# saiakarsh193/GenVox

Hardware: AMD Instinct MI355X
Metric: mel-frames/sec (teacher-forced batch) (higher is better)
Workload: dtype f32

## Files before the change

### genvox_amd/_lib.py

```python
from __future__ import annotations

import ctypes as C
import os

_HERE = os.path.dirname(os.path.abspath(__file__))
LIB_PATH = os.path.join(_HERE, os.environ.get("GVX_LIB", "libgenvox_amd.so"))


class GvxError(RuntimeError):
    pass


class gvx_dims(C.Structure):
    _fields_ = [(n, C.c_int32) for n in (
        "n_tokens", "embed_dim", "enc_kernel", "enc_n_conv", "prenet_dim", "att_rnn_dim", "dec_rnn_dim", "att_dim",
        "att_loc_filters", "att_loc_kernel", "postnet_dim", "postnet_kernel", "postnet_n_conv", "n_mels")]


class gvx_weight_desc(C.Structure):
    _fields_ = [("name", C.c_char_p), ("data", C.c_void_p), ("numel", C.c_int64)]


_vp, _i, _sz, _f, _l = C.c_void_p, C.c_int, C.c_size_t, C.c_float, C.c_long

# ... 192 lines not shown
    "gvx_mel_project": (_i, [_vp, _i, _i, _i, _vp, _i, _vp, _vp]),
    "gvx_dtw_workspace_bytes": (_sz, [_i, _i, _i, _i]),
    "gvx_dtw_uses_lds_tables": (_i, [_i, _i, _i]),
    "gvx_dtw_distance": (_i, [_vp, _vp, _vp, _vp, _i, _i, _i, _i, _vp, _vp, _vp, _sz, _vp]),
    "gvx_monotonic_align_workspace_bytes": (_sz, [_i, _i, _i]),
    "gvx_monotonic_align_uses_lds": (_i, [_i, _i]),
    "gvx_monotonic_align": (_i, [_vp, _vp, _vp, _i, _i, _i, _f, _vp, _vp, _vp, _vp, _vp, _vp, _vp, _sz, _vp]),
    "gvx_duration_scale": (_i, [_vp, _vp, _vp, _i, _i, _f, _vp, _vp, _vp, _vp, _vp]),
    "gvx_mel_time_warp": (_i, [_vp, _vp, _vp, _vp, _i, _i, _i, _i, _i, _vp, _vp, _vp, _vp, _vp]),
    "gvx_pitch_frames": (_i, [_l, _i]),
    "gvx_pitch_tile_frames": (_i, [C.POINTER(gvx_pitch_params)]),
    "gvx_pitch_yin": (_i, [_vp, _vp, _i, _l, C.POINTER(gvx_pitch_params), _vp, _vp, _vp, _vp, _vp]),
    "gvx_f0_compare": (_i, [_vp, _vp, _vp, _vp, _i, _i, _vp, _vp, _vp, _vp, _vp]),
    "gvx_psola_max_marks": (_l, [_l, _i]),
    "gvx_psola_max_grains": (_l, [_l, _i]),
    "gvx_psola_plan": (_i, [_vp, _vp, _vp, _vp, _i, _l, C.POINTER(gvx_psola_params), _vp, _vp, _vp, _vp, _vp, _vp, _vp]),
    "gvx_psola_synth": (_i, [_vp, _vp, _vp, _vp, _vp, _vp, _vp, _vp, _i, _l, C.POINTER(gvx_psola_params), _vp, _vp]),
    "gvx_melgan_blob_floats":(_sz, [C.POINTER(gvx_melgan_dims)]),
    "gvx_melgan_workspace_bytes": (_sz, [C.POINTER(gvx_melgan_dims), _i, _i]),
    "gvx_melgan_pack_weights_device": (_i, [C.POINTER(gvx_melgan_dims), C.POINTER(gvx_weight_desc), _i, _vp, _vp]),
    "gvx_melgan_create": (_i, [C.POINTER(gvx_melgan_dims), C.POINTER(_vp)]),
    "gvx_melgan_destroy": (None, [_vp]),
    "gvx_melgan_bind": (_i, [_vp, _vp]),
    "gvx_melgan_forward": (_i, [_vp, _vp, _vp, _i, _i, _vp, C.POINTER(_vp), _vp, _sz, _vp]),
    "gvx_melgan_timing_enable": (_i, [_vp, _i]),
    "gvx_melgan_stage_times_ms": (_i, [_vp, C.POINTER(_f), C.POINTER(_i)]),
    "gvx_melgan_tape_bytes": (_sz, [C.POINTER(gvx_melgan_dims), _i, _i]),
    "gvx_melgan_tape_layout": (_i, [C.POINTER(gvx_melgan_dims), _i, _i, C.POINTER(gvx_melgan_tape_entry), _i]),
    "gvx_melgan_backward_workspace_bytes": (_sz, [C.POINTER(gvx_melgan_dims), _i, _i]),
    "gvx_melgan_forward_train": (_i, [_vp, _vp, _vp, _i, _i, _vp, _vp, _sz, _vp, _sz, _vp]),
    "gvx_melgan_backward": (_i, [_vp, _vp, _vp, _i, _i, _vp, _sz, C.POINTER(gvx_weight_desc), _i, _vp, _vp, _sz, _vp]),
    "gvx_hifigan_blob_floats": (_sz, [C.POINTER(gvx_hifigan_dims)]),
    "gvx_hifigan_workspace_bytes": (_sz, [C.POINTER(gvx_hifigan_dims), _i, _i]),
    "gvx_hifigan_pack_weights_device": (_i, [C.POINTER(gvx_hifigan_dims), C.POINTER(gvx_weight_desc), _i, _vp, _vp]),
    "gvx_hifigan_create": (_i, [C.POINTER(gvx_hifigan_dims), C.POINTER(_vp)]),
    "gvx_hifigan_destroy": (None, [_vp]),
    "gvx_hifigan_bind": (_i, [_vp, _vp]),
    "gvx_hifigan_forward": (_i, [_vp, _vp, _vp, _i, _i, _vp, C.POINTER(_vp), _vp, _sz, _vp]),
    "gvx_hifigan_timing_enable": (_i, [_vp, _i]),
    "gvx_hifigan_stage_times_ms": (_i, [_vp, C.POINTER(_f), C.POINTER(_i)]),
    "gvx_hifigan_backward_stage_times_ms": (_i, [_vp, C.POINTER(_f), C.POINTER(_i)]),
    "gvx_hifigan_tape_bytes": (_sz, [C.POINTER(gvx_hifigan_dims), _i, _i]),
    "gvx_hifigan_tape_layout": (_i, [C.POINTER(gvx_hifigan_dims), _i, _i, C.POINTER(gvx_melgan_tape_entry), _i]),
    "gvx_hifigan_backward_workspace_bytes": (_sz, [C.POINTER(gvx_hifigan_dims), _i, _i]),
    "gvx_hifigan_forward_train": (_i, [_vp, _vp, _vp, _i, _i, _vp, _vp, _sz, _vp, _sz, _vp]),
    "gvx_hifigan_backward": (_i, [_vp, _vp, _vp, _i, _i, _vp, _sz, C.POINTER(gvx_weight_desc), _i, _vp, _vp, _sz, _vp]),
    "gvx_melgan_disc_blob_floats": (_sz, [C.POINTER(gvx_melgan_disc_dims)]),
    "gvx_melgan_disc_pack_weights_device": (_i, [C.POINTER(gvx_melgan_disc_dims), C.POINTER(gvx_weight_desc), _i, _vp, _vp]),
    "gvx_melgan_disc_create": (_i, [C.POINTER(gvx_melgan_disc_dims), C.POINTER(_vp)]),
    "gvx_melgan_disc_destroy": (None, [_vp]),
    "gvx_melgan_disc_bind": (_i, [_vp, _vp]),
    "gvx_melgan_disc_layout": (_i, [C.POINTER(gvx_melgan_disc_dims), _i, _i, C.POINTER(gvx_melgan_disc_entry), _i]),
    "gvx_melgan_disc_features_bytes": (_sz, [C.POINTER(gvx_melgan_disc_dims), _i, _i]),
    "gvx_melgan_disc_workspace_bytes": (_sz, [C.POINTER(gvx_melgan_disc_dims), _i, _i, _i]),
    "gvx_melgan_disc_forward": (_i, [_vp, _vp, _vp, _i, _i, _vp, _sz, _vp, _sz, _vp]),
    "gvx_melgan_disc_backward": (_i, [_vp, _vp, _vp, _i, _i, _vp, _vp, C.POINTER(gvx_weight_desc), _i, _vp, _vp, _sz, _vp]),
    "gvx_snake_antialiased": (_i, [_vp, _vp, _i, _i, _i, _vp, _vp, _vp, _vp, _vp]),
    "gvx_bigvgan_blob_floats": (_sz, [C.POINTER(gvx_bigvgan_dims)]),
    "gvx_bigvgan_workspace_bytes": (_sz, [C.POINTER(gvx_bigvgan_dims), _i, _i]),
    "gvx_bigvgan_pack_weights_device": (_i, [C.POINTER(gvx_bigvgan_dims), C.POINTER(gvx_weight_desc), _i, _vp, _vp]),
    "gvx_bigvgan_create": (_i, [C.POINTER(gvx_bigvgan_dims), C.POINTER(_vp)]),
    "gvx_bigvgan_destroy": (None, [_vp]),
    "gvx_bigvgan_bind": (_i, [_vp, _vp]),
    "gvx_bigvgan_forward": (_i, [_vp, _vp, _vp, _i, _i, _vp, C.POINTER(_vp), _vp, _sz, _vp]),
    "gvx_bigvgan_timing_enable": (_i, [_vp, _i]),
    "gvx_bigvgan_stage_times_ms": (_i, [_vp, C.POINTER(_f), C.POINTER(_i)]),
    "gvx_dwconv_layernorm": (_i, [_vp, _vp, _i, _i, _i, _i, _vp, _vp, _vp, _vp, _f, _vp, _vp]),
    "gvx_istft_head_workspace_bytes": (_sz, [_i, _i, _i]),
    "gvx_istft_head": (_i, [_vp, _vp, _i, _i, _i, _i, _i, _vp, _vp, _vp, _vp]),
    "gvx_vocos_blob_floats": (_sz, [C.POINTER(gvx_vocos_dims)]),
    "gvx_vocos_workspace_bytes": (_sz, [C.POINTER(gvx_vocos_dims), _i, _i]),
    "gvx_vocos_pack_weights_device": (_i, [C.POINTER(gvx_vocos_dims), C.POINTER(gvx_weight_desc), _i, _vp, _vp]),
    "gvx_vocos_create": (_i, [C.POINTER(gvx_vocos_dims), C.POINTER(_vp)]),
    "gvx_vocos_destroy": (None, [_vp]),
    "gvx_vocos_bind": (_i, [_vp, _vp]),
    "gvx_vocos_forward": (_i, [_vp, _vp, _vp, _i, _i, _vp, C.POINTER(_vp), _vp, _sz, _vp]),
    "gvx_vocos_timing_enable": (_i, [_vp, _i]),
    "gvx_vocos_stage_times_ms": (_i, [_vp, C.POINTER(_f), C.POINTER(_i)]),
    "gvx_self_attention": (_i, [_vp, _vp, _i, _i, _i, _i, _vp, _vp]),
    "gvx_add_layer_norm": (_i, [_vp, _vp, _vp, _i, _i, _i, _vp, _vp, _vp, _vp, _vp]),
    "gvx_fastpitch_blob_floats": (_sz, [C.POINTER(gvx_fastpitch_dims)]),
    "gvx_fastpitch_workspace_bytes": (_sz, [C.POINTER(gvx_fastpitch_dims), _i, _i]),
    "gvx_fastpitch_pack_weights_device": (_i, [C.POINTER(gvx_fastpitch_dims), C.POINTER(gvx_weight_desc), _i, _vp, _vp]),
    "gvx_fastpitch_create": (_i, [C.POINTER(gvx_fastpitch_dims), C.POINTER(_vp)]),
    "gvx_fastpitch_destroy": (None, [_vp]),
    "gvx_fastpitch_bind": (_i, [_vp, _vp]),
    "gvx_fastpitch_encode": (_i, [_vp, _vp, _vp, _i, _i, _f, _vp, _vp, _vp, _vp, _vp, _vp, _vp, _vp, _vp, C.POINTER(_vp), _vp, _sz, _vp]),
    "gvx_fastpitch_decode": (_i, [_vp, _vp, _vp, _vp, _vp, _vp, _i, _i, _i, _vp, _vp, _vp, C.POINTER(_vp), _vp, _sz, _vp]),
    "gvx_fastpitch_timing_enable": (_i, [_vp, _i]),
    "gvx_fastpitch_stage_times_ms": (_i, [_vp, C.POINTER(_f), C.POINTER(_i)]),
    "gvx_lvc_gated": (_i, [_vp, _vp, _i, _i, _vp, _vp, _i, _vp, _i, _i, _i, _i, _f, _vp, _vp, _vp]),
    "gvx_univnet_blob_floats": (_sz, [C.POINTER(gvx_univnet_dims)]),
    "gvx_univnet_workspace_bytes": (_sz, [C.POINTER(gvx_univnet_dims), _i, _i]),
    "gvx_univnet_pack_weights_device": (_i, [C.POINTER(gvx_univnet_dims), C.POINTER(gvx_weight_desc), _i, _vp, _vp]),
    "gvx_univnet_create": (_i, [C.POINTER(gvx_univnet_dims), C.POINTER(_vp)]),
    "gvx_univnet_destroy": (None, [_vp]),
    "gvx_univnet_bind": (_i, [_vp, _vp]),
    "gvx_univnet_forward": (_i, [_vp, _vp, _vp, _vp, _i, _i, _vp, C.POINTER(_vp), _vp, _sz, _vp]),
    "gvx_univnet_timing_enable": (_i, [_vp, _i]),
    "gvx_univnet_stage_times_ms": (_i, [_vp, C.POINTER(_f), C.POINTER(_i)]),
    "gvx_hifigan_mpd_blob_floats": (_sz, [C.POINTER(gvx_hifigan_mpd_dims)]),
    "gvx_hifigan_mpd_pack_weights_device": (_i, [C.POINTER(gvx_hifigan_mpd_dims), C.POINTER(gvx_weight_desc), _i, _vp, _vp]),
    "gvx_hifigan_mpd_create": (_i, [C.POINTER(gvx_hifigan_mpd_dims), C.POINTER(_vp)]),
    "gvx_hifigan_mpd_destroy": (None, [_vp]),
    "gvx_hifigan_mpd_bind": (_i, [_vp, _vp]),
    "gvx_hifigan_mpd_layout": (_i, [C.POINTER(gvx_hifigan_mpd_dims), _i, _i, C.POINTER(gvx_hifigan_mpd_entry), _i]),
    "gvx_hifigan_mpd_features_bytes": (_sz, [C.POINTER(gvx_hifigan_mpd_dims), _i, _i]),
    "gvx_hifigan_mpd_workspace_bytes": (_sz, [C.POINTER(gvx_hifigan_mpd_dims), _i, _i, _i]),
    "gvx_hifigan_mpd_forward": (_i, [_vp, _vp, _vp, _i, _i, _vp, _sz, _vp, _sz, _vp]),
    "gvx_hifigan_mpd_backward": (_i, [_vp, _vp, _vp, _i, _i, _vp, _vp, C.POINTER(gvx_weight_desc), _i, _vp, _vp, _sz, _vp]),
    "gvx_hifigan_mpd_timing_enable": (_i, [_vp, _i]),
    "gvx_hifigan_mpd_layer_times_ms": (_i, [_vp, C.POINTER(_f), C.POINTER(_f), C.POINTER(_i)]),
    "gvx_mrd_blob_floats": (_sz, [C.POINTER(gvx_mrd_dims)]),
    "gvx_mrd_pack_weights_device": (_i, [C.POINTER(gvx_mrd_dims), C.POINTER(gvx_weight_desc), _i, _vp, _vp]),
    "gvx_mrd_create": (_i, [C.POINTER(gvx_mrd_dims), C.POINTER(_vp)]),
    "gvx_mrd_destroy": (None, [_vp]),
    "gvx_mrd_bind": (_i, [_vp, _vp]),
    "gvx_mrd_layout": (_i, [C.POINTER(gvx_mrd_dims), _i, _i, C.POINTER(gvx_mrd_entry), _i]),
    "gvx_mrd_features_bytes": (_sz, [C.POINTER(gvx_mrd_dims), _i, _i]),
    "gvx_mrd_workspace_bytes": (_sz, [C.POINTER(gvx_mrd_dims), _i, _i, _i]),
    "gvx_mrd_forward": (_i, [_vp, _vp, _vp, _i, _i, _vp, _sz, _vp, _sz, _vp]),
    "gvx_mrd_backward": (_i, [_vp, _vp, _vp, _i, _i, _vp, _vp, C.POINTER(gvx_weight_desc), _i, _vp, _vp, _sz, _vp]),
    "gvx_mrd_timing_enable": (_i, [_vp, _i]),
    "gvx_mrd_layer_times_ms": (_i, [_vp, C.POINTER(_f), C.POINTER(_f), C.POINTER(_i)]),
    "gvx_hifigan_msd_blob_floats": (_sz, [C.POINTER(gvx_hifigan_msd_dims)]),
    "gvx_hifigan_msd_pack_weights_device": (_i, [C.POINTER(gvx_hifigan_msd_dims), C.POINTER(gvx_weight_desc), _i, _vp, _vp]),
    "gvx_hifigan_msd_create": (_i, [C.POINTER(gvx_hifigan_msd_dims), C.POINTER(_vp)]),
    "gvx_hifigan_msd_destroy": (None, [_vp]),
    "gvx_hifigan_msd_bind": (_i, [_vp, _vp]),
    "gvx_hifigan_msd_layout": (_i, [C.POINTER(gvx_hifigan_msd_dims), _i, _i, C.POINTER(gvx_hifigan_msd_entry), _i]),
    "gvx_hifigan_msd_features_bytes": (_sz, [C.POINTER(gvx_hifigan_msd_dims), _i, _i]),
    "gvx_hifigan_msd_workspace_bytes": (_sz, [C.POINTER(gvx_hifigan_msd_dims), _i, _i, _i]),
    "gvx_hifigan_msd_forward": (_i, [_vp, _vp, _vp, _i, _i, _vp, _sz, _vp, _sz, _vp]),
    "gvx_hifigan_msd_backward": (_i, [_vp, _vp, _vp, _i, _i, _vp, _vp, C.POINTER(gvx_weight_desc), _i, _vp, _vp, _sz, _vp]),
    "gvx_hifigan_msd_timing_enable": (_i, [_vp, _i]),
    "gvx_hifigan_msd_layer_times_ms": (_i, [_vp, C.POINTER(_f), C.POINTER(_f), C.POINTER(_i)]),
    "gvx_stft_loss_create": (_i, [C.POINTER(gvx_stft_resolution), _i, _f, _f, _f, C.POINTER(_vp)]),
    "gvx_stft_loss_destroy": (None, [_vp]),
    "gvx_stft_loss_workspace_bytes": (_sz, [_vp, _i, _l]),
    "gvx_stft_loss": (_i, [_vp, _vp, _vp, _vp, _i, _l, _vp, _vp, _vp, C.POINTER(gvx_stft_loss_debug), _vp, _sz, _vp]),
    "gvx_mel_loss_create": (_i, [_i, _i, _i, _i, _vp, _f, _f, C.POINTER(_vp)]),
    "gvx_mel_loss_destroy": (None, [_vp]),
    "gvx_mel_loss_bands": (_i, [_vp, _i, _i, _vp, _vp, _vp, _vp]),
    "gvx_mel_loss_workspace_bytes": (_sz, [_vp, _i, _l]),
    "gvx_mel_loss": (_i, [_vp, _vp, _vp, _vp, _i, _l, _vp, _vp, _vp, C.POINTER(gvx_mel_loss_debug), _vp, _sz, _vp]),
    "gvx_denoise_create": (_i, [_i, _i, C.POINTER(_vp)]),
    "gvx_denoise_destroy": (None, [_vp]),
    "gvx_denoise_workspace_bytes": (_sz, [_vp, _i, _l]),
    "gvx_denoise": (_i, [_vp, _vp, _vp, _i, _l, _vp, _f, _vp, _vp, _vp, _sz, _vp]),
    "gvx_kernel_timing_enable": (_i, [_vp, _i]),
    "gvx_model_set_persistent_attention": (_i, [_vp, _i]),
    "gvx_model_set_resident_kernels": (_i, [_vp, _i]),
    "gvx_model_set_winograd": (_i, [_vp, _i]),
    "gvx_debug_conv_plan": (_i, [_vp, _i, _i, _i]),
    "gvx_teacher_forced_rows_per_call": (_i, [_vp, _i]),
    "gvx_teacher_forced_resident": (_i, [_vp, _i, _i]),
    "gvx_teacher_forced_loop_kind": (_i, [_vp, _i, _i]),
    "gvx_autoregressive_loop_kind": (_i, [_vp, _i, _i]),
    "gvx_autoregressive_windowed_loop_kind": (_i, [_vp, _i, _i]),
    "gvx_kernel_times_ms": (_i, [_vp, C.POINTER(_f), C.POINTER(_f), C.POINTER(_i)]),
}

_lib = None


def load() -> C.CDLL:
    global _lib
    if _lib is not None:
        return _lib
    if not os.path.exists(LIB_PATH):
        raise ImportError(
            f"{LIB_PATH} not found: build the gfx950 library first (python -m genvox_amd.build, or "
            f"__graft_entry__.build()). genvox_amd has no CPU or eager fallback.")
    import torch

    lib = C.CDLL(LIB_PATH)
    for name, (res, args) in SIGNATURES.items():
        fn = getattr(lib, name)
        fn.restype = res
        fn.argtypes = args
    _lib = lib
    return lib


def check(rc: int) -> None:
    if rc != 0:
        msg = load().gvx_last_error()
        raise GvxError(f"genvox_amd error {rc}: {msg.decode() if msg else '?'}")
```

### genvox_amd/build.py

```python
from __future__ import annotations

import glob
import os
import subprocess
import sys
from concurrent.futures import ThreadPoolExecutor

HERE = os.path.dirname(os.path.abspath(__file__))
CSRC = os.path.join(HERE, "csrc")
LIB = os.path.join(HERE, "libgenvox_amd.so")
SOURCES = ["gemm_f32.hip", "winograd_conv.hip", "skinny.hip", "dec_resident.hip", "attention.hip", "attn_persist.hip", "misc.hip", "griffinlim.hip", "wav_finalize.hip", "wav_to_mel.hip", "resample.hip", "eval_metrics.hip", "mas.hip", "time_warp.hip", "melgan.hip", "melgan_train.hip", "melgan_disc.hip", "hifigan.hip", "hifigan_train.hip", "hifigan_disc.hip", "hifigan_msd.hip", "mrd.hip", "bigvgan.hip", "vocos.hip", "univnet.hip", "fastpitch.hip", "pitch.hip", "psola.hip", "stft_loss.hip", "mel_loss.hip", "denoise.hip",
           "train_conv.hip", "train_ops.hip", "train_bptt_decoder.hip", "train_bptt_encoder.hip", "train_guided.hip", "gvx_pack.hip", "gvx_decoder.hip", "gvx_api.hip"]
ARCH = "gfx950"
HIPCC = os.environ.get("HIPCC", "/opt/rocm/bin/hipcc")
CXXFLAGS = ["-O3", "-std=c++17", "-fPIC", f"--offload-arch={ARCH}", "-Wall", "-Wno-unused-function",
            "-ffp-contract=off"]


def _newer(a: str, b: str) -> bool:
    return not os.path.exists(b) or os.path.getmtime(a) > os.path.getmtime(b)


def build(force: bool = False, verbose: bool = True, stamps: bool = False) -> str:
    objs, jobs = [], []
    flags = CXXFLAGS + (["-DGVX_STAMPS"] if stamps else []) + os.environ.get("GVX_EXTRA_FLAGS", "").split()
    lib = LIB.replace(".so", "_stamps.so") if stamps else LIB
    if os.environ.get("GVX_LIB_NAME"):
        lib = os.path.join(HERE, os.environ["GVX_LIB_NAME"])
    sfx = ".stamps.o" if stamps else ".o"
    if os.environ.get("GVX_LIB_NAME"):
        sfx = "." + os.environ["GVX_LIB_NAME"] + ".o"
    headers = sorted(glob.glob(os.path.join(CSRC, "*.h"))) + [os.path.join(os.path.dirname(HERE), "include", "genvox_amd.h")]
    for src in SOURCES:
        s = os.path.join(CSRC, src)
        o = os.path.join(CSRC, src.replace(".hip", sfx))
        objs.append(o)
        if force or _newer(s, o) or any(_newer(h, o) for h in headers):
            jobs.append([HIPCC, *flags, "-c", s, "-o", o])

    def run(cmd):
        if verbose:
            print(" ".join(cmd), flush=True)
        subprocess.run(cmd, check=True)

    if jobs:
        with ThreadPoolExecutor(max_workers=min(4, len(jobs))) as ex:
            list(ex.map(run, jobs))
    if jobs or not os.path.exists(lib):
        run([HIPCC, "-shared", "-fPIC", f"--offload-arch={ARCH}", *objs, "-L/opt/rocm/lib", "-lrocfft", "-Wl,-rpath,/opt/rocm/lib", "-o", lib])
    if not stamps and not os.environ.get("GVX_LIB_NAME"):
        variant = LIB.replace(".so", "_stamps.so")
        if os.path.exists(variant) and os.path.getmtime(variant) < os.path.getmtime(headers[-1]):
            os.remove(variant)
    return lib


if __name__ == "__main__":
    print(build(force="--force" in sys.argv, stamps="--stamps" in sys.argv))
```

### genvox_amd/csrc/gvx_api.hip

```cpp
#include "gvx_internal.h"

namespace gvx {
#ifdef GVX_STAMPS
hipError_t read_stamps_skinny(unsigned long long* host96);
hipError_t read_stamps_attention(unsigned long long* host96);
hipError_t read_stamps_persist(unsigned long long* host96);
hipError_t read_wg_spans(unsigned long long* host1024);
hipError_t read_stamps_resident(unsigned long long* host480);
hipError_t read_wg_stamps_resident(unsigned long long* host896);
hipError_t read_wg_stamps_resident_ar(unsigned long long* host896);
hipError_t read_row_stamps_persist_ar(unsigned long long* host256);
hipError_t read_loc_stamps_persist(unsigned long long* host32);
hipError_t read_row_stamps_persist(unsigned long long* host512);
#endif
hipError_t skinny_init();
hipError_t gemm_init();
int gemm_set_parent_epilogue(int on);
int gemm_epilogue_of(int tile, const GemmParams& p);
hipError_t attention_init();
hipError_t attention_persistent_init();
}

using namespace gvx;

// ... 9 lines not shown
    va_list ap;
    va_start(ap, fmt);
    vsnprintf(buf, sizeof buf, fmt, ap);
    va_end(ap);
    g_err = buf;
    return code;
}

std::mutex& capture_mutex() { return g_capture_mutex; }

bool conv_uses_winograd(const gvx_model* m, int cin, int cout, int k) {
    if (m->winograd <= 0 || !winograd_shape_ok(cin, cout, k)) return false;
    return m->winograd >= 2 || cin >= WINOGRAD_MIN_CHANNELS;
}

size_t winograd_scratch_floats(const gvx_model* m, int B, int T) {
    bool any = false;
    for (int i = 0; i < m->d.postnet_n_conv; ++i) any = any || postnet_layer_winograd_shape(m->d, i);
    if (!any) return 0;
    const size_t tile = (size_t)2 * WINO_PTS * m->d.postnet_dim, all = (size_t)B * ((T + WINO_OUT - 1) / WINO_OUT) * tile;
    const size_t budget = WINOGRAD_GROUP_BYTES / sizeof(float) / tile * tile;
    return all <= budget ? all : budget > tile ? budget : tile;
}

long winograd_group_tiles(long total, long fit, int C) {
    if (fit >= total) return total;
    const long groups = (total + fit - 1) / fit, per = (total + groups - 1) / groups;
    GemmParams g{};
    g.M = (int)per; g.N = C; g.K = C; g.slices = WINO_PTS;
    const long unit = gemm_round_rows(g);
    if (unit <= 0) return per;
    auto whole = [&](long rows) { g.M = (int)rows; return rows > 0 && rows <= fit && rows % unit == 0 && gemm_round_rows(g) == unit; };
    const long down = per / unit * unit, up = (per + unit - 1) / unit * unit, most = fit / unit * unit;
    if (whole(down) && total - (groups - 1) * down <= fit) return down;
    if (whole(up)) return up;
    return whole(most) ? most : per;
}

WsPlan make_ws_plan(const gvx_model* m, int B, int L, int T, int mode) {
    const gvx_dims& d = m->d;
    const int E = d.embed_dim, H = E / 2, M = d.n_mels, P = d.prenet_dim, A = d.att_rnn_dim, D = d.dec_rnn_dim;
    const int pe = (d.enc_kernel - 1) / 2, pp = (d.postnet_kernel - 1) / 2;
    WsPlan w{};
    size_t off = 0;
    auto take = [&](size_t floats) { size_t o = off; off = align_up(off + floats * sizeof(float), 256); return o; };
    w.flags = take(128);
    w.sync = take(HANDOFF_WORDS);
    w.xa = take((size_t)B * (L + 2 * pe) * E);
    w.xb = take((size_t)B * (L + 2 * pe) * E);
    w.xg = take((size_t)B * L * 8 * H);
    w.enc_h = take((size_t)2 * 2 * B * H);
    w.enc_c = take((size_t)2 * B * H);
    w.memory = take((size_t)B * L * E);
    w.len_copy = take((size_t)B);
    w.pm = take((size_t)B * L * d.att_dim);
    w.frames = take((size_t)(T + 1) * B * M);
    w.pre1 = take((size_t)(T + 1) * B * P);
    w.prenet = take((size_t)(T + 1) * B * P);
    w.h_a = take((size_t)RS_HA_SLOTS * B * A);
    w.c_a = take((size_t)B * A);
    w.c_d = take((size_t)B * D);
    w.hc = take((size_t)(T + 1) * B * (D + E));
    w.w_cum = take((size_t)B * L);
    w.q_slab = take((size_t)(A / 8) * B * d.att_dim);
    w.proj = take((size_t)B * T * m->PSB());
    w.energies = take((size_t)B * L);
    w.align_tm = take((size_t)T * B * L);
    w.loc = take((size_t)B * L * d.att_dim);
    w.p_slab = take((size_t)(D / 8) * B * m->PSB());
    w.p_ctx = take((size_t)B * m->PSB());
    w.att_part = take((size_t)2 * B * 4 * A);
    w.dec_part = take((size_t)2 * B * 4 * D);
    w.pre_gate = take(mode == WS_TEACHER_FORCED && plan_teacher_forced(m, B, L, TF_INFERENCE).pre_gate ? (size_t)T * B * 4 * A : 0);
    w.xchg = take(attention_persistent_xchg_floats(B));
    w.ar_masks = take(((size_t)2 * T * B * P + 3) / 4);
    const int cmax = d.postnet_dim > M ? d.postnet_dim : M;
    w.ya = take((size_t)B * (T + 2 * pp) * cmax);
    w.yb = take((size_t)B * (T + 2 * pp) * cmax);
    w.total = off;
    return w;
}

gvx_model::GraphSet* touch_graph_set(gvx_model* m, std::vector<gvx_model::GraphSet>& cache, const gvx_model::LoopKey& key) {
    gvx_model::GraphSet* hit = nullptr;
    for (auto& gs : cache)
        if (gs.key == key) hit = &gs;
    if (!hit) {
        if (cache.size() >= gvx_model::GRAPH_SETS) {
            size_t lru = 0;
            for (size_t i = 1; i < cache.size(); ++i)
                if (cache[i].last_use < cache[lru].last_use) lru = i;
            for (auto e : cache[lru].execs)
                if (e) (void)hipGraphExecDestroy(e);
            cache.erase(cache.begin() + lru);
        }
        cache.emplace_back();
        hit = &cache.back();
        hit->key = key;
    }
    ++hit->sightings;
    hit->last_use = ++m->use_clock;
    return hit;
}

int check_common(const gvx_model* m, int B, int L, int T, void* ws, size_t ws_bytes, int mode) {
    if (!m) return fail(GVX_ERR_INVALID_ARG, "null model");
    if (!m->dev_blob) return fail(GVX_ERR_STATE, "weights not bound (call gvx_model_bind_blob)");
    if (B < 1 || B > 64) return fail(GVX_ERR_UNSUPPORTED, "batch %d not in [1, 64] (shard larger batches across calls / GPUs)", B);
    if (L < 1 || T < 1) return fail(GVX_ERR_INVALID_ARG, "L and T must be >= 1");
    if (!ws) return fail(GVX_ERR_WORKSPACE, "null workspace");
    if (reinterpret_cast<uintptr_t>(ws) & 255) return fail(GVX_ERR_WORKSPACE, "workspace must be 256-byte aligned");
    const size_t need = make_ws_plan(m, B, L, T, mode).total;
    if (ws_bytes < need) return fail(GVX_ERR_WORKSPACE, "workspace too small: %zu < %zu bytes", ws_bytes, need);
    if (!attention_supported(L, m->d.att_dim, m->d.att_loc_filters, m->d.att_loc_kernel, m->d.embed_dim))
        return fail(GVX_ERR_UNSUPPORTED, "L = %d is too long for the attention kernels' LDS budget", L);
    return GVX_OK;
}

}

namespace {

int check_dims(const gvx_dims& d) {
    if (d.n_tokens < 1) return fail(GVX_ERR_INVALID_ARG, "n_tokens must be >= 1");
    const int dims8[] = {d.embed_dim, d.prenet_dim, d.att_rnn_dim, d.dec_rnn_dim, d.att_dim, d.postnet_dim, d.n_mels};
    const char* names[] = {"embed_dim", "prenet_dim", "att_rnn_dim", "dec_rnn_dim", "att_dim", "postnet_dim", "n_mels"};
    for (int i = 0; i < 7; ++i)
        if (dims8[i] < 8 || dims8[i] % 8) return fail(GVX_ERR_UNSUPPORTED, "%s = %d must be a positive multiple of 8", names[i], dims8[i]);
    if (d.embed_dim % 16) return fail(GVX_ERR_UNSUPPORTED, "embed_dim = %d must be a multiple of 16 (BiLSTM halves are multiples of 8)", d.embed_dim);
    if (d.att_dim > 256) return fail(GVX_ERR_UNSUPPORTED, "att_dim = %d > 256 is not supported", d.att_dim);
    if (d.att_loc_filters < 1 || d.att_loc_filters > 32) return fail(GVX_ERR_UNSUPPORTED, "att_loc_filters = %d must be in [1, 32]", d.att_loc_filters);
    const int ks[] = {d.enc_kernel, d.att_loc_kernel, d.postnet_kernel};
    for (int k : ks)
        if (k < 1 || k % 2 == 0) return fail(GVX_ERR_UNSUPPORTED, "kernel size %d must be odd (the reference pads (k-1)/2 on both sides)", k);
    if (d.enc_n_conv < 1 || d.enc_n_conv > MAX_CONV || d.postnet_n_conv < 1 || d.postnet_n_conv > MAX_CONV)
        return fail(GVX_ERR_UNSUPPORTED, "number of convolutions must be in [1, %d]", MAX_CONV);
    return GVX_OK;
}

void read_knobs(gvx_model* m) {
    auto env = [](const char* name) { const char* e = std::getenv(name); return e ? e : ""; };
    auto flag = [&](const char* name, bool dflt) { const char c = env(name)[0]; return c == '\0' ? dflt : dflt ? c != '0' : c == '1'; };
    auto number = [&](const char* name, int dflt) { const char* e = env(name); return e[0] ? std::atoi(e) : dflt; };
    m->use_graph = !flag("GVX_NO_GRAPH", false);
    m->capture_first = flag("GVX_GRAPH_FIRST", false);
    m->attn_one_launch = !flag("GVX_ATTN_SPLIT", false);
    m->attn_persistent = flag("GVX_ATTN_PERSISTENT", true);
    for (const char* name : {"AMD_SERIALIZE_KERNEL", "HIP_LAUNCH_BLOCKING"})
        if (env(name)[0] != '\0' && env(name)[0] != '0') m->attn_persistent = false;
    m->ar_resident = flag("GVX_AR_RESIDENT", false);
    m->ar_split_h = flag("GVX_AR_SPLIT_H", true);
    m->enc_persistent = flag("GVX_ENC_PERSISTENT", true);
    m->enc_fork_after = number("GVX_ENC_FORK_AFTER", 2);
    m->train_resident = flag("GVX_TRAIN_RESIDENT", true);
    m->train_resident_loop = flag("GVX_TRAIN_RESIDENT_LOOP", true);
    m->tf_rows64 = flag("GVX_TF_ROWS64", false);
    m->tf_resident = flag("GVX_TF_RESIDENT", true);
    m->ar_resident_loop = flag("GVX_AR_RESIDENT_LOOP", true);
    m->tf_long_rows_224 = flag("GVX_TF_LONG_224", true);
    m->attn_prefetch = flag("GVX_ATTN_PREFETCH", true);
    m->pa_depth = number("GVX_PA_DEPTH", 4) == 6 ? 6 : 4;
    m->side_pool = env("GVX_SIDE_POOL")[0] == '2' ? 2u : 1u;
    m->spin_limit = (unsigned)std::strtoul(env("GVX_HANDOFF_SPIN_LIMIT"), nullptr, 10);
    m->rs_debug = number("GVX_RS_DEBUG", 0);
    m->debug_skip_resident = flag("GVX_DEBUG_SKIP_RESIDENT", false);
    m->debug_enc_skip_block = number("GVX_DEBUG_ENC_SKIP_BLOCK", -1);
    m->debug_plan = std::getenv("GVX_DEBUG_PLAN") != nullptr;
    m->winograd = number("GVX_CONV_WINOGRAD", 1);
    if (m->winograd < 0 || m->winograd > 2) m->winograd = 1;
}

}

extern "C" {

const char* gvx_last_error(void) { return g_err.c_str(); }
int gvx_version(void) { return 1; }

int gvx_model_create(const gvx_dims* dims, gvx_model** out) {
    if (!dims || !out) return fail(GVX_ERR_INVALID_ARG, "null argument");
    int rc = check_dims(*dims);
    if (rc != GVX_OK) return rc;
    gvx_model* m = new gvx_model();
    m->d = *dims;
    m->blob = make_blob_layout(*dims);
    read_knobs(m);
    *out = m;
    return GVX_OK;
}

void gvx_model_destroy(gvx_model* m) {
    if (m) {
        if (m->gather_off) (void)hipFree(m->gather_off);
        if (m->gather_tid) (void)hipFree(m->gather_tid);
    }
    if (!m) return;
    if (m->ev_valid)
        for (auto& e : m->ev) (void)hipEventDestroy(e);
    for (auto& e : m->kev) (void)hipEventDestroy(e);
    m->drop_graphs();
    if (m->cap_stream) (void)hipStreamDestroy(m->cap_stream);
    if (m->pa_fork) (void)hipEventDestroy(m->pa_fork);
    if (m->pa_join) (void)hipEventDestroy(m->pa_join);
    if (m->enc_mid) (void)hipEventDestroy(m->enc_mid);
    if (m->ar_done_host) (void)hipHostFree(m->ar_done_host);
    for (hipEvent_t e : m->ar_ev)
        if (e) (void)hipEventDestroy(e);
    delete m;
}

size_t gvx_model_blob_bytes(const gvx_model* m) { return m ? m->blob.total * sizeof(float) : 0; }

int gvx_model_bind_blob(gvx_model* m, const void* device_blob) {
    if (!m || !device_blob) return fail(GVX_ERR_INVALID_ARG, "null argument");
    if (reinterpret_cast<uintptr_t>(device_blob) & 255) return fail(GVX_ERR_INVALID_ARG, "blob must be 256-byte aligned");
    if (m->dev_blob != device_blob) m->drop_graphs();
    m->dev_blob = reinterpret_cast<const float*>(device_blob);
    HIP_TRY(gemm_init());
    HIP_TRY(skinny_init());
    HIP_TRY(attention_init());
    HIP_TRY(attention_persistent_init());
    HIP_TRY(decoder_resident_init());
    return GVX_OK;
}

size_t gvx_workspace_bytes(const gvx_model* m, int B, int L, int T) {
    if (!m || B < 1 || L < 1 || T < 1) return 0;
    return make_ws_plan(m, B, L, T).total;
}

size_t gvx_workspace_bytes_autoregressive(const gvx_model* m, int B, int L, int max_steps) {
    if (!m || B < 1 || L < 1 || max_steps < 1) return 0;
    return make_ws_plan(m, B, L, max_steps, WS_AUTOREGRESSIVE).total;
}

}

namespace {

int conv_layer(const gvx_model* m, const float* in, float* out, int B, int T, int cin, int cout, int k, size_t w_off, size_t b_off,
               int act, int out_halo, hipStream_t s) {
    const int p = (k - 1) / 2;
    GemmParams g{};
    g.A = in; g.amap = RowMap{T, (long)(T + 2 * p) * cin, (long)cin};
    g.W = m->dev_blob + w_off; g.ldw = (long)k * cin;
    g.C = out + (long)out_halo * cout; g.cmap = RowMap{T, (long)(T + 2 * out_halo) * cout, (long)cout};
    g.bias = m->dev_blob + b_off;
    g.M = B * T; g.N = cout; g.K = k * cin; g.act = act;
    HIP_TRY(launch_gemm(g, s));
    return GVX_OK;
}

int winograd_layer(const gvx_model* m, const char* who, const float* cur, float* nxt, int B, int T, int C, size_t u_off, size_t b_off,
                   const int32_t* row_len, int act, float* wino, size_t wino_floats, hipStream_t s) {
    const long total = (long)B * ((T + WINO_OUT - 1) / WINO_OUT);
    const size_t tile = (size_t)2 * WINO_PTS * C, budget = WINOGRAD_GROUP_BYTES / sizeof(float);
    long fit = (long)((wino_floats < budget ? wino_floats : budget) / tile);
    if (fit < 1) return fail(GVX_ERR_WORKSPACE, "%s: %zu floats of scratch do not hold one Winograd tile (%zu)", who, wino_floats, tile);
    if (m->wino_group > 0 && m->wino_group < fit) fit = m->wino_group;
    const long per_group = winograd_group_tiles(total, fit, C);
    for (long mt0 = 0, Mt; mt0 < total; mt0 += Mt) {
        Mt = total - mt0 <= fit ? total - mt0 : per_group;
        float* V = wino;
        float* Mm = wino + (size_t)WINO_PTS * Mt * C;
        HIP_TRY(launch_winograd_input(cur, V, B, mt0, Mt, T, C, s));
        GemmParams g{};
        g.A = V; g.amap = RowMap{(int)Mt, 0, (long)C};
        g.W = m->dev_blob + u_off; g.ldw = C;
        g.C = Mm; g.cmap = RowMap{(int)Mt, 0, (long)C};
        g.bias = nullptr; g.M = (int)Mt; g.N = C; g.K = C; g.act = ACT_NONE;
        g.slices = WINO_PTS; g.a_slice = Mt * C; g.w_slice = (long)C * C; g.c_slice = Mt * C;
        HIP_TRY(launch_gemm(g, s));
        HIP_TRY(launch_winograd_output(Mm, m->dev_blob + b_off, row_len, nxt, B, mt0, Mt, T, C, act, s));
    }
    return GVX_OK;
}

struct WinoScratch { size_t off, floats; };
WinoScratch encoder_wino_scratch(const WsPlan& wp, bool alone) {
    if (alone) return {wp.xg, (wp.total - wp.xg) / sizeof(float)};
    const size_t front = wp.frames - wp.xg, back = wp.pre_gate - wp.h_a;
    return front >= back ? WinoScratch{wp.xg, front / sizeof(float)} : WinoScratch{wp.h_a, back / sizeof(float)};
}

int encoder_impl(gvx_model* m, const int64_t* tokens, const int32_t* lengths, int B, int L, float* memory_out, void* ws,
                 const WsPlan& wp, const WinoScratch& wsc, hipStream_t s, const float* conv_out = nullptr, float* c_seq_out = nullptr,
                 float* xg_out = nullptr, hipEvent_t dense_done = nullptr) {
    const gvx_dims& d = m->d;
    const int E = d.embed_dim, H = E / 2, pe = (d.enc_kernel - 1) / 2;
    float* xa = ws_ptr<float>(ws, wp.xa);
    float* xb = ws_ptr<float>(ws, wp.xb);
    float* xg = ws_ptr<float>(ws, wp.xg);
    float* enc_h = ws_ptr<float>(ws, wp.enc_h);
    float* enc_c = ws_ptr<float>(ws, wp.enc_c);
    int* flags = ws_ptr<int>(ws, wp.flags);
    float* cur = xa;
    float* nxt = xb;
    if (conv_out) {
        HIP_TRY(launch_to_channels_last(conv_out, xa, B, E, L, pe, nullptr, s));
    } else {
        HIP_TRY(launch_embed(tokens, m->dev_blob + m->blob.emb, d.n_tokens, xa, xb, B, L, E, pe, flags + FLAG_TOKEN, s));
        for (int i = 0; i < d.enc_n_conv; ++i) {
            if (dense_done && i == m->enc_fork_after) { HIP_TRY(hipEventRecord(dense_done, s)); dense_done = nullptr; }
            const bool wino = encoder_layer_winograd_shape(d, i) && conv_uses_winograd(m, E, E, d.enc_kernel);
            int rc = wino ? winograd_layer(m, "encoder", cur, nxt, B, L, E, m->blob.enc_u[i], m->blob.enc_b[i], nullptr, ACT_RELU,
                                           ws_ptr<float>(ws, wsc.off), wsc.floats, s)
                          : conv_layer(m, cur, nxt, B, L, E, E, d.enc_kernel, m->blob.enc_w[i], m->blob.enc_b[i], ACT_RELU, pe, s);
            if (rc != GVX_OK) return rc;
            float* t = cur; cur = nxt; nxt = t;
        }
    }
    if (dense_done) HIP_TRY(hipEventRecord(dense_done, s));
    {
        GemmParams g{};
        g.A = cur + (long)pe * E; g.amap = RowMap{L, (long)(L + 2 * pe) * E, (long)E};
        g.W = m->dev_blob + m->blob.enc_wih; g.ldw = E;
        g.C = xg; g.cmap = RowMap{B * L, 0, (long)8 * H};
        g.bias = m->dev_blob + m->blob.enc_bih;
        g.M = B * L; g.N = 8 * H; g.K = E; g.act = ACT_NONE;
        HIP_TRY(launch_gemm(g, s));
    }
    const bool resident = m->enc_persistent && encoder_persistent_supported(B, H);
    if (!resident) HIP_TRY(zero_async(enc_h, (size_t)4 * B * H * sizeof(float), s));
    if (!resident) HIP_TRY(zero_async(enc_c, (size_t)2 * B * H * sizeof(float), s));
    float* mem_ws = ws_ptr<float>(ws, wp.memory);
    if (!resident) HIP_TRY(zero_async(mem_ws, (size_t)B * L * E * sizeof(float), s));
    const int32_t* len_ws = nullptr;
    if (lengths) {
        int32_t* lc = ws_ptr<int32_t>(ws, wp.len_copy);
        HIP_TRY(hipMemcpyAsync(lc, lengths, (size_t)B * sizeof(int32_t), hipMemcpyDeviceToDevice, s));
        len_ws = lc;
    }
    auto enqueue = [&](hipStream_t st) -> int {
        for (int step = 0; step < L; ++step) {
            SkinnyJob jobs[2];
            for (int dir = 0; dir < 2; ++dir) {
                SkinnyJob& J = jobs[dir];
                std::memset(&J, 0, sizeof J);
                float* h_cur = enc_h + ((size_t)dir * 2 + (step & 1)) * B * H;
                float* h_nxt = enc_h + ((size_t)dir * 2 + ((step + 1) & 1)) * B * H;
                J.Wp = m->dev_blob + m->blob.enc_whh_frag[dir];
                J.x[0] = XSeg{h_cur, H};
                J.N = 4 * H; J.nkg = H / 8; J.mode = 0; J.B = B;
                J.c = enc_c + (size_t)dir * B * H;
                J.h_out = h_nxt;
                J.addend = xg + (size_t)dir * 4 * H; J.add_bs = (long)L * 8 * H; J.add_ts = 8 * H;
                J.lengths = len_ws; J.step = step; J.reverse = dir; J.seq_len = L;
                J.seq_out = mem_ws + (size_t)dir * H; J.seq_bs = (long)L * E; J.seq_ts = E;
                if (c_seq_out) J.c_seq_out = c_seq_out + (size_t)dir * H;
                J.h_prev = h_cur;
            }
            HIP_TRY(launch_skinny(jobs, 2, SK_ENCODER, st));
        }
        return GVX_OK;
    };
    if (resident) {
        unsigned* sync = ws_ptr<unsigned>(ws, wp.sync);
        void* const zp[2] = {enc_h, sync + HANDOFF_TIMEOUT};
        const size_t zb[2] = {(size_t)4 * B * H * sizeof(float), sizeof(unsigned)};
        HIP_TRY(launch_zero_many(zp, zb, 2, s));
        EncPersistParams ep{};
        ep.Wp[0] = m->dev_blob + m->blob.enc_whh_frag[0]; ep.Wp[1] = m->dev_blob + m->blob.enc_whh_frag[1];
        ep.xg = xg; ep.lengths = len_ws; ep.hx = enc_h; ep.seq_out = mem_ws; ep.c_seq_out = c_seq_out;
        ep.sync = sync; ep.spin_limit = m->spin_limit; ep.B = B; ep.L = L; ep.H = H;
        ep.debug_skip_block = m->debug_enc_skip_block;
        HIP_TRY(launch_encoder_persistent(ep, s));
        float* outs[2] = {mem_ws, c_seq_out};
        const size_t counts[2] = {(size_t)B * L * E, (size_t)B * L * E};
        HIP_TRY(launch_poison_on_timeout(sync + HANDOFF_TIMEOUT, flags + FLAG_TIMEOUT, outs, counts, c_seq_out ? 2 : 1, s));
    } else {
        const gvx_model::LoopKey key{ws, mem_ws, m->dev_blob, B, L, 0, lengths != nullptr};
        const int rc = run_chunk(m, m->use_graph && !c_seq_out ? touch_graph_set(m, m->enc_graphs, key) : nullptr, 0, s, enqueue);
        if (rc != GVX_OK) return rc;
    }
    if (xg_out) HIP_TRY(hipMemcpyAsync(xg_out, xg, (size_t)B * L * 8 * H * sizeof(float), hipMemcpyDeviceToDevice, s));
    if (memory_out != mem_ws)
        HIP_TRY(hipMemcpyAsync(memory_out, mem_ws, (size_t)B * L * E * sizeof(float), hipMemcpyDeviceToDevice, s));
    return GVX_OK;
}

int postnet_impl(gvx_model* m, const float* mel_in, const int32_t* mel_lengths, int B, int T, float* mel_post_out, float* ya,
                 float* yb, float* wino, size_t wino_floats, hipStream_t s) {
    const gvx_dims& d = m->d;
    const int M = d.n_mels, pp = (d.postnet_kernel - 1) / 2, n = d.postnet_n_conv;
    HIP_TRY(launch_to_channels_last(mel_in, ya, B, M, T, pp, mel_lengths, s));
    float* cur = ya;
    float* nxt = yb;
    for (int i = 0; i < n; ++i) {
        const int cin = i == 0 ? M : d.postnet_dim, cout = i == n - 1 ? M : d.postnet_dim;
        const bool last = i == n - 1;
        if (postnet_layer_winograd_shape(d, i) && conv_uses_winograd(m, cin, cout, d.postnet_kernel)) {
            const int rc = winograd_layer(m, "Postnet", cur, nxt, B, T, cin, m->blob.post_u[i], m->blob.post_b[i], mel_lengths, ACT_TANH, wino, wino_floats, s);
            if (rc != GVX_OK) return rc;
            float* t = cur; cur = nxt; nxt = t;
            continue;
        }
        const int out_halo = last ? 0 : pp;
        const bool fused_halo = out_halo > 0 && T >= out_halo;
        if (out_halo > 0 && !fused_halo) HIP_TRY(launch_zero_halo(nxt, B, T, pp, cout, s));
        GemmParams g{};
        g.A = cur; g.amap = RowMap{T, (long)(T + 2 * pp) * cin, (long)cin};
        g.W = m->dev_blob + m->blob.post_w[i]; g.ldw = (long)d.postnet_kernel * cin;
        g.C = nxt + (long)out_halo * cout; g.cmap = RowMap{T, (long)(T + 2 * out_halo) * cout, (long)cout};
        g.bias = m->dev_blob + m->blob.post_b[i];
        g.M = B * T; g.N = cout; g.K = d.postnet_kernel * cin; g.act = last ? ACT_NONE : ACT_TANH;
        g.row_len = last ? nullptr : mel_lengths;
        g.c_halo = fused_halo ? out_halo : 0;
        HIP_TRY(launch_gemm(g, s));
        float* t = cur; cur = nxt; nxt = t;
    }
    HIP_TRY(launch_residual_to_channels_first(mel_in, cur, mel_post_out, B, M, T, mel_lengths, s));
    return GVX_OK;
}

struct PostnetPlan { size_t ya, yb, wino, wino_floats, total; };
PostnetPlan make_postnet_plan(const gvx_model* m, int B, int T) {
    const gvx_dims& d = m->d;
    const int pp = (d.postnet_kernel - 1) / 2, cmax = d.postnet_dim > d.n_mels ? d.postnet_dim : d.n_mels;
    const size_t buf = align_up((size_t)B * (T + 2 * pp) * cmax * sizeof(float), 256);
    PostnetPlan p;
    p.ya = align_up((128 + HANDOFF_WORDS) * sizeof(float), 256);
    p.yb = p.ya + buf;
    p.wino = p.yb + buf;
    const WsPlan w = make_ws_plan(m, B, 1, T, WS_AUTOREGRESSIVE);
    const size_t tile = (size_t)2 * WINO_PTS * d.postnet_dim, room = (w.ya - w.xa) / sizeof(float) / tile * tile;
    p.wino_floats = winograd_scratch_floats(m, B, T);
    if (p.wino_floats > room) p.wino_floats = room > tile ? room : tile;
    p.total = p.wino + align_up(p.wino_floats * sizeof(float), 256);
    return p;
}

}

extern "C" {

int gvx_teacher_forced_rows_per_call(const gvx_model* m, int L) {
    if (!m) return 0;
    return plan_teacher_forced(m, 64, L, TF_INFERENCE).kind != 0 ? 64 : 32;
}

int gvx_teacher_forced_resident(const gvx_model* m, int B, int L) {
    if (!m || B < 1 || L < 1) return 0;
    return plan_teacher_forced(m, B, L, TF_INFERENCE).kind != 0 ? 1 : 0;
}

int gvx_teacher_forced_loop_kind(const gvx_model* m, int B, int L) {
    if (!m || B < 1 || L < 1) return 0;
    return plan_teacher_forced(m, B, L, TF_INFERENCE).kind;
}

int gvx_autoregressive_loop_kind(const gvx_model* m, int B, int L) {
    if (!m || B < 1 || L < 1) return 0;
    return plan_autoregressive(m, B, L).kind;
}

int gvx_autoregressive_windowed_loop_kind(const gvx_model* m, int B, int L) {
    if (!m || B < 1 || L < 1) return 0;
    return plan_autoregressive(m, B, L, true).kind;
}

int gvx_debug_decoder_plan_windowed(const gvx_model* m, int B, int L, int* out) {
    if (!m || !out) return fail(GVX_ERR_INVALID_ARG, "null argument");
    if (B < 1 || L < 1) return fail(GVX_ERR_INVALID_ARG, "B, L >= 1 (got %d, %d)", B, L);
    const ArLoopPlan a = plan_autoregressive(m, B, L, true);
    out[0] = a.kind; out[1] = a.split_h; out[2] = a.fold; out[3] = a.graph;
    return GVX_OK;
}

int gvx_debug_decoder_plan(const gvx_model* m, int mode, int B, int L, int* out) {
    if (!m || !out) return fail(GVX_ERR_INVALID_ARG, "null argument");
    if (mode < 0 || mode > 2 || B < 1 || L < 1) return fail(GVX_ERR_INVALID_ARG, "mode must be 0, 1 or 2 and B, L >= 1 (got %d, %d, %d)", mode, B, L);
    const TfLoopPlan t = plan_teacher_forced(m, B, L, (TfMode)mode);
    const ArLoopPlan a = plan_autoregressive(m, B, L);
    const int v[12] = {t.kind, t.pa_layout, t.tile_layout, t.rows64, t.pre_gate, t.timeout_check, t.side_stream, t.graph,
                       a.kind, a.split_h, a.fold, a.graph};
    for (int i = 0; i < 12; ++i) out[i] = v[i];
    return GVX_OK;
}

long long gvx_debug_graph_replays(const gvx_model* m) { return m ? (long long)m->graph_replays : -1; }

int gvx_debug_encoder_resident(const gvx_model* m, int B) {
    if (!m || B < 1) return 0;
    return m->enc_persistent && encoder_persistent_supported(B, m->H()) ? 1 : 0;
}

int gvx_model_set_persistent_attention(gvx_model* m, int enable) {
    if (!m) return fail(GVX_ERR_INVALID_ARG, "null argument");
    m->attn_persistent = enable != 0;
    return GVX_OK;
}

int gvx_model_set_winograd(gvx_model* m, int mode) {
    if (!m) return fail(GVX_ERR_INVALID_ARG, "null argument");
    if (mode < 0 || mode > 2) return fail(GVX_ERR_INVALID_ARG, "winograd mode must be 0, 1 or 2 (got %d)", mode);
    m->winograd = mode;
    return GVX_OK;
}

int gvx_debug_conv_plan(const gvx_model* m, int cin, int cout, int k) {
    if (!m || cin < 1 || cout < 1 || k < 1) return -1;
    return conv_uses_winograd(m, cin, cout, k) ? 1 : 0;
}

int gvx_debug_set_winograd_group(gvx_model* m, int tiles) {
    if (!m || tiles < 0) return fail(GVX_ERR_INVALID_ARG, "bad argument");
    m->wino_group = tiles;
    return GVX_OK;
}

long gvx_debug_winograd_group_tiles(long total, long fit, int channels) {
    if (total < 1 || fit < 1 || channels < 4 || total > INT_MAX) return -1;
    return winograd_group_tiles(total, fit, channels);
}

int gvx_debug_gemm_parent_epilogue(int on) { return gemm_set_parent_epilogue(on); }

int gvx_debug_gemm_epilogue(int tile, int kmajor, int has_bias, int act, int has_keep, int has_row_len, int c_halo) {
    if (tile < 1111 || tile > 9999 || c_halo < 0) return -1;
    static const float some_bias = 0.f; static const uint8_t some_keep = 0; static const int32_t some_len = 0;
    GemmParams g{};
    g.kmajor = kmajor != 0;
    g.bias = has_bias ? &some_bias : nullptr; g.act = act;
    g.keep = has_keep ? &some_keep : nullptr; g.row_len = has_row_len ? &some_len : nullptr; g.c_halo = c_halo;
    return gemm_epilogue_of(tile, g);
}

int gvx_debug_gemm_row_walk(int R, long s1, long s0, int first_row, long* off, int* grp, int* idx) {
    if (R < 1 || first_row < 0 || !off || !grp || !idx) return GVX_ERR_INVALID_ARG;
    const RowMap map{R, s1, s0};
    RowWalk w = row_walk_begin(map, first_row);
    for (int q = 0; q < 16; ++q) {
        if (q > 0) row_walk_advance(w, map, mfma32_row_step(q));
        off[q] = w.off; grp[q] = w.grp; idx[q] = w.idx;
    }
    return GVX_OK;
}

int gvx_debug_winograd_constants(double* at, double* g, double* bt) {
    if (!at || !g || !bt) return fail(GVX_ERR_INVALID_ARG, "null argument");
    for (int i = 0; i < WINO_OUT; ++i)
        for (int s = 0; s < WINO_PTS; ++s) at[i * WINO_PTS + s] = wino_AT(i, s);
    for (int s = 0; s < WINO_PTS; ++s) {
        for (int k = 0; k < WINO_TAPS; ++k) g[s * WINO_TAPS + k] = wino_G(s, k);
        for (int i = 0; i < WINO_PTS; ++i) bt[s * WINO_PTS + i] = wino_BT(s, i);
    }
    return GVX_OK;
}

int gvx_model_set_resident_kernels(gvx_model* m, int enable) {
    if (!m) return fail(GVX_ERR_INVALID_ARG, "null argument");
    m->attn_persistent = m->enc_persistent = m->tf_resident = enable != 0;
    if (!enable) m->ar_resident = false;
    return GVX_OK;
}

int gvx_workspace_status(const gvx_model* m, void* ws, size_t ws_bytes, void* stream, int32_t* host_out) {
    if (!m || !ws || !host_out) return fail(GVX_ERR_INVALID_ARG, "null argument");
    const WsPlan wp = make_ws_plan(m, 1, 1, 1, WS_AUTOREGRESSIVE);
    if (ws_bytes < wp.flags + 4 * sizeof(int32_t)) return fail(GVX_ERR_WORKSPACE, "workspace too small");
    hipStream_t s = (hipStream_t)stream;
    int32_t h[4] = {0, 0, 0, 0}, tmo = 0;
    int32_t* flags = ws_ptr<int32_t>(ws, wp.flags);
    HIP_TRY(hipMemcpyAsync(h, flags, sizeof h, hipMemcpyDeviceToHost, s));
    if (ws_bytes >= wp.sync + HANDOFF_WORDS * sizeof(unsigned))
        HIP_TRY(hipMemcpyAsync(&tmo, reinterpret_cast<const char*>(ws) + wp.sync + HANDOFF_TIMEOUT * sizeof(unsigned), sizeof tmo,
                               hipMemcpyDeviceToHost, s));
    HIP_TRY(zero_async(flags + FLAG_TOKEN, sizeof(int32_t), s));
    HIP_TRY(zero_async(flags + FLAG_TIMEOUT, sizeof(int32_t), s));
    if (ws_bytes >= wp.sync + HANDOFF_WORDS * sizeof(unsigned))
        HIP_TRY(zero_async(ws_ptr<unsigned>(ws, wp.sync) + HANDOFF_TIMEOUT, sizeof(unsigned), s));
    HIP_TRY(hipStreamSynchronize(s));
    host_out[0] = h[FLAG_TOKEN];
    host_out[1] = h[FLAG_TIMEOUT] ? h[FLAG_TIMEOUT] : tmo;
    return GVX_OK;
}

int gvx_encoder_forward(gvx_model* m, const int64_t* tokens, const int32_t* lengths, int B, int L, float* memory_out,
                        void* ws, size_t ws_bytes, void* stream) {
    int rc = check_common(m, B, L, 1, ws, ws_bytes, WS_AUTOREGRESSIVE);
    if (rc != GVX_OK) return rc;
    if (!tokens || !memory_out) return fail(GVX_ERR_INVALID_ARG, "null argument");
    const WsPlan wp = make_ws_plan(m, B, L, 1, WS_AUTOREGRESSIVE);
    return encoder_impl(m, tokens, lengths, B, L, memory_out, ws, wp, encoder_wino_scratch(wp, true), (hipStream_t)stream);
}

int gvx_decoder_teacher_forced(gvx_model* m, const float* memory, const int32_t* lengths, int B, int L, const float* mel_in, int T,
                               const uint8_t* keep_masks, float* mel_out, float* gate_out, float* align_out, void* ws,
                               size_t ws_bytes, void* stream) {
    int rc = check_common(m, B, L, T, ws, ws_bytes);
    if (rc != GVX_OK) return rc;
    if (!memory || !mel_in || !keep_masks || !mel_out || !gate_out || !align_out) return fail(GVX_ERR_INVALID_ARG, "null argument");
    const WsPlan wp = make_ws_plan(m, B, L, T);
    rc = decoder_tf_impl(m, memory, lengths, B, L, mel_in, T, keep_masks, mel_out, gate_out, align_out, ws, wp, (hipStream_t)stream);
    if (rc != GVX_OK) return rc;
    float* outs[3] = {mel_out, gate_out, align_out};
    const size_t counts[3] = {(size_t)B * m->d.n_mels * T, (size_t)B * T, (size_t)B * T * L};
    return poison_if_timed_out(m, B, L, ws, wp, outs, counts, 3, (hipStream_t)stream);
}

int gvx_encoder_lstm_forward(gvx_model* m, const float* conv_out, const int32_t* lengths, int B, int L, float* memory_out,
                             float* cell_states_out, float* input_preact_out, void* ws, size_t ws_bytes, void* stream) {
    int rc = check_common(m, B, L, 1, ws, ws_bytes, WS_AUTOREGRESSIVE);
    if (rc != GVX_OK) return rc;
    if (!conv_out || !memory_out) return fail(GVX_ERR_INVALID_ARG, "null argument");
    if (cell_states_out) HIP_TRY(zero_async(cell_states_out, (size_t)B * L * m->d.embed_dim * sizeof(float), (hipStream_t)stream));
    const WsPlan wp = make_ws_plan(m, B, L, 1, WS_AUTOREGRESSIVE);
    return encoder_impl(m, nullptr, lengths, B, L, memory_out, ws, wp, encoder_wino_scratch(wp, true), (hipStream_t)stream, conv_out, cell_states_out,
                        input_preact_out);
}

int gvx_decoder_teacher_forced_train(gvx_model* m, const float* memory, const int32_t* lengths, int B, int L, const float* mel_in, int T,
                                     const uint8_t* keep_masks, const uint8_t* att_keep, const uint8_t* dec_keep, float p_att, float p_dec,
                                     float* mel_out, float* gate_out, float* align_out, float* att_hidden_all, float* att_cell_all,
                                     float* dec_cell_all, float* dec_hidden_context_all, float* att_preact_all, float* dec_preact_all,
                                     void* ws, size_t ws_bytes, void* stream) {
    int rc = check_common(m, B, L, T, ws, ws_bytes);
    if (rc != GVX_OK) return rc;
    if (!memory || !mel_in || !keep_masks || !att_keep || !dec_keep || !mel_out || !gate_out || !align_out) return fail(GVX_ERR_INVALID_ARG, "null argument");
    if (!(p_att >= 0.f && p_att < 1.f && p_dec >= 0.f && p_dec < 1.f)) return fail(GVX_ERR_INVALID_ARG, "dropout probabilities must be in [0, 1)");
    if (plan_teacher_forced(m, B, L, TF_TRAIN_PARTIAL_TAPE).rows64)
        return fail(GVX_ERR_UNSUPPORTED, "training mode with %d rows on a GVX_TF_ROWS64 handle: the 64-row loop has no dropout and no tape (at most 32 rows per call)", B);
    hipStream_t s = (hipStream_t)stream;
    const int A = m->d.att_rnn_dim, D = m->d.dec_rnn_dim, E = m->d.embed_dim;
    const LstmDropout tr{att_keep, dec_keep, 1.f / (1.f - p_att), 1.f / (1.f - p_dec), att_hidden_all, att_cell_all, dec_cell_all, att_preact_all, dec_preact_all};
    if (att_hidden_all) HIP_TRY(zero_async(att_hidden_all, (size_t)B * A * sizeof(float), s));
    if (att_cell_all) HIP_TRY(zero_async(att_cell_all, (size_t)B * A * sizeof(float), s));
    if (dec_cell_all) HIP_TRY(zero_async(dec_cell_all, (size_t)B * D * sizeof(float), s));
    const WsPlan wp = make_ws_plan(m, B, L, T);
    rc = decoder_tf_impl(m, memory, lengths, B, L, mel_in, T, keep_masks, mel_out, gate_out, align_out, ws, wp, s, false, &tr);
    if (rc != GVX_OK) return rc;
    {
        float* outs[3] = {mel_out, gate_out, align_out};
        const size_t counts[3] = {(size_t)B * m->d.n_mels * T, (size_t)B * T, (size_t)B * T * L};
        rc = poison_if_timed_out(m, B, L, ws, wp, outs, counts, 3, s);
        if (rc != GVX_OK) return rc;
    }
    if (dec_hidden_context_all)
        HIP_TRY(hipMemcpyAsync(dec_hidden_context_all, ws_ptr<float>(ws, wp.hc), (size_t)(T + 1) * B * (D + E) * sizeof(float),
                               hipMemcpyDeviceToDevice, s));
    return GVX_OK;
}

int gvx_train_export(const gvx_model* m, const void* ws_c, size_t ws_bytes, int B, int L, int T, int what, float* dst, void* stream) {
    void* ws = const_cast<void*>(ws_c);
    if (!m || !ws || !dst) return fail(GVX_ERR_INVALID_ARG, "null argument");
    const WsPlan wp = make_ws_plan(m, B, L, T);
    if (ws_bytes < wp.total) return fail(GVX_ERR_WORKSPACE, "workspace too small");
    const gvx_dims& d = m->d;
    hipStream_t s = (hipStream_t)stream;
    const size_t rows = (size_t)(T + 1) * B;
    switch (what) {
        case 0: HIP_TRY(hipMemcpyAsync(dst, ws_ptr<float>(ws, wp.frames), rows * d.n_mels * sizeof(float), hipMemcpyDeviceToDevice, s)); break;
        case 1: HIP_TRY(hipMemcpyAsync(dst, ws_ptr<float>(ws, wp.pre1), rows * d.prenet_dim * sizeof(float), hipMemcpyDeviceToDevice, s)); break;
        case 2: return gvx_train_unblock(ws_ptr<float>(ws, wp.prenet), dst, T + 1, B, d.prenet_dim, stream);
        case 3: HIP_TRY(hipMemcpyAsync(dst, ws_ptr<float>(ws, wp.pm), (size_t)B * L * d.att_dim * sizeof(float), hipMemcpyDeviceToDevice, s)); break;
        case 4: HIP_TRY(hipMemcpyAsync(dst, ws_ptr<float>(ws, wp.memory), (size_t)B * L * d.embed_dim * sizeof(float), hipMemcpyDeviceToDevice, s)); break;
        default: return fail(GVX_ERR_INVALID_ARG, "gvx_train_export: unknown buffer %d", what);
    }
    return GVX_OK;
}

size_t gvx_postnet_workspace_bytes(const gvx_model* m, int B, int T) {
    if (!m || B < 1 || T < 1) return 0;
    return make_postnet_plan(m, B, T).total;
}

int gvx_postnet_forward(gvx_model* m, const float* mel_in, const int32_t* mel_lengths, int B, int T, float* mel_post_out, void* ws,
                        size_t ws_bytes, void* stream) {
    if (!m) return fail(GVX_ERR_INVALID_ARG, "null model");
    if (!m->dev_blob) return fail(GVX_ERR_STATE, "weights not bound (call gvx_model_bind_blob)");
    if (B < 1 || T < 1) return fail(GVX_ERR_INVALID_ARG, "B and T must be >= 1");
    if ((long)B * T > (1L << 30)) return fail(GVX_ERR_UNSUPPORTED, "B * T = %ld frames exceed the GEMM row index range", (long)B * T);
    if (!ws) return fail(GVX_ERR_WORKSPACE, "null workspace");
    if (reinterpret_cast<uintptr_t>(ws) & 255) return fail(GVX_ERR_WORKSPACE, "workspace must be 256-byte aligned");
    const PostnetPlan pp = make_postnet_plan(m, B, T);
    if (ws_bytes < pp.total) return fail(GVX_ERR_WORKSPACE, "workspace too small: %zu < %zu bytes", ws_bytes, pp.total);
    if (!mel_in || !mel_post_out) return fail(GVX_ERR_INVALID_ARG, "null argument");
    return postnet_impl(m, mel_in, mel_lengths, B, T, mel_post_out, ws_ptr<float>(ws, pp.ya), ws_ptr<float>(ws, pp.yb), ws_ptr<float>(ws, pp.wino), pp.wino_floats,
                        (hipStream_t)stream);
}

int gvx_mask_padding(float* mel, float* mel_post, float* gate, const int32_t* mel_lengths, int B, int n_mels, int T, void* stream) {
    if (!mel_lengths || B < 1 || T < 1 || n_mels < 1) return fail(GVX_ERR_INVALID_ARG, "bad argument");
    HIP_TRY(launch_mask_padding(mel, mel_post, gate, mel_lengths, B, n_mels, T, (hipStream_t)stream));
    return GVX_OK;
}

int gvx_tacotron2_forward(gvx_model* m, const int64_t* tokens, const int32_t* token_lengths, int B, int L, const float* mel_in,
                          const int32_t* mel_lengths, int T, const uint8_t* keep_masks, float* mel_out, float* mel_post_out,
                          float* gate_out, float* align_out, void* ws, size_t ws_bytes, void* stream) {
    int rc = check_common(m, B, L, T, ws, ws_bytes);
    if (rc != GVX_OK) return rc;
    if (!tokens || !mel_in || !keep_masks || !mel_out || !gate_out || !align_out)
        return fail(GVX_ERR_INVALID_ARG, "null argument");
    hipStream_t s = (hipStream_t)stream;
    const WsPlan wp = make_ws_plan(m, B, L, T);
    const bool timed = m->timing && m->ev_valid;
    float* memory = ws_ptr<float>(ws, wp.memory);
    if (timed) HIP_TRY(hipEventRecord(m->ev[0], s));
    const bool overlap = plan_teacher_forced(m, B, L, TF_INFERENCE).side_stream;
    if (overlap) {
        rc = ensure_side_stream(m);
        if (rc != GVX_OK) return rc;
        HIP_TRY(hipEventRecord(m->pa_fork, s));
        HIP_TRY(hipStreamWaitEvent(m->pa_stream, m->pa_fork, 0));
        rc = encoder_impl(m, tokens, token_lengths, B, L, memory, ws, wp, encoder_wino_scratch(wp, false), m->pa_stream, nullptr, nullptr, nullptr, m->enc_mid);
        if (rc != GVX_OK) return rc;
        rc = decoder_init_states(m, memory, B, L, decoder_buffers(ws, wp), m->pa_stream);
        if (rc != GVX_OK) return rc;
        HIP_TRY(hipEventRecord(m->pa_join, m->pa_stream));
        HIP_TRY(hipStreamWaitEvent(s, m->enc_mid, 0));
        rc = decoder_prenet_part(m, B, L, mel_in, T, keep_masks, ws, wp, s);
        if (rc != GVX_OK) return rc;
        HIP_TRY(hipStreamWaitEvent(s, m->pa_join, 0));
    } else {
        rc = encoder_impl(m, tokens, token_lengths, B, L, memory, ws, wp, encoder_wino_scratch(wp, false), s);
        if (rc != GVX_OK) return rc;
    }
    if (timed) HIP_TRY(hipEventRecord(m->ev[1], s));
    rc = decoder_tf_impl(m, memory, token_lengths, B, L, mel_in, T, keep_masks, mel_out, gate_out, align_out, ws, wp, s, overlap);
    if (rc != GVX_OK) return rc;
    if (timed) HIP_TRY(hipEventRecord(m->ev[4], s));
    if (mel_post_out) {
        rc = postnet_impl(m, mel_out, nullptr, B, T, mel_post_out, ws_ptr<float>(ws, wp.ya), ws_ptr<float>(ws, wp.yb), ws_ptr<float>(ws, wp.xa),
                          (wp.ya - wp.xa) / sizeof(float), s);
        if (rc != GVX_OK) return rc;
        if (mel_lengths) HIP_TRY(launch_mask_padding(mel_out, mel_post_out, gate_out, mel_lengths, B, m->d.n_mels, T, s));
    }
    float* outs[4] = {mel_out, gate_out, align_out, mel_post_out};
    const size_t nm = (size_t)B * m->d.n_mels * T;
    const size_t counts[4] = {nm, (size_t)B * T, (size_t)B * T * L, nm};
    rc = poison_if_timed_out(m, B, L, ws, wp, outs, counts, mel_post_out ? 4 : 3, s);
    if (rc != GVX_OK) return rc;
    if (timed) HIP_TRY(hipEventRecord(m->ev[5], s));
    return GVX_OK;
}

int gvx_tacotron2_loss(const float* mel_out, const float* mel_post_out, const float* gate_out, const float* mel_target,
                       const float* gate_target, int B, int n_mels, int T, float* loss_out, void* scratch, size_t scratch_bytes,
                       void* stream) {
    if (!mel_out || !mel_post_out || !gate_out || !mel_target || !gate_target || !loss_out || !scratch)
        return fail(GVX_ERR_INVALID_ARG, "null argument");
    if (B < 1 || n_mels < 1 || T < 1) return fail(GVX_ERR_INVALID_ARG, "B, n_mels and T must be >= 1");
    if (scratch_bytes < loss_scratch_bytes() || (reinterpret_cast<uintptr_t>(scratch) & 7))
        return fail(GVX_ERR_WORKSPACE, "scratch too small (%zu bytes needed) or not 8-byte aligned", loss_scratch_bytes());
    HIP_TRY(launch_tacotron2_loss(mel_out, mel_post_out, gate_out, mel_target, gate_target, (long)B * n_mels * T, (long)B * T,
                                  reinterpret_cast<double*>(scratch), loss_out, (hipStream_t)stream));
    return GVX_OK;
}

int gvx_prenet_masks_generate(uint8_t* masks_out, size_t n, uint64_t seed, void* stream) {
    if (!masks_out) return fail(GVX_ERR_INVALID_ARG, "null argument");
    HIP_TRY(launch_mask_gen(masks_out, n, seed, (hipStream_t)stream));
    return GVX_OK;
}

int gvx_stage_timing_enable(gvx_model* m, int enable) {
    if (!m) return fail(GVX_ERR_INVALID_ARG, "null model");
    if (enable && !m->ev_valid) {
        for (auto& e : m->ev) HIP_TRY(hipEventCreate(&e));
        m->ev_valid = true;
    }
    m->timing = enable != 0;
    return GVX_OK;
}

int gvx_kernel_timing_enable(gvx_model* m, int enable) {
    if (!m) return fail(GVX_ERR_INVALID_ARG, "null model");
    m->ktiming = enable != 0;
    return GVX_OK;
}

int gvx_kernel_times_ms(gvx_model* m, float* lstm_avg_ms, float* attn_avg_ms, int* n_steps) {
    if (!m || !lstm_avg_ms || !attn_avg_ms) return fail(GVX_ERR_INVALID_ARG, "null argument");
    if (m->n_lstm_ev < 1) return fail(GVX_ERR_STATE, "no timed decoder loop has run");
    HIP_TRY(hipEventSynchronize(m->kev[2]));
    float a = 0, b = 0;
    HIP_TRY(hipEventElapsedTime(&a, m->kev[0], m->kev[1]));
    HIP_TRY(hipEventElapsedTime(&b, m->kev[1], m->kev[2]));
    *lstm_avg_ms = a / m->n_lstm_ev;
    *attn_avg_ms = m->n_attn_ev > 0 ? b / m->n_attn_ev : 0.f;
    if (n_steps) *n_steps = m->n_lstm_ev;
    return GVX_OK;
}

int gvx_stage_times_ms(gvx_model* m, float* t5, int* launches) {
    if (!m || !t5) return fail(GVX_ERR_INVALID_ARG, "null argument");
    if (!m->ev_valid) return fail(GVX_ERR_STATE, "stage timing was not enabled");
    HIP_TRY(hipEventSynchronize(m->ev[5]));
    for (int i = 0; i < 5; ++i) HIP_TRY(hipEventElapsedTime(&t5[i], m->ev[i], m->ev[i + 1]));
    if (launches) *launches = m->last_decoder_launches;
    return GVX_OK;
}
#ifdef GVX_STAMPS
int gvx_debug_read_stamps_skinny(unsigned long long* host96) {
    HIP_TRY(hipDeviceSynchronize());
    HIP_TRY(gvx::read_stamps_skinny(host96));
    return GVX_OK;
}
int gvx_debug_read_stamps_persist(unsigned long long* host96) {
    HIP_TRY(hipDeviceSynchronize());
    HIP_TRY(gvx::read_stamps_persist(host96));
    return GVX_OK;
}
int gvx_debug_read_wg_spans(unsigned long long* host1024) {
    HIP_TRY(hipDeviceSynchronize());
    HIP_TRY(gvx::read_wg_spans(host1024));
    return GVX_OK;
}
int gvx_debug_read_stamps_resident(unsigned long long* host480) {
    HIP_TRY(hipDeviceSynchronize());
    HIP_TRY(gvx::read_stamps_resident(host480));
    return GVX_OK;
}
int gvx_debug_read_wg_stamps_resident(unsigned long long* host896, unsigned long long* rows512) {
    HIP_TRY(hipDeviceSynchronize());
    HIP_TRY(gvx::read_wg_stamps_resident(host896));
    HIP_TRY(gvx::read_row_stamps_persist(rows512));
    return GVX_OK;
}
int gvx_debug_read_loc_stamps(unsigned long long* host32) {
    HIP_TRY(hipDeviceSynchronize());
    HIP_TRY(gvx::read_loc_stamps_persist(host32));
    return GVX_OK;
}
int gvx_debug_read_stamps_ar(unsigned long long* host896, unsigned long long* rows256) {
    HIP_TRY(hipDeviceSynchronize());
    HIP_TRY(gvx::read_wg_stamps_resident_ar(host896));
    HIP_TRY(gvx::read_row_stamps_persist_ar(rows256));
    return GVX_OK;
}
int gvx_debug_read_stamps(unsigned long long* host96) {
    HIP_TRY(hipDeviceSynchronize());
    unsigned long long tmp[96];
    HIP_TRY(gvx::read_stamps_skinny(host96));
    HIP_TRY(gvx::read_stamps_attention(tmp));
    for (int i = 32; i < 96; ++i) host96[i] = tmp[i];
    return GVX_OK;
}
#endif

}
```

### genvox_amd/csrc/gvx_decoder.hip

```cpp
#include "gvx_internal.h"

using namespace gvx;

namespace gvx {

namespace {
bool resident_attention_serves(const gvx_model* m, int B, int L) {
    const gvx_dims& d = m->d;
    return attention_persistent_supported(B, L, d.att_dim, d.att_loc_filters, d.att_loc_kernel, d.embed_dim, d.att_rnn_dim, d.dec_rnn_dim);
}
}

TfLoopPlan plan_teacher_forced(const gvx_model* m, int B, int L, TfMode mode) {
    TfLoopPlan p{};
    const bool train = mode != TF_INFERENCE;
    const bool pa_shape = (B <= 32 || m->tf_rows64) && m->attn_persistent && m->attn_one_launch && resident_attention_serves(m, B, L);
    const bool pa = pa_shape && (!train || m->train_resident);
    p.pa_layout = attention_persistent_layout(B, L);
    const bool resident = pa && (p.pa_layout == 1 || p.pa_layout == 2) && m->tf_resident &&
                          (!train || (m->train_resident_loop && mode == TF_TRAIN_WHOLE_TAPE)) && decoder_resident_supported(B, L);
    p.kind = resident ? 2 : (pa ? 1 : 0);
    p.tile_layout = resident && p.pa_layout == 2 && B > 2 && B <= 16 && m->tf_long_rows_224 ? 1 : p.pa_layout;
    p.rows64 = p.kind == 1 && p.pa_layout == 3;
    p.pre_gate = p.timeout_check = pa_shape;
    p.side_stream = p.kind != 0;
    p.graph = m->use_graph && !m->ktiming && p.kind != 2 && (p.rows64 || !train);
    return p;
}

ArLoopPlan plan_autoregressive(const gvx_model* m, int B, int L, bool windowed) {
    ArLoopPlan p{};
    const gvx_dims& d = m->d;
    const int E = d.embed_dim, D = d.dec_rnn_dim, lay = attention_persistent_layout(B, L);
    const bool pa_any = m->attn_one_launch && resident_attention_serves(m, B, L);
    const bool pair = pa_any && B <= 32 && E / 4 == D / 8 && m->attn_persistent && m->tf_resident && m->ar_resident_loop &&
                      decoder_resident_supported(B, L) && (lay == 1 || (lay == 2 && B <= 16)) && d.prenet_dim == 256 && d.n_mels <= 80 &&
                      m->PSB() <= 96 && d.att_dim == 128;
    p.kind = pair ? 2 : (pa_any && lay == 1 && m->ar_resident ? 1 : 0);
    if (windowed && !(p.kind == 2 && lay == 1)) p.kind = 0;
    p.fold = B <= 32 && E / 4 == D / 8;
    p.split_h = p.kind == 0 && m->ar_split_h && m->attn_persistent && m->attn_one_launch && B <= 32 && d.att_dim > 32 && d.att_dim <= 128;
    p.graph = m->use_graph && p.kind != 2;
    return p;
}

DecoderBuffers decoder_buffers(void* ws, const WsPlan& wp) {
    DecoderBuffers b;
    b.pm = ws_ptr<float>(ws, wp.pm); b.frames = ws_ptr<float>(ws, wp.frames); b.pre1 = ws_ptr<float>(ws, wp.pre1);
    b.prenet = ws_ptr<float>(ws, wp.prenet); b.h_a = ws_ptr<float>(ws, wp.h_a); b.c_a = ws_ptr<float>(ws, wp.c_a);
    b.c_d = ws_ptr<float>(ws, wp.c_d); b.hc = ws_ptr<float>(ws, wp.hc); b.w_cum = ws_ptr<float>(ws, wp.w_cum);
    b.q_slab = ws_ptr<float>(ws, wp.q_slab); b.proj = ws_ptr<float>(ws, wp.proj); b.energies = ws_ptr<float>(ws, wp.energies);
    b.align_tm = ws_ptr<float>(ws, wp.align_tm); b.len_copy = ws_ptr<int32_t>(ws, wp.len_copy);
    b.loc = ws_ptr<float>(ws, wp.loc);
    b.p_slab = ws_ptr<float>(ws, wp.p_slab); b.p_ctx = ws_ptr<float>(ws, wp.p_ctx);
    b.att_part = ws_ptr<float>(ws, wp.att_part); b.dec_part = ws_ptr<float>(ws, wp.dec_part);
    b.pre_gate = ws_ptr<float>(ws, wp.pre_gate);
    return b;
}

int decoder_init_states(gvx_model* m, const float* memory, int B, int L, const DecoderBuffers& db, hipStream_t s) {
    const gvx_dims& d = m->d;
    const int E = d.embed_dim, A = d.att_rnn_dim, D = d.dec_rnn_dim;
    void* const zp[5] = {db.h_a, db.c_a, db.c_d, db.hc , db.w_cum};
    const size_t zb[5] = {(size_t)RS_HA_SLOTS * B * A * sizeof(float), (size_t)B * A * sizeof(float), (size_t)B * D * sizeof(float),
                          (size_t)B * (D + E) * sizeof(float), (size_t)B * L * sizeof(float)};
    HIP_TRY(launch_zero_many(zp, zb, 5, s));
    GemmParams g{};
    g.A = memory; g.amap = RowMap{B * L, 0, (long)E};
    g.W = m->dev_blob + m->blob.wmem; g.ldw = E;
    g.C = db.pm; g.cmap = RowMap{B * L, 0, (long)d.att_dim};
    g.M = B * L; g.N = d.att_dim; g.K = E; g.act = ACT_NONE;
    HIP_TRY(launch_gemm(g, s));
    return GVX_OK;
}

namespace {

void fill_att_job(const gvx_model* m, SkinnyJob& J, const float* prenet_t, int t, int B, const DecoderBuffers& db) {
    const gvx_dims& d = m->d;
    const int E = d.embed_dim, P = d.prenet_dim, A = d.att_rnn_dim, D = d.dec_rnn_dim;
    std::memset(&J, 0, sizeof J);
    const float* hc_t = db.hc + (size_t)t * B * (D + E);
    J.Wp = m->dev_blob + m->blob.att_frag; J.bias = m->dev_blob + m->blob.att_bias;
    J.x[0] = XSeg{prenet_t, P};
    J.x[1] = XSeg{hc_t + (size_t)D * B, E};
    J.x[2] = XSeg{db.h_a + (size_t)(t & 1) * B * A, A};
    J.N = 4 * A; J.nkg = (P + E + A) / 8; J.mode = 0; J.B = B;
    J.c = db.c_a;
    J.h_out = db.h_a + (size_t)((t + 1) & 1) * B * A;
    J.Wq_t = m->dev_blob + m->blob.wq_t; J.q_slab = db.q_slab; J.att_dim = d.att_dim;
}

void fill_dec_job(const gvx_model* m, SkinnyJob& J, int t, int B, const DecoderBuffers& db) {
    const gvx_dims& d = m->d;
    const int E = d.embed_dim, A = d.att_rnn_dim, D = d.dec_rnn_dim;
    std::memset(&J, 0, sizeof J);
    const float* hc_t = db.hc + (size_t)t * B * (D + E);
    float* hc_n = db.hc + (size_t)(t + 1) * B * (D + E);
    J.Wp = m->dev_blob + m->blob.dec_frag; J.bias = m->dev_blob + m->blob.dec_bias;
    J.x[0] = XSeg{db.h_a + (size_t)((t + 1) & 1) * B * A, A};
    J.x[1] = XSeg{hc_n + (size_t)D * B, E};
    J.x[2] = XSeg{hc_t, D};
    J.N = 4 * D; J.nkg = (A + E + D) / 8; J.mode = 0; J.B = B;
    J.c = db.c_d;
    J.h_out = hc_n;
}

void fill_loc(const gvx_model* m, LocJob& q, int t, int B, int L, const float* align_base, long align_bs, long align_ts,
              const DecoderBuffers& db) {
    const gvx_dims& d = m->d;
    q.w_prev = t > 0 ? align_base + (size_t)(t - 1) * align_ts : nullptr; q.w_prev_bs = align_bs;
    q.w_cum = db.w_cum;
    q.loc_conv_t = m->dev_blob + m->blob.loc_conv; q.loc_dense_t = m->dev_blob + m->blob.loc_dense;
    q.loc_out = db.loc;
    q.pm = m->attn_one_launch ? db.pm : nullptr;
    q.B = B; q.L = L; q.a = d.att_dim; q.kl = d.att_loc_kernel; q.G = attention_groups(B, L);
}

void fill_attn(const gvx_model* m, AttnParams& p, const float* memory, const int32_t* lengths, int t, int B, int L,
               float* align_out, long align_bs, long align_ts, const DecoderBuffers& db) {
    const gvx_dims& d = m->d;
    const int E = d.embed_dim, D = d.dec_rnn_dim;
    std::memset(&p, 0, sizeof p);
    p.q_slab = db.q_slab; p.n_slabs = d.att_rnn_dim / 8;
    p.w_cum = db.w_cum;
    p.loc = db.loc; p.v = m->dev_blob + m->blob.v;
    p.pm = db.pm; p.memory = memory; p.lengths = lengths;
    p.w_out = align_out + (size_t)t * align_ts; p.w_out_bs = align_bs;
    p.ctx_out = db.hc + (size_t)(t + 1) * B * (D + E) + (size_t)D * B;
    p.energies = db.energies;
    p.B = B; p.L = L; p.a = d.att_dim; p.F = d.att_loc_filters; p.kl = d.att_loc_kernel; p.E = E;
    p.G = m->attn_one_launch ? attention_slices(B, E) : attention_groups(B, L);
}

hipError_t launch_attn(const gvx_model* m, const AttnParams& p, hipStream_t s) {
    return m->attn_one_launch ? launch_attention_step(p, s) : launch_attention(p, s);
}

struct SidePool { hipStream_t s[2] = {nullptr, nullptr}; unsigned next = 0; };
std::mutex g_pool_mutex;
std::unordered_map<int, SidePool> g_side_pools;

struct ResidentTurn { hipEvent_t ev[4] = {nullptr, nullptr, nullptr, nullptr}; unsigned n = 0; };
std::mutex g_turn_mutex;
std::unordered_map<int, ResidentTurn> g_turns;

int turn_begin(hipStream_t s) {
    int dev = 0;
    HIP_TRY(hipGetDevice(&dev));
    ResidentTurn& t = g_turns[dev];
    if (!t.ev[0])
        for (auto& e : t.ev) HIP_TRY(hipEventCreateWithFlags(&e, hipEventDisableTiming));
    if (t.n > 0) HIP_TRY(hipStreamWaitEvent(s, t.ev[(t.n - 1) & 3], 0));
    return GVX_OK;
}
int turn_end(hipStream_t s) {
    int dev = 0;
    HIP_TRY(hipGetDevice(&dev));
    ResidentTurn& t = g_turns[dev];
    HIP_TRY(hipEventRecord(t.ev[t.n & 3], s));
    ++t.n;
    return GVX_OK;
}

}

int ensure_side_stream(gvx_model* m) {
    if (!m->pa_fork) {
        HIP_TRY(hipEventCreateWithFlags(&m->pa_fork, hipEventDisableTiming));
        HIP_TRY(hipEventCreateWithFlags(&m->pa_join, hipEventDisableTiming));
        HIP_TRY(hipEventCreateWithFlags(&m->enc_mid, hipEventDisableTiming));
    }
    int dev = 0;
    HIP_TRY(hipGetDevice(&dev));
    std::lock_guard<std::mutex> lock(g_pool_mutex);
    SidePool& pool = g_side_pools[dev];
    if (!pool.s[0]) {
        int least = 0, greatest = 0;
        HIP_TRY(hipDeviceGetStreamPriorityRange(&least, &greatest));
        for (auto& st : pool.s) HIP_TRY(hipStreamCreateWithPriority(&st, hipStreamNonBlocking, greatest));
    }
    m->pa_stream = pool.s[pool.next++ % m->side_pool];
    return GVX_OK;
}

namespace {

AttnPersistParams fill_attn_persist(const gvx_model* m, const DecoderBuffers& db, const float* memory, const int32_t* len_ws,
                                    unsigned* sync, int B, int L, int T) {
    const gvx_dims& d = m->d;
    const int E = d.embed_dim, D = d.dec_rnn_dim;
    AttnPersistParams pp{};
    pp.q_slab = db.q_slab;
    pp.v = m->dev_blob + m->blob.v; pp.pm = db.pm; pp.memory = memory; pp.lengths = len_ws;
    pp.loc_conv_t = m->dev_blob + m->blob.loc_conv; pp.loc_dense_t = m->dev_blob + m->blob.loc_dense;
    pp.w_out = db.align_tm; pp.w_out_bs = (long)L; pp.w_out_ts = (long)B * L;
    pp.ctx_base = db.hc + (size_t)B * (D + E) + (size_t)D * B; pp.ctx_ts = (long)B * (D + E);
    pp.sync = sync; pp.B = B; pp.L = L; pp.T = T; pp.kl = d.att_loc_kernel;
    pp.spin_limit = m->spin_limit;
    return pp;
}
void use_resident_flags(const gvx_model* m, AttnPersistParams& pp) {
    pp.q_flags = pp.sync + RS_FLAG_Q; pp.n_q_flags = pp.n_slabs;
    pp.ctx_flags = pp.sync + RS_FLAG_CTX;
    pp.debug = m->rs_debug;
}

int launch_resident_attention(gvx_model* m, const AttnPersistParams& pp, hipStream_t s) {
    HIP_TRY(hipEventRecord(m->pa_fork, s));
    HIP_TRY(hipStreamWaitEvent(m->pa_stream, m->pa_fork, 0));
    if (!m->debug_skip_resident) HIP_TRY(launch_attention_persistent(pp, m->pa_stream));
    HIP_TRY(hipEventRecord(m->pa_join, m->pa_stream));
    return GVX_OK;
}

template <class P>
void fill_resident_common(const gvx_model* m, const DecoderBuffers& db, unsigned* sync, int B, int T, P& rp) {
    const gvx_dims& d = m->d;
    rp.att_frag = m->dev_blob + m->blob.att_frag; rp.att_bias = m->dev_blob + m->blob.att_bias; rp.wq_t = m->dev_blob + m->blob.wq_t;
    rp.dec_frag = m->dev_blob + m->blob.dec_frag; rp.dec_bias = m->dev_blob + m->blob.dec_bias;
    rp.h_a = db.h_a; rp.hc = db.hc; rp.q_slab = db.q_slab; rp.c_a = db.c_a; rp.c_d = db.c_d;
    rp.sync = sync;
    rp.att_frag_bytes = (unsigned)(frag_floats(4 * d.att_rnn_dim, d.prenet_dim + d.embed_dim + d.att_rnn_dim) * sizeof(float));
    rp.B = B; rp.T = T; rp.spin_limit = m->spin_limit; rp.debug = m->rs_debug;
}

int ensure_ar_host_slots(gvx_model* m) {
    if (m->ar_done_host) return GVX_OK;
    HIP_TRY(hipHostMalloc(reinterpret_cast<void**>(&m->ar_done_host), 2 * sizeof(int32_t), hipHostMallocDefault));
    for (auto& e : m->ar_ev) HIP_TRY(hipEventCreateWithFlags(&e, hipEventDisableTiming));
    return GVX_OK;
}

}

int decoder_prenet_part(gvx_model* m, int B, int L, const float* mel_in, int T, const uint8_t* keep_masks, void* ws, const WsPlan& wp,
                        hipStream_t s) {
    const gvx_dims& d = m->d;
    const int M = d.n_mels, P = d.prenet_dim;
    const DecoderBuffers db = decoder_buffers(ws, wp);
    HIP_TRY(zero_async(db.frames, (size_t)B * M * sizeof(float), s));
    HIP_TRY(launch_frames_from_mel(mel_in, db.frames, B, M, T, s));
    const int rows = (T + 1) * B;
    GemmParams g{};
    g.A = db.frames; g.amap = RowMap{rows, 0, (long)M};
    g.W = m->dev_blob + m->blob.pre_w0; g.ldw = M;
    g.C = db.pre1; g.cmap = RowMap{rows, 0, (long)P};
    g.keep = keep_masks; g.keep_ld = P;
    g.M = rows; g.N = P; g.K = M; g.act = ACT_RELU;
    HIP_TRY(launch_gemm(g, s));
    g.A = db.pre1; g.amap = RowMap{rows, 0, (long)P};
    g.W = m->dev_blob + m->blob.pre_w1; g.ldw = P;
    g.C = db.prenet; g.cmap = RowMap{B, (long)B * P, 8}; g.c_nblk = (long)B * 8;
    g.keep = keep_masks + (size_t)rows * P;
    g.K = P;
    HIP_TRY(launch_gemm(g, s));
    if (plan_teacher_forced(m, B, L, TF_INFERENCE).pre_gate) {
        GemmParams h{};
        h.A = db.prenet; h.amap = RowMap{B, (long)B * P, 8}; h.a_kblk = (long)B * 8;
        h.W = m->dev_blob + m->blob.att_wpre; h.ldw = P;
        h.C = db.pre_gate; h.cmap = RowMap{T * B, 0, (long)4 * d.att_rnn_dim};
        h.M = T * B; h.N = 4 * d.att_rnn_dim; h.K = P; h.act = ACT_NONE;
        HIP_TRY(launch_gemm(h, s));
    }
    return GVX_OK;
}

int poison_if_timed_out(const gvx_model* m, int B, int L, void* ws, const WsPlan& wp, float* const* outs, const size_t* counts, int n,
                        hipStream_t s) {
    if (!plan_teacher_forced(m, B, L, TF_INFERENCE).timeout_check) return GVX_OK;
    HIP_TRY(launch_poison_on_timeout(ws_ptr<unsigned>(ws, wp.sync) + HANDOFF_TIMEOUT, ws_ptr<int>(ws, wp.flags) + FLAG_TIMEOUT, outs, counts, n, s));
    return GVX_OK;
}

namespace {

struct TfLoop {
    gvx_model* m; TfLoopPlan plan; DecoderBuffers db;
    const float* memory; const int32_t* len_ws; void* ws; unsigned* sync; float* xchg;
    int B, L, T;
    const LstmDropout* train;
};

void defer_context(const TfLoop& c, SkinnyJob& J, int t_ctx, bool first) {
    if (c.plan.kind == 0) return;
    const gvx_dims& d = c.m->d;
    J.defer_seg = 1;
    if (J.q_slab) {
        const int P = d.prenet_dim, E = d.embed_dim, A = d.att_rnn_dim;
        J.x[0] = XSeg{J.x[1].p, 0};
        J.kg0 = P / 8; J.nkg_w = (P + E + A) / 8; J.nkg = (E + A) / 8;
        J.addend = c.db.pre_gate + (size_t)(t_ctx + 1) * c.B * 4 * A; J.add_bs = 4 * A;
    }
    J.tmo = c.sync + HANDOFF_TIMEOUT;
    J.spin_limit = c.m->spin_limit;
    if (t_ctx >= 0) { J.ctx_cnt = c.sync + HANDOFF_CNT_CTX; J.ctx_target = (unsigned)c.B * (unsigned)(t_ctx + 1); }
    J.start_cnt = c.sync + HANDOFF_CNT_Q;
    if (first) { J.ready_cnt = c.sync + HANDOFF_READY; J.ready_target = (unsigned)attention_persistent_workgroups(c.B, c.L); }
}

void wire_tape(const LstmDropout& tr, SkinnyJob* att, SkinnyJob* dec, int t, size_t BA, size_t BD) {
    if (att) {
        att->h_keep = tr.att_keep + (size_t)t * BA; att->h_scale = tr.att_scale;
        if (tr.h_a_all) { att->x[2].p = tr.h_a_all + (size_t)t * BA; att->h_out = tr.h_a_all + (size_t)(t + 1) * BA; }
        if (tr.c_a_all) { att->c = tr.c_a_all + (size_t)t * BA; att->c_out = tr.c_a_all + (size_t)(t + 1) * BA; }
        if (tr.pre_a_all) att->pre_out = tr.pre_a_all + (size_t)t * 4 * BA;
    }
    if (dec) {
        if (tr.pre_d_all) dec->pre_out = tr.pre_d_all + (size_t)(t - 1) * 4 * BD;
        dec->h_keep = tr.dec_keep + (size_t)(t - 1) * BD; dec->h_scale = tr.dec_scale;
        if (tr.h_a_all) dec->x[0].p = tr.h_a_all + (size_t)t * BA;
        if (tr.c_d_all) { dec->c = tr.c_d_all + (size_t)(t - 1) * BD; dec->c_out = tr.c_d_all + (size_t)t * BD; }
    }
}

int tf_step_jobs(const TfLoop& c, int t, SkinnyJob* jobs) {
    const gvx_dims& d = c.m->d;
    SkinnyJob* att = t < c.T ? &jobs[0] : nullptr;
    SkinnyJob* dec = t > 0 ? &jobs[att ? 1 : 0] : nullptr;
    if (att) {
        fill_att_job(c.m, *att, c.db.prenet + (size_t)t * c.B * d.prenet_dim, t, c.B, c.db);
        defer_context(c, *att, t - 1, t == 0);
    }
    if (dec) {
        fill_dec_job(c.m, *dec, t - 1, c.B, c.db);
        defer_context(c, *dec, t - 1, false);
    }
    if (c.train) wire_tape(*c.train, att, dec, t, (size_t)c.B * d.att_rnn_dim, (size_t)c.B * d.dec_rnn_dim);
    return (att ? 1 : 0) + (dec ? 1 : 0);
}

int tf_step_jobs64(const TfLoop& c, int t, SkinnyJob* jobs) {
    const gvx_model* m = c.m;
    const gvx_dims& d = m->d;
    const int E = d.embed_dim, P = d.prenet_dim, A = d.att_rnn_dim, D = d.dec_rnn_dim, B = c.B, T = c.T;
    const DecoderBuffers& db = c.db;
    float* dec_part2[2] = {db.dec_part, db.dec_part + (size_t)B * 4 * D};
    int n = 0;
    if (t < T) {
        fill_att_job(m, jobs[n], db.prenet + (size_t)t * B * P, t, B, db);
        defer_context(c, jobs[n], t - 1, t == 0);
        ++n;
    }
    if (t >= 1 && t - 1 < T) {
        SkinnyJob& J = jobs[n];
        fill_dec_job(m, J, t - 1, B, db);
        J.x[2] = XSeg{nullptr, 0};
        J.nkg = (A + E) / 8; J.kg0 = 0; J.nkg_w = (A + E + D) / 8;
        J.mode = 2; J.bias = nullptr; J.c = nullptr; J.h_out = nullptr;
        J.y = dec_part2[t & 1];
        defer_context(c, J, t - 1, false);
        ++n;
    }
    if (t >= 2 && t - 2 < T) {
        SkinnyJob& J = jobs[n];
        std::memset(&J, 0, sizeof J);
        const float* hc_t = db.hc + (size_t)(t - 2) * B * (D + E);
        float* hc_n = db.hc + (size_t)(t - 1) * B * (D + E);
        J.Wp = m->dev_blob + m->blob.dec_frag; J.bias = m->dev_blob + m->blob.dec_bias;
        J.x[0] = XSeg{hc_t, D};
        J.N = 4 * D; J.nkg = D / 8; J.kg0 = (A + E) / 8; J.nkg_w = (A + E + D) / 8; J.mode = 0; J.B = B;
        J.c = db.c_d; J.h_out = hc_n;
        J.addend = dec_part2[(t - 1) & 1]; J.add_bs = 4 * D;
        J.start_cnt = c.sync + HANDOFF_CNT_Q;
        ++n;
    }
    return n;
}

template <class F>
int enqueue_or_replay(const TfLoop& c, int variant, hipStream_t s, F&& enqueue) {
    if (!c.plan.graph) return enqueue(s);
    const gvx_model::LoopKey key{c.ws, c.memory, c.m->dev_blob, c.B, c.L, c.T, c.len_ws != nullptr, 0.f, variant};
    return run_chunk(c.m, touch_graph_set(c.m, c.m->loop_graphs, key), 0, s, enqueue);
}

int tf_loop_resident(const TfLoop& c, hipStream_t s, int* launches) {
    gvx_model* m = c.m;
    const gvx_dims& d = m->d;
    DecResidentParams rp{};
    fill_resident_common(m, c.db, c.sync, c.B, c.T, rp);
    rp.pre_gate = c.db.pre_gate;
    rp.kg_pre = d.prenet_dim / 8;
    if (const LstmDropout* train = c.train) {
        rp.h_a = train->h_a_all;
        rp.tr_keep_a = train->att_keep; rp.tr_keep_d = train->dec_keep; rp.tr_scale_a = train->att_scale; rp.tr_scale_d = train->dec_scale;
        rp.tr_c_a = train->c_a_all; rp.tr_c_d = train->c_d_all; rp.tr_pre_a = train->pre_a_all; rp.tr_pre_d = train->pre_d_all;
    }
    rp.dec_frag_bytes = (unsigned)(frag_floats(4 * d.dec_rnn_dim, d.att_rnn_dim + d.embed_dim + d.dec_rnn_dim) * sizeof(float));
    rp.layout = c.plan.tile_layout;
    if (m->ktiming) HIP_TRY(hipEventRecord(m->kev[0], s));
    HIP_TRY(launch_decoder_resident(rp, s));
    if (m->ktiming) {
        HIP_TRY(hipEventRecord(m->kev[1], s));
        HIP_TRY(hipEventRecord(m->kev[2], s));
        m->n_lstm_ev = c.T; m->n_attn_ev = 0;
    }
    *launches = 1;
    return GVX_OK;
}

int tf_loop_beside_attention(const TfLoop& c, hipStream_t s, int* launches) {
    *launches = c.plan.rows64 ? c.T + 2 : c.T + 1;
    if (c.plan.rows64)
        return enqueue_or_replay(c, 48, s, [&](hipStream_t st) -> int {
            SkinnyJob jobs[3];
            for (int t = 0; t < c.T + 2; ++t) HIP_TRY(launch_skinny_pa64(jobs, tf_step_jobs64(c, t, jobs), st));
            return GVX_OK;
        });
    return enqueue_or_replay(c, c.m->pa_depth + 16 * c.plan.pa_layout, s, [&](hipStream_t st) -> int {
        SkinnyJob jobs[2];
        for (int t = 0; t < c.T; ++t) {
            tf_step_jobs(c, t, jobs);
            HIP_TRY(launch_skinny_pa(jobs[0], t > 0 ? &jobs[1] : nullptr, st, c.m->pa_depth, c.plan.pa_layout));
        }
        tf_step_jobs(c, c.T, jobs);
        HIP_TRY(launch_skinny(jobs, 1, SK_DECODER, st));
        return GVX_OK;
    });
}

int tf_loop_per_step(const TfLoop& c, hipStream_t s, int* launches) {
    const gvx_model* m = c.m;
    const gvx_dims& d = m->d;
    const int B = c.B, L = c.L, T = c.T;
    *launches = (m->attn_one_launch ? 2 : 3) * T + 1;
    return enqueue_or_replay(c, 0, s, [&](hipStream_t st) -> int {
        SkinnyJob jobs[2];
        for (int t = 0; t < T; ++t) {
            const int n = tf_step_jobs(c, t, jobs);
            LocJob lq;
            fill_loc(m, lq, t, B, L, c.db.align_tm, (long)L, (long)B * L, c.db);
            HIP_TRY(launch_skinny(jobs, n, SK_DECODER, st, &lq));
            AttnParams ap;
            fill_attn(m, ap, c.memory, c.len_ws, t, B, L, c.db.align_tm, (long)L, (long)B * L, c.db);
            if (m->attn_prefetch && m->attn_one_launch && B <= 32) {
                ap.pf_w[0] = m->dev_blob + m->blob.att_frag; ap.pf_w[1] = m->dev_blob + m->blob.dec_frag;
                ap.pf_nkg[0] = (d.prenet_dim + d.embed_dim + d.att_rnn_dim) / 8; ap.pf_nkg[1] = (d.att_rnn_dim + d.embed_dim + d.dec_rnn_dim) / 8;
                ap.pf_tiles0 = 4 * d.att_rnn_dim / 32; ap.pf_tiles = ap.pf_tiles0 + 4 * d.dec_rnn_dim / 32;
            }
            HIP_TRY(launch_attn(m, ap, st));
        }
        tf_step_jobs(c, T, jobs);
        HIP_TRY(launch_skinny(jobs, 1, SK_DECODER, st));
        return GVX_OK;
    });
}

int tf_time_step_launches(const TfLoop& c, hipStream_t s) {
    gvx_model* m = c.m;
    const int B = c.B, L = c.L, REPS = 64, tm = c.T > 1 ? c.T / 2 : 0;
    SkinnyJob jobs[3];
    fill_att_job(m, jobs[0], c.db.prenet + (size_t)tm * B * m->d.prenet_dim, tm, B, c.db);
    if (tm > 0) fill_dec_job(m, jobs[1], tm - 1, B, c.db);
    m->n_lstm_ev = REPS;
    m->n_attn_ev = 0;
    if (c.plan.kind == 0) {
        LocJob lq;
        fill_loc(m, lq, tm, B, L, c.db.align_tm, (long)L, (long)B * L, c.db);
        AttnParams ap;
        fill_attn(m, ap, c.memory, c.len_ws, tm, B, L, c.db.align_tm, (long)L, (long)B * L, c.db);
        ap.w_out = c.db.energies;
        ap.w_cum = c.db.energies;
        HIP_TRY(hipEventRecord(m->kev[0], s));
        for (int i = 0; i < REPS; ++i) HIP_TRY(launch_skinny(jobs, tm > 0 ? 2 : 1, SK_DECODER, s, &lq));
        HIP_TRY(hipEventRecord(m->kev[1], s));
        for (int i = 0; i < REPS; ++i) HIP_TRY(launch_attn(m, ap, s));
        HIP_TRY(hipEventRecord(m->kev[2], s));
        m->n_attn_ev = REPS;
        return GVX_OK;
    }
    HIP_TRY(hipStreamWaitEvent(s, m->pa_join, 0));
    int n = 0;
    if (c.plan.rows64) {
        n = tf_step_jobs64(c, tm > 2 ? tm : 2, jobs);
    } else {
        defer_context(c, jobs[0], tm - 1, false);
        if (tm > 0) defer_context(c, jobs[1], tm - 1, false);
        n = tm > 0 ? 2 : 1;
    }
    for (int i = 0; i < n; ++i) jobs[i].start_cnt = nullptr;
    HIP_TRY(hipEventRecord(m->kev[0], s));
    for (int i = 0; i < REPS; ++i)
        HIP_TRY(c.plan.rows64 ? launch_skinny_pa64(jobs, n, s) : launch_skinny_pa(jobs[0], tm > 0 ? &jobs[1] : nullptr, s, m->pa_depth, c.plan.pa_layout));
    HIP_TRY(hipEventRecord(m->kev[1], s));
    HIP_TRY(hipEventRecord(m->kev[2], s));
    return GVX_OK;
}

}

int decoder_tf_impl(gvx_model* m, const float* memory, const int32_t* lengths, int B, int L, const float* mel_in, int T,
                    const uint8_t* keep_masks, float* mel_out, float* gate_out, float* align_out, void* ws, const WsPlan& wp,
                    hipStream_t s, bool prenet_done, const LstmDropout* train) {
    const gvx_dims& d = m->d;
    const int E = d.embed_dim, M = d.n_mels, D = d.dec_rnn_dim;
    const DecoderBuffers db = decoder_buffers(ws, wp);
    unsigned* sync = ws_ptr<unsigned>(ws, wp.sync);
    HIP_TRY(zero_async(sync, HANDOFF_WORDS * sizeof(unsigned), s));
    const bool timed = m->timing && m->ev_valid;
    int rc = GVX_OK;
    if (!prenet_done) {
        rc = decoder_prenet_part(m, B, L, mel_in, T, keep_masks, ws, wp, s);
        if (rc != GVX_OK) return rc;
        rc = decoder_init_states(m, memory, B, L, db, s);
        if (rc != GVX_OK) return rc;
    }
    if (timed) HIP_TRY(hipEventRecord(m->ev[2], s));
    const int32_t* len_ws = nullptr;
    if (lengths) {
        HIP_TRY(hipMemcpyAsync(db.len_copy, lengths, (size_t)B * sizeof(int32_t), hipMemcpyDeviceToDevice, s));
        len_ws = db.len_copy;
    }
    if (m->ktiming) {
        rc = m->reserve_events(4);
        if (rc != GVX_OK) return rc;
        m->n_lstm_ev = m->n_attn_ev = 0;
    }
    const bool tape_whole = train && train->h_a_all && train->c_a_all && train->c_d_all && train->pre_a_all && train->pre_d_all;
    const TfLoopPlan plan = plan_teacher_forced(m, B, L, !train ? TF_INFERENCE : (tape_whole ? TF_TRAIN_WHOLE_TAPE : TF_TRAIN_PARTIAL_TAPE));
    const TfLoop c{m, plan, db, memory, len_ws, ws, sync, ws_ptr<float>(ws, wp.xchg), B, L, T, train};
    std::unique_lock<std::mutex> turn;
    if (plan.side_stream) {
        if (!prenet_done) {
            rc = ensure_side_stream(m);
            if (rc != GVX_OK) return rc;
        }
        turn = std::unique_lock<std::mutex>(g_turn_mutex);
        rc = turn_begin(s);
        if (rc != GVX_OK) return rc;
        AttnPersistParams pp = fill_attn_persist(m, db, memory, len_ws, sync, B, L, T);
        pp.n_slabs = attention_persistent_slabs(plan.tile_layout);
        pp.xchg = c.xchg;
        pp.q_first = 2;
        if (plan.kind == 2) use_resident_flags(m, pp);
        rc = launch_resident_attention(m, pp, s);
        if (rc != GVX_OK) return rc;
    }
    int launches = 0;
    switch (plan.kind) {
        case 2: rc = tf_loop_resident(c, s, &launches); break;
        case 1: rc = tf_loop_beside_attention(c, s, &launches); break;
        default: rc = tf_loop_per_step(c, s, &launches); break;
    }
    if (rc != GVX_OK) return rc;
    if (plan.side_stream) {
        HIP_TRY(hipStreamWaitEvent(s, m->pa_join, 0));
        ++launches;
        rc = turn_end(s);
        if (rc != GVX_OK) return rc;
        turn.unlock();
    }
    if (m->ktiming && plan.kind != 2) {
        rc = tf_time_step_launches(c, s);
        if (rc != GVX_OK) return rc;
    }
    HIP_TRY(launch_permute01(db.align_tm, align_out, T, B, L, s));
    m->last_decoder_launches = launches;
    if (timed) HIP_TRY(hipEventRecord(m->ev[3], s));
    {
        const int PS = m->PS();
        GemmParams g{};
        g.A = db.hc + (size_t)B * (D + E); g.amap = RowMap{B, (long)B * (D + E), 8}; g.a_kblk = (long)B * 8;
        g.W = m->dev_blob + m->blob.proj_w; g.ldw = D + E;
        g.C = db.proj; g.cmap = RowMap{B, (long)PS, (long)T * PS};
        g.bias = m->dev_blob + m->blob.proj_b;
        g.M = T * B; g.N = M + 1; g.K = D + E; g.act = ACT_NONE;
        HIP_TRY(launch_gemm(g, s));
        HIP_TRY(launch_split_projection(db.proj, mel_out, gate_out, B, M, T, s));
    }
    return GVX_OK;
}

namespace {

struct ArLoop {
    gvx_model* m; ArLoopPlan plan; DecoderBuffers db;
    const float* memory_ws; const int32_t* len_ws; const uint8_t* masks_ws; void* ws; unsigned* sync; float* xchg;
    int32_t* n_done; int32_t* n_frames_ws;
    int B, L, T;
    float gate_threshold;
    int32_t* centres; int win_back, win_ahead;
};

void print_ws_plan_once(const WsPlan& wp) {
    static bool printed = false;
    if (printed) return;
    printed = true;
#define GVX_PL(f) std::fprintf(stderr, "wsplan %s %zu\n", #f, wp.f);
    GVX_PL(xa) GVX_PL(xb) GVX_PL(xg) GVX_PL(enc_h) GVX_PL(enc_c) GVX_PL(flags) GVX_PL(sync) GVX_PL(memory) GVX_PL(pm) GVX_PL(frames) GVX_PL(pre1) GVX_PL(prenet) GVX_PL(h_a) GVX_PL(c_a) GVX_PL(c_d)
    GVX_PL(hc) GVX_PL(w_cum) GVX_PL(q_slab) GVX_PL(proj) GVX_PL(energies) GVX_PL(align_tm) GVX_PL(len_copy) GVX_PL(loc) GVX_PL(ar_masks)
    GVX_PL(p_slab) GVX_PL(p_ctx) GVX_PL(att_part) GVX_PL(dec_part) GVX_PL(pre_gate) GVX_PL(xchg) GVX_PL(ya) GVX_PL(yb) GVX_PL(total)
#undef GVX_PL
}

struct ArStep {
    const float* hc_t; float* hc_n; float* ctx_n; float* ha_new; float* att_part2; float* dec_part2;
    int kgP, kgE, kgA, kgD;
};
ArStep ar_step(const ArLoop& c, int t) {
    const gvx_dims& d = c.m->d;
    const int E = d.embed_dim, A = d.att_rnn_dim, D = d.dec_rnn_dim, B = c.B;
    ArStep q;
    q.hc_t = c.db.hc + (size_t)t * B * (D + E);
    q.hc_n = c.db.hc + (size_t)(t + 1) * B * (D + E);
    q.ctx_n = q.hc_n + (size_t)D * B;
    q.ha_new = c.db.h_a + (size_t)((t + 1) & 1) * B * A;
    q.att_part2 = c.db.att_part + (size_t)B * 4 * A;
    q.dec_part2 = c.db.dec_part + (size_t)B * 4 * D;
    q.kgP = d.prenet_dim / 8; q.kgE = E / 8; q.kgA = A / 8; q.kgD = D / 8;
    return q;
}

int ar_launch_a(const ArLoop& c, const ArStep& q, int t, hipStream_t st) {
    const gvx_model* m = c.m;
    const gvx_dims& d = m->d;
    const DecoderBuffers& db = c.db;
    const int P = d.prenet_dim, A = d.att_rnn_dim, D = d.dec_rnn_dim, B = c.B, L = c.L;
    const int kgP = q.kgP, kgE = q.kgE, kgA = q.kgA, kgD = q.kgD;
    SkinnyJob ja[2];
    std::memset(ja, 0, sizeof ja);
    {
        SkinnyJob& J = ja[0];
        J.Wp = m->dev_blob + m->blob.att_frag; J.bias = m->dev_blob + m->blob.att_bias;
        J.x[0] = XSeg{db.prenet, P};
        J.N = 4 * A; J.nkg = kgP; J.kg0 = 0; J.nkg_w = kgP + kgE + kgA; J.mode = 0; J.B = B;
        J.addend = db.att_part; J.add_bs = 4 * A; J.add_ts = 0;
        J.c = db.c_a; J.h_out = q.ha_new;
        J.Wq_t = m->dev_blob + m->blob.wq_t; J.q_slab = db.q_slab; J.att_dim = d.att_dim;
    }
    {
        SkinnyJob& J = ja[1];
        J.Wp = m->dev_blob + m->blob.dec_frag;
        J.x[0] = XSeg{q.hc_t, D};
        J.N = 4 * D; J.nkg = kgD; J.kg0 = kgA + kgE; J.nkg_w = kgA + kgE + kgD; J.mode = 2; J.B = B;
        J.y = db.dec_part;
    }
    if (c.plan.kind != 0) {
        if (t == 0) {
            ja[0].ready_cnt = c.sync + HANDOFF_READY; ja[0].ready_target = (unsigned)B;
            ja[0].tmo = c.sync + HANDOFF_TIMEOUT; ja[0].spin_limit = m->spin_limit;
        }
        HIP_TRY(launch_skinny(ja, 2, SK_AR, st));
        return GVX_OK;
    }
    LocJob lq;
    fill_loc(m, lq, t, B, L, db.align_tm, (long)L, (long)B * L, db);
    HIP_TRY(launch_skinny(ja, 2, SK_AR, st, &lq));
    AttnParams ap;
    fill_attn(m, ap, c.memory_ws, c.len_ws, t, B, L, db.align_tm, (long)L, (long)B * L, db);
    if (c.centres) {
        ap.c_prev = t > 0 ? c.centres + (t - 1) : nullptr; ap.c_out = c.centres + t; ap.c_bs = (long)c.T;
        ap.win_back = c.win_back; ap.win_ahead = c.win_ahead;
    }
    if (!c.plan.split_h) {
        HIP_TRY(launch_attn(m, ap, st));
        return GVX_OK;
    }
    SkinnyJob jb[2];
    std::memset(jb, 0, sizeof jb);
    {
        SkinnyJob& J = jb[0];
        J.Wp = m->dev_blob + m->blob.dec_frag;
        J.x[0] = XSeg{q.ha_new, A};
        J.N = 4 * D; J.nkg = kgA; J.kg0 = 0; J.nkg_w = kgA + kgE + kgD; J.mode = 2; J.B = B;
        J.y = q.dec_part2;
    }
    {
        SkinnyJob& J = jb[1];
        J.Wp = m->dev_blob + m->blob.att_frag;
        J.x[0] = XSeg{q.ha_new, A};
        J.N = 4 * A; J.nkg = kgA; J.kg0 = kgP + kgE; J.nkg_w = kgP + kgE + kgA; J.mode = 2; J.B = B;
        J.y = q.att_part2;
    }
    HIP_TRY(launch_skinny_attn(jb, 2, ap, st));
    return GVX_OK;
}

int ar_launch_cd(const ArLoop& c, const ArStep& q, int t, hipStream_t st) {
    const gvx_model* m = c.m;
    const gvx_dims& d = m->d;
    const DecoderBuffers& db = c.db;
    const int E = d.embed_dim, M = d.n_mels, P = d.prenet_dim, A = d.att_rnn_dim, D = d.dec_rnn_dim, B = c.B, T = c.T, PSB = m->PSB();
    const int kgP = q.kgP, kgE = q.kgE, kgA = q.kgA, kgD = q.kgD;
    const bool fold = c.plan.fold;
    SkinnyJob jc[3];
    std::memset(jc, 0, sizeof jc);
    {
        SkinnyJob& J = jc[0];
        J.Wp = m->dev_blob + m->blob.dec_frag; J.bias = m->dev_blob + m->blob.dec_bias;
        J.x[0] = XSeg{q.ha_new, A};
        J.x[1] = XSeg{q.ctx_n, E};
        J.N = 4 * D; J.nkg = kgA + kgE; J.kg0 = 0; J.nkg_w = kgA + kgE + kgD; J.mode = 0; J.B = B;
        J.addend = db.dec_part; J.add_bs = 4 * D; J.add_ts = 0;
        J.c = db.c_d; J.h_out = q.hc_n;
        J.Wq_t = m->dev_blob + m->blob.proj_hd_t; J.q_slab = db.p_slab; J.att_dim = PSB;
        if (fold) { J.xw = m->dev_blob + m->blob.proj_ctx_t; J.xsrc = q.ctx_n; }
    }
    {
        SkinnyJob& J = jc[1];
        J.Wp = m->dev_blob + m->blob.att_frag;
        J.x[0] = XSeg{q.ctx_n, 0};
        J.x[1] = XSeg{q.ctx_n, E};
        J.x[2] = XSeg{q.ha_new, A};
        J.N = 4 * A; J.nkg = kgE + kgA; J.kg0 = kgP; J.nkg_w = kgP + kgE + kgA; J.mode = 2; J.B = B;
        J.y = db.att_part;
    }
    if (c.plan.split_h) {
        SkinnyJob& Jd = jc[0];
        Jd.x[0] = XSeg{q.ctx_n, E}; Jd.x[1] = XSeg{nullptr, 0};
// ... 226 lines not shown
```

### genvox_amd/csrc/gvx_internal.h

```cpp
#pragma once
#include "../../include/genvox_amd.h"
#include "gvx_kernels.h"
#include "winograd_f45.h"

#include <cmath>
#include <cstdarg>
#include <cstdio>
#include <cstdlib>
#include <cstring>
#include <mutex>
#include <string>
#include <unordered_map>
#include <vector>

namespace gvx {

int fail(int code, const char* fmt, ...);

#define HIP_TRY(expr)                                                                          \
    do {                                                                                       \
        hipError_t _e = (expr);                                                                \
        if (_e != hipSuccess) return fail(GVX_ERR_HIP, "%s failed: %s", #expr, hipGetErrorString(_e)); \
    } while (0)

constexpr int MAX_CONV = 8;
constexpr double BN_EPS = 1e-5;

struct Blob {
    size_t emb;
    size_t enc_w[MAX_CONV], enc_b[MAX_CONV];
    size_t enc_wih, enc_bih, enc_whh_frag[2];
    size_t pre_w0, pre_w1, pre_w0_t, pre_w1_t;
    size_t att_frag, att_bias, att_wpre, wq_t, wmem, v, loc_conv, loc_dense;
    size_t dec_frag, dec_bias;
    size_t proj_w, proj_b, proj_frag, proj_hd_t, proj_ctx_frag, proj_ctx_t;
    size_t post_w[MAX_CONV], post_b[MAX_CONV];
    size_t post_u[MAX_CONV];
    size_t enc_u[MAX_CONV];
    size_t total;
};
inline bool winograd_shape_ok(int cin, int cout, int k) { return k == WINO_TAPS && cin == cout && cin % 32 == 0; }
inline bool postnet_layer_winograd_shape(const gvx_dims& d, int i) {
    return i > 0 && i < d.postnet_n_conv - 1 && winograd_shape_ok(d.postnet_dim, d.postnet_dim, d.postnet_kernel);
}
inline bool encoder_layer_winograd_shape(const gvx_dims& d, int i) {
    return i >= 0 && i < d.enc_n_conv && winograd_shape_ok(d.embed_dim, d.embed_dim, d.enc_kernel);
}
Blob make_blob_layout(const gvx_dims& d);

inline size_t frag_floats(int N, int K) { return (size_t)((N + 31) / 32) * (K / 8) * 64 * 4; }

struct WsPlan {
    size_t xa, xb, xg, enc_h, enc_c, flags, sync, memory;
    size_t pm, frames, pre1, prenet, h_a, c_a, c_d, hc, w_cum, q_slab, proj, energies, align_tm, len_copy, loc, ar_masks, p_slab, p_ctx;
    size_t att_part, dec_part, pre_gate, xchg;
    size_t ya, yb;
    size_t total;
};

}

struct gvx_model {
    gvx_dims d;
    gvx::Blob blob;
    const float* dev_blob = nullptr;
    bool use_graph = true;
    bool capture_first = false;
    bool attn_one_launch = true;
    bool attn_persistent = true;
    bool ar_resident = false;
    bool enc_persistent = true;
    bool ar_split_h = true;
    bool tf_rows64 = false;
    bool tf_resident = true;
    bool ar_resident_loop = true;
    bool tf_long_rows_224 = true;
    bool train_resident = true;
    bool train_resident_loop = true;
    bool attn_prefetch = true;
    int winograd = 1;
    int wino_group = 0;
    int enc_fork_after = 2;
    int pa_depth = 4;
    unsigned side_pool = 1;
    unsigned spin_limit = 0;
    int rs_debug = 0;
    bool debug_skip_resident = false;
    int debug_enc_skip_block = -1;
    bool debug_plan = false;
    bool timing = false;
    hipEvent_t ev[6] = {nullptr, nullptr, nullptr, nullptr, nullptr, nullptr};
    bool ev_valid = false;
    int last_decoder_launches = 0;
    struct LoopKey {
        const void* ws; const void* memory; const void* blob; int B, L, T; bool has_len;
        float threshold = 0.f;
        int variant = 0;
        const void* centres = nullptr; int win_back = 0, win_ahead = 0;
        bool operator==(const LoopKey& o) const {
            return ws == o.ws && memory == o.memory && blob == o.blob && B == o.B && L == o.L && T == o.T &&
                   has_len == o.has_len && threshold == o.threshold && variant == o.variant && centres == o.centres &&
                   win_back == o.win_back && win_ahead == o.win_ahead;
        }
    };
    struct GraphSet {
        LoopKey key;
        int sightings = 0;
        uint64_t last_use = 0;
        std::vector<hipGraphExec_t> execs;
    };
    static constexpr size_t GRAPH_SETS = 4;
    std::vector<GraphSet> ar_graphs, loop_graphs, enc_graphs;
    uint64_t use_clock = 0;
    uint64_t graph_replays = 0;
    hipStream_t pa_stream = nullptr;
    hipEvent_t pa_fork = nullptr, pa_join = nullptr, enc_mid = nullptr;
    int32_t* ar_done_host = nullptr;
    hipEvent_t ar_ev[2] = {nullptr, nullptr};
    std::vector<std::string> gather_names;
    std::vector<int64_t> gather_numel;
    int32_t* gather_off = nullptr;
    uint8_t* gather_tid = nullptr;
    void drop_graphs() {
        for (auto* c : {&ar_graphs, &loop_graphs, &enc_graphs}) {
            for (auto& gs : *c)
                for (auto e : gs.execs)
                    if (e) (void)hipGraphExecDestroy(e);
            c->clear();
        }
    }
    hipStream_t cap_stream = nullptr;
    bool ktiming = false;
    std::vector<hipEvent_t> kev;
    int n_lstm_ev = 0, n_attn_ev = 0;
    int reserve_events(size_t n) {
        while (kev.size() < n) {
            hipEvent_t e;
            if (hipEventCreate(&e) != hipSuccess) return GVX_ERR_HIP;
            kev.push_back(e);
        }
        return GVX_OK;
    }
    int H() const { return d.embed_dim / 2; }
    int PS() const { return (d.n_mels + 1 + 3) & ~3; }
    int PSB() const { return (d.n_mels + 1 + 7) & ~7; }
};

namespace gvx {

enum TfMode : int { TF_INFERENCE = 0, TF_TRAIN_WHOLE_TAPE = 1, TF_TRAIN_PARTIAL_TAPE = 2 };
struct TfLoopPlan {
    int kind;
    int pa_layout;
    int tile_layout;
    bool rows64;
    bool pre_gate;
    bool timeout_check;
    bool side_stream;
    bool graph;
};
struct ArLoopPlan {
    int kind;
    bool split_h;
    bool fold;
    bool graph;
};
TfLoopPlan plan_teacher_forced(const gvx_model* m, int B, int L, TfMode mode);
ArLoopPlan plan_autoregressive(const gvx_model* m, int B, int L, bool windowed = false);

enum WsMode : int { WS_TEACHER_FORCED = 0, WS_AUTOREGRESSIVE = 1 };

constexpr int WINOGRAD_MIN_CHANNELS = 256;
constexpr size_t WINOGRAD_GROUP_BYTES = (size_t)128 << 20;
bool conv_uses_winograd(const gvx_model* m, int cin, int cout, int k);
long winograd_group_tiles(long total, long fit, int C);
size_t winograd_scratch_floats(const gvx_model* m, int B, int T);

constexpr int FLAG_TOKEN = 0;
constexpr int FLAG_AR_DONE = 1;
constexpr int FLAG_TIMEOUT = 2;
constexpr int FLAG_AR_FRAMES = 64;

WsPlan make_ws_plan(const gvx_model* m, int B, int L, int T, int mode = WS_TEACHER_FORCED);
int check_common(const gvx_model* m, int B, int L, int T, void* ws, size_t ws_bytes, int mode = WS_TEACHER_FORCED);

template <typename T>
T* ws_ptr(void* ws, size_t off) { return reinterpret_cast<T*>(reinterpret_cast<char*>(ws) + off); }

inline hipError_t zero_async(void* p, size_t bytes, hipStream_t s) { return hipMemsetAsync(p, 0, bytes, s); }

gvx_model::GraphSet* touch_graph_set(gvx_model* m, std::vector<gvx_model::GraphSet>& cache, const gvx_model::LoopKey& key);
std::mutex& capture_mutex();

template <class F>
int run_chunk(gvx_model* m, gvx_model::GraphSet* gs, size_t chunk, hipStream_t s, F&& enqueue) {
    if (!m->use_graph || !gs || (gs->sightings < 2 && !m->capture_first)) return enqueue(s);
    if (gs->execs.size() <= chunk) gs->execs.resize(chunk + 1, nullptr);
    hipGraphExec_t exec = gs->execs[chunk];
    if (!exec) {
        std::lock_guard<std::mutex> lock(capture_mutex());
        hipGraph_t graph = nullptr;
        if (!m->cap_stream) HIP_TRY(hipStreamCreateWithFlags(&m->cap_stream, hipStreamNonBlocking));
        HIP_TRY(hipStreamBeginCapture(m->cap_stream, hipStreamCaptureModeThreadLocal));
        const int rc = enqueue(m->cap_stream);
        const hipError_t ce = hipStreamEndCapture(m->cap_stream, &graph);
        if (rc != GVX_OK) { if (graph) (void)hipGraphDestroy(graph); return rc; }
        HIP_TRY(ce);
        HIP_TRY(hipGraphInstantiate(&exec, graph, nullptr, nullptr, 0));
        HIP_TRY(hipGraphDestroy(graph));
        gs->execs[chunk] = exec;
    }
    HIP_TRY(hipGraphLaunch(exec, s));
    ++m->graph_replays;
    return GVX_OK;
}

struct DecoderBuffers {
    float *pm, *frames, *pre1, *prenet, *h_a, *c_a, *c_d, *hc, *w_cum, *q_slab, *proj, *energies, *align_tm, *loc, *p_slab, *p_ctx;
    float *att_part, *dec_part, *pre_gate;
    int32_t* len_copy;
};
DecoderBuffers decoder_buffers(void* ws, const WsPlan& wp);

struct LstmDropout {
    const uint8_t* att_keep; const uint8_t* dec_keep; float att_scale, dec_scale;
    float* h_a_all; float* c_a_all; float* c_d_all;
    float* pre_a_all; float* pre_d_all;
};

int ensure_side_stream(gvx_model* m);
int decoder_init_states(gvx_model* m, const float* memory, int B, int L, const DecoderBuffers& db, hipStream_t s);
int decoder_prenet_part(gvx_model* m, int B, int L, const float* mel_in, int T, const uint8_t* keep_masks, void* ws, const WsPlan& wp,
                        hipStream_t s);
int decoder_tf_impl(gvx_model* m, const float* memory, const int32_t* lengths, int B, int L, const float* mel_in, int T,
                    const uint8_t* keep_masks, float* mel_out, float* gate_out, float* align_out, void* ws, const WsPlan& wp,
                    hipStream_t s, bool prenet_done = false, const LstmDropout* train = nullptr);
int poison_if_timed_out(const gvx_model* m, int B, int L, void* ws, const WsPlan& wp, float* const* outs, const size_t* counts, int n,
                        hipStream_t s);

}
```

### genvox_amd/csrc/gvx_kernels.h

```cpp
#pragma once
#include <hip/hip_runtime.h>
#include <stddef.h>
#include <stdint.h>

#ifdef GVX_STAMPS
namespace gvx { namespace { __device__ unsigned long long gvx_stamps[3][32]; } }
#define GVX_STAMP(k, i)                                                                         \
    do {                                                                                        \
        if (blockIdx.x == 0 && blockIdx.y == 0 && threadIdx.x == 0) gvx::gvx_stamps[k][i] = wall_clock64(); \
    } while (0)
#else
#define GVX_STAMP(k, i) do { } while (0)
#endif

namespace gvx {

int set_error(int code, const char* msg);

inline size_t align_up(size_t x, size_t a) { return (x + a - 1) / a * a; }

enum Act : int { ACT_NONE = 0, ACT_RELU = 1, ACT_TANH = 2, ACT_GELU = 3 };

struct RowMap {
    int R;
    long s1, s0;
};

struct RowWalk { int grp, idx; long off; };
__host__ __device__ inline RowWalk row_walk_begin(const RowMap& m, int row) {
    RowWalk w;
    w.grp = row / m.R; w.idx = row - w.grp * m.R;
    w.off = (long)w.grp * m.s1 + (long)w.idx * m.s0;
    return w;
}
__host__ __device__ inline void row_walk_advance(RowWalk& w, const RowMap& m, int step) {
    w.idx += step; w.off += (long)step * m.s0;
    while (w.idx >= m.R) { w.idx -= m.R; ++w.grp; w.off += m.s1 - (long)m.R * m.s0; }
}
__host__ __device__ inline int mfma32_row_step(int q) { return (q & 3) ? 1 : 5; }

struct GemmParams {
    const float* A; RowMap amap; long a_kblk = 8;
    const float* W; long ldw;
    float* C; RowMap cmap; long c_nblk = 8;
    const float* bias;
    const uint8_t* keep; long keep_ld;
    int M, N, K;
    int act;
    int splitk = 1; int kchunk = 0; long c_split = 0;
    bool kmajor = false; RowMap wmap{1, 0, 0};
    int m_begin = 0;
    const int32_t* row_len = nullptr;
    int c_halo = 0;
    int slices = 1; long a_slice = 0, w_slice = 0, c_slice = 0;
    const float* res = nullptr;
};
hipError_t launch_gemm(const GemmParams& p, hipStream_t s);
struct GemmPlan { hipError_t err; int tile; int rows_big; };
GemmPlan plan_gemm(const GemmParams& p);
long gemm_round_rows(const GemmParams& p);
void set_splitk(GemmParams& p, int splitk);
hipError_t launch_gemm_splitk(const GemmParams& p, int splitk, float* scratch, hipStream_t s);

struct XSeg { const float* p; int len; };

struct SkinnyJob {
    const float* Wp;
    const float* bias;
    XSeg x[3];
    int N;
    int nkg;
    int kg0, nkg_w;
    int mode;
    float* c;
    float* h_out;
    const float* addend; long add_bs, add_ts;
    const float* addend2;
    const int32_t* lengths; int step; int reverse; int seq_len;
    float* seq_out; long seq_bs, seq_ts;
    const float* h_prev;
    const uint8_t* h_keep; float h_scale;
    float* c_out; float* c_seq_out;
    float* pre_out;
    const float* Wq_t;
    float* q_slab; int att_dim;
    const float* xw; const float* xsrc;
    int defer_seg;
    const unsigned* ctx_cnt; unsigned ctx_target;
    unsigned* start_cnt;
    const unsigned* ready_cnt; unsigned ready_target;
    unsigned* tmo;
    unsigned spin_limit;
    float* y;
    const uint8_t* keep; long keep_stride;
    int act;
    int B;
};
struct LocJob {
    const float* w_prev; long w_prev_bs;
    const float* w_cum;
    const float* loc_conv_t;
    const float* loc_dense_t;
    const float* pm;
    float* loc_out;
    int B, L, a, kl, G;
};
enum SkinnyKind : int { SK_DECODER = 0, SK_ENCODER = 1, SK_AR = 2, SK_TRAIN = 3 };
hipError_t launch_skinny(const SkinnyJob* jobs, int njobs, int kind, hipStream_t s, const LocJob* loc = nullptr);
struct AttnParams;
hipError_t launch_skinny_attn(const SkinnyJob* jobs, int njobs, const AttnParams& ap, hipStream_t s);
struct EncPersistParams {
    const float* Wp[2];
    const float* xg;
    const int32_t* lengths;
    float* hx;
    float* seq_out;
    float* c_seq_out;
    unsigned* sync;
    unsigned spin_limit;
    int B, L, H;
    int debug_skip_block;
};
bool encoder_persistent_supported(int B, int H);
hipError_t launch_encoder_persistent(const EncPersistParams& p, hipStream_t s);
hipError_t launch_skinny_pa(const SkinnyJob& att, const SkinnyJob* dec, hipStream_t s, int depth = 4, int layout = 1);
hipError_t launch_skinny_pa64(const SkinnyJob* jobs, int njobs, hipStream_t s);

struct AttnParams {
    const float* q_slab; int n_slabs;
    float* w_cum;
    const float* loc;
    const float* v;
    const float* pm;
    const float* memory;
    const int32_t* lengths;
    float* energies;
    float* w_out; long w_out_bs;
    float* ctx_out;
    int B, L, a, F, kl, E, G;
    const float* pf_w[2]; int pf_nkg[2]; int pf_tiles0, pf_tiles;
    const int32_t* c_prev; int32_t* c_out; long c_bs; int win_back, win_ahead;
};
hipError_t launch_attention(const AttnParams& p, hipStream_t s);
hipError_t launch_attention_step(const AttnParams& p, hipStream_t s);
int attention_slices(int B, int E);
int attention_groups(int B, int L);
bool attention_supported(int L, int a, int F, int kl, int E);

constexpr int HANDOFF_CNT_Q = 0, HANDOFF_CNT_CTX = 1024, HANDOFF_READY = 2048, HANDOFF_TIMEOUT = 3072;
constexpr int HANDOFF_STOP = 3072 + 512;
constexpr int HANDOFF_PAIR = 4096;
constexpr int HANDOFF_WORDS = 69632;
constexpr unsigned HANDOFF_SPIN_LIMIT = 200000u;
struct AttnPersistParams {
    const float* q_slab; int n_slabs;
    const float* v; const float* pm; const float* memory; const int32_t* lengths;
    const float* loc_conv_t; const float* loc_dense_t;
    float* w_out; long w_out_bs, w_out_ts;
    float* ctx_base; long ctx_ts;
    unsigned* sync;
    int B, L, T, kl;
    unsigned spin_limit;
    float* xchg;
    unsigned q_first;
    const unsigned* q_flags; int n_q_flags;
    unsigned* ctx_flags;
    int debug;
    const float* p_slab; int PSB, n_mels;
    const float* proj_b;
    float* proj_out;
    const float* pre_w0_t;
    const uint8_t* keep0;
    float* y1;
    int32_t* n_frames; int32_t* n_done; float gate_threshold;
    const unsigned* p_flags;
    unsigned* y1_flags;
    int32_t* centres; int win_back, win_ahead;
};
constexpr int RS_REP = 32;
constexpr int RS_FLAG_ATT = 8192;
constexpr int RS_FLAG_DEC = RS_FLAG_ATT + RS_REP * 128;
constexpr int RS_REP1 = 8;
constexpr int RS_FLAG_CTX = RS_FLAG_DEC + RS_REP * 128;
constexpr int RS_FLAG_Q = RS_FLAG_CTX + RS_REP1 * 32 * 32;
constexpr int RS_FLAG_Y1 = RS_FLAG_Q + RS_REP1 * 96 * 32;
constexpr int RS_REP_PRE = 8;
constexpr int RS_FLAG_PRE = RS_FLAG_Y1 + 32 * 32;
constexpr int RS_REP_P = 4;
constexpr int RS_FLAG_P = RS_FLAG_PRE + RS_REP_PRE * 8 * 32;
static_assert(RS_FLAG_P + RS_REP_P * 128 * 32 <= HANDOFF_WORDS, "flag replicas inside the hand-off block");
constexpr int RS_HA_SLOTS = 8;
struct DecResidentParams {
    const float* att_frag; const float* att_bias; const float* wq_t;
    const float* dec_frag; const float* dec_bias;
    const float* pre_gate;
    float* h_a;
    float* hc;
    float* q_slab;
    float* c_a; float* c_d;
    unsigned* sync;
    unsigned att_frag_bytes, dec_frag_bytes;
    int B, T;
    unsigned spin_limit;
    int debug;
    int kg_pre;
    int layout;
    const uint8_t* tr_keep_a; const uint8_t* tr_keep_d; float tr_scale_a, tr_scale_d;
    float* tr_c_a; float* tr_c_d; float* tr_pre_a; float* tr_pre_d;
};
struct ArResidentParams {
    const float* att_frag; const float* att_bias; const float* wq_t;
    const float* dec_frag; const float* dec_bias;
    const float* proj_hd_t;
    const float* proj_ctx_t;
    const float* pre_w1;
    const uint8_t* keep1;
    float* prenet;
    const float* y1;
    float* h_a; float* hc; float* q_slab;
    float* p_slab;
    float* c_a; float* c_d;
    const int32_t* n_done;
    unsigned* sync;
    unsigned att_frag_bytes;
    int B, T, PSB;
    unsigned spin_limit;
    int debug;
};
bool decoder_resident_supported(int B, int L);
hipError_t launch_decoder_ar_resident(const ArResidentParams& p, hipStream_t s);
hipError_t decoder_resident_init();
hipError_t launch_decoder_resident(const DecResidentParams& p, hipStream_t s);

bool attention_persistent_supported(int B, int L, int a, int F, int kl, int E, int att_rnn_dim, int dec_rnn_dim);
int attention_persistent_layout(int B, int L);
int attention_persistent_slabs(int layout);
int attention_persistent_workgroups(int B, int L);
size_t attention_persistent_xchg_floats(int B);
hipError_t attention_persistent_init();
hipError_t launch_attention_persistent(const AttnPersistParams& p, hipStream_t s);
hipError_t launch_handoff_set(unsigned* word, hipStream_t s);

#if defined(__HIPCC__)
typedef __attribute__((ext_vector_type(4))) unsigned gvx_u32x4;
__device__ __forceinline__ __amdgpu_buffer_rsrc_t make_rsrc(const void* p) {
    return __builtin_amdgcn_make_buffer_rsrc(const_cast<void*>(p), 0, 0x7fffffff, 0x00020000);
}
__device__ __forceinline__ float4 load_sc1(__amdgpu_buffer_rsrc_t r, unsigned byte_off) {
    const gvx_u32x4 v = __builtin_amdgcn_raw_buffer_load_b128(r, (int)byte_off, 0, 16);
    return make_float4(__uint_as_float(v.x), __uint_as_float(v.y), __uint_as_float(v.z), __uint_as_float(v.w));
}
__device__ __forceinline__ float load_sc1_f32(__amdgpu_buffer_rsrc_t r, unsigned byte_off) {
    return __uint_as_float(__builtin_amdgcn_raw_buffer_load_b32(r, (int)byte_off, 0, 16));
}
__device__ __forceinline__ void store_sc1(__amdgpu_buffer_rsrc_t r, unsigned byte_off, float4 v) {
    gvx_u32x4 u;
    u.x = __float_as_uint(v.x); u.y = __float_as_uint(v.y); u.z = __float_as_uint(v.z); u.w = __float_as_uint(v.w);
    __builtin_amdgcn_raw_buffer_store_b128(u, r, (int)byte_off, 0, 16);
}
template <bool FEW_WAITERS = false>
__device__ __forceinline__ bool handoff_wait(const unsigned* cnt, unsigned target, unsigned* tmo, unsigned code, unsigned limit = 0u,
                                             const unsigned* stop = nullptr) {
    if (limit == 0u) limit = HANDOFF_SPIN_LIMIT;
    unsigned spins = 0;
    while (__hip_atomic_load(cnt, __ATOMIC_RELAXED, __HIP_MEMORY_SCOPE_AGENT) < target) {
        ++spins;
        if ((spins & (FEW_WAITERS ? 127u : 7u)) == 1u) {
            if (__hip_atomic_load(tmo, __ATOMIC_RELAXED, __HIP_MEMORY_SCOPE_AGENT) != 0u) return false;
            if (stop && __hip_atomic_load(stop, __ATOMIC_RELAXED, __HIP_MEMORY_SCOPE_AGENT) != 0u) return false;
            if (spins > (FEW_WAITERS ? 16u : 1u) * limit) {
                __hip_atomic_store(tmo, code, __ATOMIC_RELAXED, __HIP_MEMORY_SCOPE_AGENT);
                return false;
            }
        }
        if (FEW_WAITERS || spins < 8u) __builtin_amdgcn_s_sleep(FEW_WAITERS ? 2 : 8);
        else __builtin_amdgcn_s_sleep(64);
    }
    return true;
}
#endif

hipError_t launch_embed(const int64_t* tokens, const float* emb, int n_tokens, float* x, float* x2, int B, int L, int E, int halo,
                        int* err_flag, hipStream_t s);
hipError_t launch_frames_from_mel(const float* mel_in, float* frames, int B, int M, int T, hipStream_t s);
hipError_t launch_split_projection(const float* proj, float* mel_out, float* gate_out, int B, int M, int T, hipStream_t s);
hipError_t launch_to_channels_last(const float* src, float* dst, int B, int M, int T, int halo, const int32_t* lens, hipStream_t s);
hipError_t launch_residual_to_channels_first(const float* mel, const float* y, float* mel_post, int B, int M, int T,
                                             const int32_t* lens, hipStream_t s);
hipError_t launch_zero_halo(float* buf, int B, int T, int halo, int C, hipStream_t s);
hipError_t launch_winograd_input(const float* x, float* V, int B, long mt0, long nmt, int T, int C, hipStream_t s);
hipError_t launch_winograd_output(const float* M, const float* bias, const int32_t* row_len, float* y, int B, long mt0, long nmt, int T, int C, int act, hipStream_t s);
hipError_t launch_mask_padding(float* mel, float* mel_post, float* gate, const int32_t* mel_lengths, int B, int M, int T,
                               hipStream_t s);
hipError_t launch_zero_many(void* const* ptrs, const size_t* bytes, int n_arrays, hipStream_t s);
hipError_t launch_poison_on_timeout(const unsigned* tmo, int* sticky, float* const* ptrs, const size_t* counts, int n_arrays, hipStream_t s);
hipError_t launch_permute01(const float* src, float* dst, int T, int B, int n, hipStream_t s);
size_t loss_scratch_bytes();
hipError_t launch_tacotron2_loss(const float* mel, const float* mel_post, const float* gate, const float* mel_t, const float* gate_t,
                                 long n_mel, long n_gate, double* scratch, float* out3, hipStream_t s);
hipError_t launch_mask_gen(uint8_t* out, size_t n, uint64_t seed, hipStream_t s);
hipError_t launch_ar_stop(const float* proj_t, int gate_col, float threshold, int t, int B,
                          int32_t* n_frames, int32_t* n_done, hipStream_t s);
hipError_t launch_ar_project(const float* p_slab, int n_slabs, const float* p_ctx, float* proj_t, int M, float threshold, int t, int B,
                             int32_t* n_frames, int32_t* n_done, const float* w0t, const float* w1t, int P, const uint8_t* keep0,
                             const uint8_t* keep1, float* prenet_out, hipStream_t s);
hipError_t launch_ar_centres_finish(int32_t* centres, const int32_t* n_frames, const unsigned* tmo, int B, int T, hipStream_t s);
hipError_t launch_ar_emit_all(const float* proj, float* mel_out, float* gate_out, int B, int M, int Tmax, int steps,
                              const int32_t* n_frames, hipStream_t s);
hipError_t launch_permute01_partial(const float* src, float* dst, int steps, int Tdst, int B, int n, const int32_t* n_frames,
                                    hipStream_t s);

}
```

### genvox_amd/csrc/misc.hip

```cpp
#include "gvx_kernels.h"

namespace gvx {

__global__ void embed_kernel(const int64_t* tokens, const float* emb, int n_tokens, float* x, float* x2, int B, int L, int E, int halo, int* err_flag) {
    const int row = blockIdx.x;
    if (row >= B * L) {
        const int k = row - B * L, b = k / (2 * halo), r = k - b * 2 * halo;
        const long at = ((long)b * (L + 2 * halo) + (r < halo ? r : L + r)) * E;
        const float4 z = make_float4(0.f, 0.f, 0.f, 0.f);
        for (int i = threadIdx.x; i < E / 4; i += blockDim.x) {
            reinterpret_cast<float4*>(x + at)[i] = z;
            if (x2) reinterpret_cast<float4*>(x2 + at)[i] = z;
        }
        return;
    }
    const int b = row / L, l = row - b * L;
    long tok = tokens[row];
    bool ok = tok >= 0 && tok < n_tokens;
    if (!ok && threadIdx.x == 0) atomicExch(err_flag, 1);
    const float4* src = reinterpret_cast<const float4*>(emb + (ok ? tok : 0) * E);
    float4* dst = reinterpret_cast<float4*>(x + ((long)b * (L + 2 * halo) + halo + l) * E);
    for (int i = threadIdx.x; i < E / 4; i += blockDim.x) dst[i] = ok ? src[i] : make_float4(0.f, 0.f, 0.f, 0.f);
}

// ... 31 lines not shown
            const long o = (long)b * p.db + (long)j * p.dj + i;
            const bool live = (p.len_axis ? j : i) < len;
            p.dst[o] = live ? (p.add ? v + p.add[o] : v) : 0.f;
        } else if (p.extra && j == p.extra_col) {
            p.extra[(long)b * p.extra_bs + i] = v;
        }
    }
    if (p.halo > 0 && blockIdx.x == 0 && blockIdx.y == 0) {
        const int tid = ty * 32 + tx, n = p.halo * p.ni;
        float* front = p.dst + (long)b * p.db - (long)p.halo * p.dj;
        float* back = p.dst + (long)b * p.db + (long)p.nj * p.dj;
        for (int e = tid; e < n; e += 256) {
            const int hr = e / p.ni, c = e - hr * p.ni;
            front[(long)hr * p.dj + c] = 0.f;
            back[(long)hr * p.dj + c] = 0.f;
        }
    }
}

static hipError_t launch_tr3(const Tr3& p, int B, hipStream_t s) {
    dim3 grid((p.nj + 31) / 32, (p.ni + 31) / 32, B);
    hipLaunchKernelGGL(transpose3_kernel, grid, dim3(32, 8), 0, s, p);
    return hipGetLastError();
}

hipError_t launch_frames_from_mel(const float* mel_in, float* frames, int B, int M, int T, hipStream_t s) {
    Tr3 p{};
    p.src = mel_in; p.sb = (long)M * T; p.si = T; p.ni = M; p.nj = T;
    p.dst = frames + (long)B * M; p.db = M; p.dj = (long)B * M;
    p.nj_main = T;
    return launch_tr3(p, B, s);
}

hipError_t launch_split_projection(const float* proj, float* mel_out, float* gate_out, int B, int M, int T, hipStream_t s) {
    const int PS = (M + 1 + 3) & ~3;
    Tr3 p{};
    p.src = proj; p.sb = (long)T * PS; p.si = PS; p.ni = T; p.nj = M + 1;
    p.dst = mel_out; p.db = (long)M * T; p.dj = T;
    p.nj_main = M; p.extra = gate_out; p.extra_bs = T; p.extra_col = M;
    return launch_tr3(p, B, s);
}

hipError_t launch_to_channels_last(const float* src, float* dst, int B, int M, int T, int halo, const int32_t* lens, hipStream_t s) {
    Tr3 p{};
    p.src = src; p.sb = (long)M * T; p.si = T; p.ni = M; p.nj = T;
    p.dst = dst + (long)halo * M; p.db = (long)(T + 2 * halo) * M; p.dj = M;
    p.nj_main = T;
    p.lens = lens; p.len_axis = 1; p.halo = halo;
    return launch_tr3(p, B, s);
}

hipError_t launch_residual_to_channels_first(const float* mel, const float* y, float* mel_post, int B, int M, int T,
                                             const int32_t* lens, hipStream_t s) {
    Tr3 p{};
    p.src = y; p.sb = (long)T * M; p.si = M; p.ni = T; p.nj = M;
    p.dst = mel_post; p.db = (long)M * T; p.dj = T; p.add = mel;
    p.nj_main = M;
    p.lens = lens; p.len_axis = 0;
    return launch_tr3(p, B, s);
}

__global__ void permute01_kernel(const float* src, float* dst, int T, int B, int n) {
    const long rows = (long)T * B;
    for (long r = blockIdx.x; r < rows; r += gridDim.x) {
        const int t = (int)(r / B), b = (int)(r - (long)t * B);
        const float* sp = src + r * n;
        float* dp = dst + ((long)b * T + t) * n;
        for (int i = threadIdx.x; i < n; i += blockDim.x) dp[i] = sp[i];
    }
}

hipError_t launch_permute01(const float* src, float* dst, int T, int B, int n, hipStream_t s) {
    const long rows = (long)T * B;
    const int grid = (int)(rows < 4096 ? rows : 4096);
    hipLaunchKernelGGL(permute01_kernel, dim3(grid), dim3(128), 0, s, src, dst, T, B, n);
    return hipGetLastError();
}

__global__ void zero_halo_kernel(float* buf, int T, int halo, int C) {
    const int b = blockIdx.x;
    float* base = buf + (long)b * (T + 2 * halo) * C;
    const int n = halo * C;
    for (int i = threadIdx.x; i < n; i += blockDim.x) {
        base[i] = 0.f;
        base[(long)(halo + T) * C + i] = 0.f;
    }
}

hipError_t launch_zero_halo(float* buf, int B, int T, int halo, int C, hipStream_t s) {
    if (halo <= 0) return hipSuccess;
    hipLaunchKernelGGL(zero_halo_kernel, dim3(B), dim3(256), 0, s, buf, T, halo, C);
    return hipGetLastError();
}

__global__ void mask_padding_kernel(float* mel, float* mel_post, float* gate, const int32_t* mel_lengths, int M, int T) {
    const int b = blockIdx.y;
    const int len = mel_lengths[b];
    const long n = (long)M * T;
    for (long i = (long)blockIdx.x * blockDim.x + threadIdx.x; i < n; i += (long)gridDim.x * blockDim.x) {
        const int t = (int)(i % T);
        if (t >= len) {
            if (mel) mel[(long)b * n + i] = 0.f;
            if (mel_post) mel_post[(long)b * n + i] = 0.f;
            if (gate && i < T) gate[(long)b * T + t] = 1e3f;
        }
    }
}

hipError_t launch_mask_padding(float* mel, float* mel_post, float* gate, const int32_t* mel_lengths, int B, int M, int T,
                               hipStream_t s) {
    const long n = (long)M * T;
    int gx = (int)((n + 255) / 256);
    if (gx > 64) gx = 64;
    hipLaunchKernelGGL(mask_padding_kernel, dim3(gx, B), dim3(256), 0, s, mel, mel_post, gate, mel_lengths, M, T);
    return hipGetLastError();
}

struct ZeroArgs { uint32_t* p[8]; size_t n[8]; };
__global__ void zero_many_kernel(ZeroArgs a) {
    uint32_t* p = a.p[blockIdx.y];
    const size_t n = a.n[blockIdx.y];
    for (size_t k = (size_t)blockIdx.x * blockDim.x + threadIdx.x; k < n; k += (size_t)gridDim.x * blockDim.x) p[k] = 0u;
}
hipError_t launch_zero_many(void* const* ptrs, const size_t* bytes, int n_arrays, hipStream_t s) {
    if (n_arrays < 1 || n_arrays > 8) return hipErrorInvalidValue;
    ZeroArgs a{};
    size_t most = 0;
    for (int i = 0; i < n_arrays; ++i) {
        if ((reinterpret_cast<uintptr_t>(ptrs[i]) & 3) || (bytes[i] & 3)) return hipErrorInvalidValue;
        a.p[i] = reinterpret_cast<uint32_t*>(ptrs[i]); a.n[i] = bytes[i] / 4;
        if (a.n[i] > most) most = a.n[i];
    }
    int gx = (int)((most + 1023) / 1024);
    if (gx < 1) gx = 1;
    if (gx > 64) gx = 64;
    hipLaunchKernelGGL(zero_many_kernel, dim3(gx, n_arrays), dim3(256), 0, s, a);
    return hipGetLastError();
}

struct PoisonArgs { float* p[4]; size_t n[4]; };
__global__ void poison_on_timeout_kernel(const unsigned* tmo, int* sticky, PoisonArgs a) {
    const unsigned code = __hip_atomic_load(tmo, __ATOMIC_RELAXED, __HIP_MEMORY_SCOPE_AGENT);
    if (code == 0u) return;
    if (blockIdx.x == 0 && threadIdx.x == 0) *sticky = (int)code;
    const float nan = __int_as_float(0x7fc00000);
#pragma unroll
    for (int i = 0; i < 4; ++i)
        for (size_t k = (size_t)blockIdx.x * blockDim.x + threadIdx.x; k < a.n[i]; k += (size_t)gridDim.x * blockDim.x) a.p[i][k] = nan;
}
hipError_t launch_poison_on_timeout(const unsigned* tmo, int* sticky, float* const* ptrs, const size_t* counts, int n_arrays, hipStream_t s) {
    PoisonArgs a{};
    for (int i = 0; i < 4; ++i) { a.p[i] = i < n_arrays ? ptrs[i] : nullptr; a.n[i] = i < n_arrays && ptrs[i] ? counts[i] : 0; }
    hipLaunchKernelGGL(poison_on_timeout_kernel, dim3(64), dim3(256), 0, s, tmo, sticky, a);
    return hipGetLastError();
}

__device__ __forceinline__ uint64_t splitmix64(uint64_t x) {
    x += 0x9E3779B97F4A7C15ull;
    x = (x ^ (x >> 30)) * 0xBF58476D1CE4E5B9ull;
    x = (x ^ (x >> 27)) * 0x94D049BB133111EBull;
    return x ^ (x >> 31);
}

__global__ void mask_gen_kernel(uint8_t* out, size_t n, uint64_t seed) {
    const size_t words = (n + 7) / 8;
    for (size_t w = (size_t)blockIdx.x * blockDim.x + threadIdx.x; w < words; w += (size_t)gridDim.x * blockDim.x) {
        const uint64_t bits = splitmix64(splitmix64(seed) ^ (w >> 3));
        const unsigned byte = (unsigned)(bits >> (8 * (w & 7))) & 0xFFu;
        uint64_t v = 0;
#pragma unroll
        for (int i = 0; i < 8; ++i) v |= (uint64_t)((byte >> i) & 1u) << (8 * i);
        if (8 * w + 8 <= n) {
            reinterpret_cast<uint64_t*>(out)[w] = v;
        } else {
            for (size_t i = 8 * w; i < n; ++i) out[i] = (uint8_t)((v >> (8 * (i - 8 * w))) & 1u);
        }
    }
}

hipError_t launch_mask_gen(uint8_t* out, size_t n, uint64_t seed, hipStream_t s) {
    if (n == 0) return hipSuccess;
    if (reinterpret_cast<uintptr_t>(out) & 7) return hipErrorInvalidValue;
    const size_t words = (n + 7) / 8;
    int grid = (int)((words + 255) / 256);
    if (grid > 2048) grid = 2048;
    hipLaunchKernelGGL(mask_gen_kernel, dim3(grid), dim3(256), 0, s, out, n, seed);
    return hipGetLastError();
}

__global__ void ar_stop_kernel(const float* proj_t, int gate_col, float threshold, int t, int B, int32_t* n_frames, int32_t* n_done) {
    const int b = blockIdx.x * blockDim.x + threadIdx.x;
    if (b >= B) return;
    if (n_frames[b] != 0) return;
    const float g = proj_t[(long)(gate_col >> 3) * B * 8 + b * 8 + (gate_col & 7)];
    const float sg = 1.f / (1.f + expf(-g));
    if (sg > threshold) {
        n_frames[b] = t + 1;
        atomicAdd(n_done, 1);
    }
}

hipError_t launch_ar_stop(const float* proj_t, int gate_col, float threshold, int t, int B, int32_t* n_frames, int32_t* n_done,
                          hipStream_t s) {
    hipLaunchKernelGGL(ar_stop_kernel, dim3((B + 63) / 64), dim3(64), 0, s, proj_t, gate_col, threshold, t, B, n_frames, n_done);
    return hipGetLastError();
}

constexpr int ARP_KQ = 4;
__global__ __launch_bounds__(256) void ar_project_kernel(const float* __restrict__ p_slab, int n_slabs, const float* __restrict__ p_ctx,
                                                         float* __restrict__ proj_t, int M, int PSB, float threshold, int t, int B,
                                                         int32_t* n_frames, int32_t* n_done, const float* __restrict__ w0t,
                                                         const float* __restrict__ w1t, int P, const uint8_t* __restrict__ keep0,
                                                         const uint8_t* __restrict__ keep1, float* __restrict__ prenet_out) {
    extern __shared__ float arp_smem[];
    __shared__ float part[2][128];
    __shared__ float mel[128];
    float* h1 = arp_smem;
    float* red = arp_smem + P;
    const int sl = blockIdx.x, S = gridDim.x, b = blockIdx.y, tid = threadIdx.x;
    const int half = tid / PSB, n = tid - half * PSB;
    if (half < 2 && n <= M) {
        const int s_begin = half == 0 ? 0 : n_slabs / 2, s_end = half == 0 ? n_slabs / 2 : n_slabs;
        const float* sp = p_slab + (long)b * PSB + n;
        const long sstride = (long)B * PSB;
        float acc = 0.f;
        int q0 = s_begin;
        for (; q0 + 16 <= s_end; q0 += 16) {
            float v[16];
#pragma unroll
            for (int q = 0; q < 16; ++q) v[q] = sp[(long)(q0 + q) * sstride];
#pragma unroll
            for (int q = 0; q < 16; ++q) acc += v[q];
        }
        for (; q0 < s_end; ++q0) acc += sp[(long)q0 * sstride];
        part[half][n] = acc;
    }
    __syncthreads();
    if (half == 0 && n <= M) {
        const long blocked = (long)(n >> 3) * B * 8 + b * 8 + (n & 7);
        const float v = (part[0][n] + part[1][n]) + p_ctx[blocked];
        if (n < M) mel[n] = v;
        if (sl == 0) {
            proj_t[blocked] = v;
            if (n == M && n_frames[b] == 0) {
                const float sg = 1.f / (1.f + expf(-v));
                if (sg > threshold) {
                    n_frames[b] = t + 1;
                    atomicAdd(n_done, 1);
                }
            }
        }
    }
    if (!keep0) return;
    __syncthreads();
    for (int j = tid; j < P; j += 256) {
        float acc = 0.f;
        for (int k = 0; k < M; ++k) acc = fmaf(w0t[(long)k * P + j], mel[k], acc);
        acc = fmaxf(acc, 0.f);
        h1[j] = keep0[(long)b * P + j] ? 2.f * acc : 0.f;
    }
    __syncthreads();
    const int OS = (P + S - 1) / S, o_begin = sl * OS, o_cnt = min(OS, P - o_begin);
    if (o_cnt <= 0) return;
    const int KC = (P + ARP_KQ - 1) / ARP_KQ;
    for (int idx = tid; idx < o_cnt * ARP_KQ; idx += 256) {
        const int kq = idx / o_cnt, ol = idx - kq * o_cnt;
        const int k_end = min(P, (kq + 1) * KC);
        const float* wcol = w1t + o_begin + ol;
        float acc = 0.f;
        for (int k = kq * KC; k < k_end; ++k) acc = fmaf(wcol[(long)k * P], h1[k], acc);
        red[kq * OS + ol] = acc;
    }
    __syncthreads();
    for (int ol = tid; ol < o_cnt; ol += 256) {
        float acc = red[ol];
#pragma unroll
        for (int kq = 1; kq < ARP_KQ; ++kq) acc += red[kq * OS + ol];
        const int o = o_begin + ol;
        acc = fmaxf(acc, 0.f);
        acc = keep1[(long)b * P + o] ? 2.f * acc : 0.f;
        prenet_out[(long)(o >> 3) * B * 8 + b * 8 + (o & 7)] = acc;
    }
}

constexpr int ARP_THREADS = 1024;
template <int KPT>
__global__ __launch_bounds__(ARP_THREADS) void ar_project_fast_kernel(const float* __restrict__ p_slab, int n_slabs,
                                                                      const float* __restrict__ p_ctx, float* __restrict__ proj_t, int M,
                                                                      int PSB, float threshold, int t, int B, int32_t* n_frames,
                                                                      int32_t* n_done, const float* __restrict__ w0t,
                                                                      const float* __restrict__ w1t, int P,
                                                                      const uint8_t* __restrict__ keep0, const uint8_t* __restrict__ keep1,
                                                                      float* __restrict__ prenet_out) {
    __shared__ float4 sp4[32][32];
    __shared__ float4 l1p[16][64];
    __shared__ float4 l2p[64][16];
    __shared__ float4 l2q[16][16];
    __shared__ __attribute__((aligned(16))) float mel[128];
    __shared__ __attribute__((aligned(16))) float h1[256];
    const int sl = blockIdx.x, S = gridDim.x, b = blockIdx.y;
    const unsigned tid = threadIdx.x;
    const bool more = keep0 != nullptr;
    const unsigned n4c = (unsigned)PSB >> 2;
    const unsigned sg = tid / n4c, n4 = tid - sg * n4c;
    const bool slab_thread = sg < 32;
    float4 sv[4];
// ... 248 lines not shown
```

### include/genvox_amd.h

```cpp
#ifndef GENVOX_AMD_H
#define GENVOX_AMD_H

#include <stddef.h>
#include <stdint.h>

#ifdef __cplusplus
extern "C" {
#endif

typedef enum gvx_status {
    GVX_OK = 0,
    GVX_ERR_INVALID_ARG = -1,
    GVX_ERR_UNSUPPORTED = -2,
    GVX_ERR_MISSING_WEIGHT = -3,
    GVX_ERR_SHAPE = -4,
    GVX_ERR_WORKSPACE = -5,
    GVX_ERR_HIP = -6,
    GVX_ERR_STATE = -7
} gvx_status;

typedef struct gvx_dims {
    int32_t n_tokens;
    int32_t embed_dim;
    int32_t enc_kernel;
    int32_t enc_n_conv;
    int32_t prenet_dim;
    int32_t att_rnn_dim;
    int32_t dec_rnn_dim;
    int32_t att_dim;
    int32_t att_loc_filters;
    int32_t att_loc_kernel;
    int32_t postnet_dim;
    int32_t postnet_kernel;
    int32_t postnet_n_conv;
    int32_t n_mels;
} gvx_dims;

typedef struct gvx_weight_desc {
    const char* name;
    const float* data;
    int64_t numel;
} gvx_weight_desc;

typedef struct gvx_model gvx_model;

#define GVX_WORKSPACE_CLEAR_BYTES 12804

const char* gvx_last_error(void);
int gvx_version(void);

int gvx_model_create(const gvx_dims* dims, gvx_model** out);
void gvx_model_destroy(gvx_model* model);
size_t gvx_model_blob_bytes(const gvx_model* model);
int gvx_model_pack_weights(gvx_model* model, const gvx_weight_desc* table, int n, void* host_blob);
int gvx_model_bind_blob(gvx_model* model, const void* device_blob);
int gvx_model_pack_weights_device(gvx_model* model, const gvx_weight_desc* table, int n, void* device_blob, void* stream);

size_t gvx_workspace_bytes(const gvx_model* model, int B, int L, int T);
size_t gvx_workspace_bytes_autoregressive(const gvx_model* model, int B, int L, int max_steps);

int gvx_workspace_status(const gvx_model* model, void* workspace, size_t workspace_bytes, void* stream, int32_t* host_out);

int gvx_model_set_persistent_attention(gvx_model* model, int enable);

int gvx_model_set_resident_kernels(gvx_model* model, int enable);

int gvx_model_set_winograd(gvx_model* model, int mode);
int gvx_debug_conv_plan(const gvx_model* model, int cin, int cout, int k);

int gvx_teacher_forced_rows_per_call(const gvx_model* model, int L);

int gvx_teacher_forced_resident(const gvx_model* model, int B, int L);

int gvx_teacher_forced_loop_kind(const gvx_model* model, int B, int L);

int gvx_autoregressive_loop_kind(const gvx_model* model, int B, int L);
int gvx_autoregressive_windowed_loop_kind(const gvx_model* model, int B, int L);

int gvx_encoder_forward(gvx_model* model, const int64_t* tokens, const int32_t* lengths, int B, int L,
                        float* memory_out, void* workspace, size_t workspace_bytes, void* stream);

int gvx_decoder_teacher_forced(gvx_model* model, const float* memory, const int32_t* lengths, int B, int L,
                               const float* mel_in, int T, const uint8_t* keep_masks,
                               float* mel_out, float* gate_out, float* align_out,
                               void* workspace, size_t workspace_bytes, void* stream);

int gvx_decoder_autoregressive(gvx_model* model, const float* memory, const int32_t* lengths, int B, int L,
                               int max_steps, float gate_threshold, const uint8_t* keep_masks,
                               float* mel_out, float* gate_out, float* align_out, int32_t* n_frames_out,
                               int* steps_run_out, void* workspace, size_t workspace_bytes, void* stream);

int gvx_decoder_autoregressive_windowed(gvx_model* model, const float* memory, const int32_t* lengths, int B, int L,
                                        int max_steps, float gate_threshold, const uint8_t* keep_masks,
                                        float* mel_out, float* gate_out, float* align_out, int32_t* n_frames_out,
                                        int* steps_run_out, void* workspace, size_t workspace_bytes, void* stream,
                                        int window_back, int window_ahead, int32_t* centres_out);

size_t gvx_postnet_workspace_bytes(const gvx_model* model, int B, int T);
int gvx_postnet_forward(gvx_model* model, const float* mel_in, const int32_t* mel_lengths, int B, int T, float* mel_post_out,
                        void* workspace, size_t workspace_bytes, void* stream);

int gvx_mask_padding(float* mel, float* mel_post, float* gate, const int32_t* mel_lengths,
                     int B, int n_mels, int T, void* stream);

int gvx_tacotron2_forward(gvx_model* model, const int64_t* tokens, const int32_t* token_lengths, int B, int L,
                          const float* mel_in, const int32_t* mel_lengths, int T, const uint8_t* keep_masks,
                          float* mel_out, float* mel_post_out, float* gate_out, float* align_out,
                          void* workspace, size_t workspace_bytes, void* stream);

int gvx_tacotron2_loss(const float* mel_out, const float* mel_post_out, const float* gate_out, const float* mel_target,
                       const float* gate_target, int B, int n_mels, int T, float* loss_out, void* scratch, size_t scratch_bytes,
                       void* stream);

int gvx_encoder_lstm_forward(gvx_model* model, const float* conv_out, const int32_t* lengths, int B, int L, float* memory_out,
                             float* cell_states_out, float* input_preact_out, void* workspace, size_t workspace_bytes, void* stream);
int gvx_decoder_teacher_forced_train(gvx_model* model, const float* memory, const int32_t* lengths, int B, int L, const float* mel_in,
                                     int T, const uint8_t* keep_masks, const uint8_t* att_keep, const uint8_t* dec_keep, float p_att,
                                     float p_dec, float* mel_out, float* gate_out, float* align_out, float* att_hidden_all,
                                     float* att_cell_all, float* dec_cell_all, float* dec_hidden_context_all, float* att_preact_all,
                                     float* dec_preact_all, void* workspace, size_t workspace_bytes, void* stream);
int gvx_train_export(const gvx_model* model, const void* workspace, size_t workspace_bytes, int B, int L, int T, int what, float* dst, void* stream);
size_t gvx_conv_train_saved_bytes(int B, int Cin, int Cout, int T, int k);
size_t gvx_conv_train_workspace_bytes(int B, int Cin, int Cout, int T, int k);
int gvx_conv_bn_act_train_forward(const float* x, const float* w, const float* bias, const float* gamma, const float* beta,
                                  float* running_mean, float* running_var, int B, int Cin, int Cout, int T, int k, int act,
                                  const uint8_t* keep, float p_drop, float* y, void* saved, size_t saved_bytes, void* workspace,
                                  size_t workspace_bytes, void* stream);
int gvx_conv_bn_act_train_backward(const float* dy, const void* saved, size_t saved_bytes, const float* w, const float* gamma,
                                   const float* x_wgrad, int B, int Cin, int Cout, int T, int k, int act, const uint8_t* keep,
                                   float p_drop, float* dx, float* dw, float* dbias, float* dgamma, float* dbeta, void* workspace,
                                   size_t workspace_bytes, void* stream);
int gvx_tacotron2_loss_backward(const float* mel_out, const float* mel_post_out, const float* gate_out, const float* mel_target,
                                const float* gate_target, int B, int n_mels, int T, float* dmel_out, float* dmel_post_out,
                                float* dgate_out, void* stream);

int gvx_train_gemm_nt(const float* A, long lda, const float* W, long ldw, float* C, long ldc, int M, int N, int K, const float* bias,
                      float* scratch, size_t scratch_bytes, void* stream);
int gvx_train_gemm_tn(const float* A, long lda, const float* Bm, long ldb, float* C, long ldc, int M, int N, long rows, float* scratch,
                      size_t scratch_bytes, void* stream);
int gvx_train_transpose(const float* src, long ld_src, float* dst, long rows, int cols, long rows_padded, void* stream);
int gvx_train_colsum(const float* X, long rows, int C, float* out, void* stream);
int gvx_train_axpby(const float* a, long lda, float alpha, const float* b, long ldb, float beta, float* y, long ldy, long rows, int cols, void* stream);
int gvx_train_relu_dropout_backward(const float* dy, const float* act_out, const uint8_t* keep, float scale, long n, float* dz, void* stream);
int gvx_train_unblock(const float* blocked, float* rows_out, long n_slots, int B, int K, void* stream);
int gvx_train_embedding_backward(const int64_t* tokens, const float* dx, long n_tokens_in_batch, int E, int n_rows, float* demb, void* stream);
typedef struct gvx_tensor_ref { const float* data; int64_t numel; } gvx_tensor_ref;
typedef struct gvx_adam_ref { float* param; const float* grad; float* exp_avg; float* exp_avg_sq; int64_t numel; } gvx_adam_ref;
size_t gvx_train_sqnorm_scratch_bytes(int n_tensors);
int gvx_train_sqnorm_many(const gvx_tensor_ref* refs_device, int n_tensors, double* scratch, double* sumsq_out, void* stream);
int gvx_train_adam_step_many(const gvx_adam_ref* refs_device, int n_tensors, float grad_scale, float lr, float weight_decay, float beta1,
                             float beta2, float eps, int step, void* stream);

typedef struct gvx_bptt_decoder_args {
    int32_t B, L, T;
    int32_t A, D, E, P, a, F, kl;
    float att_scale, dec_scale;
    const float* dhc_all;
    const float* pre_a;
    const float* pre_d;
    const float* c_a_all;
    const float* c_d_all;
    const uint8_t* att_keep;
    const uint8_t* dec_keep;
    const float* q_all;
    const float* ctx_all;
    int64_t ctx_ts, ctx_bs;
    const float* w_all;
    const float* memory;
    const float* pm;
    const float* w_ih_a; const float* w_hh_a;
    const float* w_ih_d; const float* w_hh_d;
    const float* wq;
    const float* v;
    const float* loc_conv;
    const float* loc_dense;
    float* dga_all;
    float* dgd_all;
    float* dq_all;
    float* dctx_all;
    float* dpm;
    float* dmemory;
    float* dv;
    float* dloc_dense;
    float* dloc_conv;
} gvx_bptt_decoder_args;
size_t gvx_train_decoder_bptt_workspace_bytes(const gvx_bptt_decoder_args* args);
int gvx_train_decoder_bptt(const gvx_bptt_decoder_args* args, void* workspace, size_t workspace_bytes, void* stream);
int gvx_train_decoder_bptt_ext(const gvx_bptt_decoder_args* args, const float* dw_ext, int64_t dw_ext_ts, int64_t dw_ext_bs,
                               void* workspace, size_t workspace_bytes, void* stream);
size_t gvx_guided_attention_loss_scratch_bytes(int B, int T, int L);
int gvx_guided_attention_loss(const float* align, const int32_t* token_lengths, const int32_t* mel_lengths, int B, int T, int L,
                              float sigma, float alpha, float* loss_out, float* dalign, void* scratch, size_t scratch_bytes,
                              void* stream);
size_t gvx_train_encoder_lstm_bptt_workspace_bytes(int B, int H);
int gvx_train_encoder_lstm_bptt(const float* xg, const float* memory, const float* cell_states, const float* dmemory, const float* w_hh,
                                const int32_t* lengths, int B, int L, int H, float* dg_pos, float* hprev_pos, void* workspace,
                                size_t workspace_bytes, void* stream);
int gvx_train_encoder_lstm_bptt_resident(const float* xg, const float* memory, const float* cell_states, const float* dmemory,
                                         const float* w_hh, const int32_t* lengths, int B, int L, int H, float* dg_pos,
                                         float* hprev_pos, void* workspace, size_t workspace_bytes, void* stream);
int gvx_train_encoder_lstm_bptt_status(const void* workspace, size_t workspace_bytes, int B, int H, int* code_out, void* stream);

int gvx_prenet_masks_generate(uint8_t* masks_out, size_t n, uint64_t seed, void* stream);

int gvx_stage_timing_enable(gvx_model* model, int enable);
int gvx_stage_times_ms(gvx_model* model, float* times5_out, int* decoder_launches_out);

typedef struct gvx_gl_plan gvx_gl_plan;
int gvx_gl_plan_create(int n_fft, int hop, gvx_gl_plan** out);
void gvx_gl_plan_destroy(gvx_gl_plan* plan);
size_t gvx_gl_workspace_bytes(gvx_gl_plan* plan, int B, int T, int n_mels);

int gvx_stft(gvx_gl_plan* plan, const float* signal, const float* window, int B, long n_samples, float* spec_out,
             void* workspace, size_t workspace_bytes, void* stream);
int gvx_istft(gvx_gl_plan* plan, const float* spec, const float* window, int B, int T, float* signal_out,
              void* workspace, size_t workspace_bytes, void* stream);
int gvx_mel_to_magnitude(gvx_gl_plan* plan, const float* mel_db, const float* inv_basis, int B, int n_mels, int T, int log10_kind,
                         float ref, float* mag_out, void* workspace, size_t workspace_bytes, void* stream);
// ... 495 lines not shown
```

Baseline: 2.042 million.

## Add fused prenet kernel, fold encoder tail setup, move alignment permute to side stream

Adds an opt-in MFMA kernel that fuses frame extraction and both prenet layers into one launch. It is off by default via GVX_PRENET_FUSED. Separately, the resident encoder path now folds the length copy, decoder state zeroing and handoff clearing into its setup and tail kernels. The alignment permute is moved onto the side stream. Together these aim to cut small launches and serialization on the main stream, at the cost of more coupling between encoder and decoder setup.

```diff
diff --git a/genvox_amd/_lib.py b/genvox_amd/_lib.py
--- a/genvox_amd/_lib.py
+++ b/genvox_amd/_lib.py
@@ -368,6 +368,7 @@
     "gvx_model_set_persistent_attention": (_i, [_vp, _i]),
     "gvx_model_set_resident_kernels": (_i, [_vp, _i]),
     "gvx_model_set_winograd": (_i, [_vp, _i]),
+    "gvx_model_set_prenet_fused": (_i, [_vp, _i]),
     "gvx_debug_conv_plan": (_i, [_vp, _i, _i, _i]),
     "gvx_teacher_forced_rows_per_call": (_i, [_vp, _i]),
     "gvx_teacher_forced_resident": (_i, [_vp, _i, _i]),
diff --git a/genvox_amd/build.py b/genvox_amd/build.py
--- a/genvox_amd/build.py
+++ b/genvox_amd/build.py
@@ -9,7 +9,7 @@
 HERE = os.path.dirname(os.path.abspath(__file__))
 CSRC = os.path.join(HERE, "csrc")
 LIB = os.path.join(HERE, "libgenvox_amd.so")
-SOURCES = ["gemm_f32.hip", "winograd_conv.hip", "skinny.hip", "dec_resident.hip", "attention.hip", "attn_persist.hip", "misc.hip", "griffinlim.hip", "wav_finalize.hip", "wav_to_mel.hip", "resample.hip", "eval_metrics.hip", "mas.hip", "time_warp.hip", "melgan.hip", "melgan_train.hip", "melgan_disc.hip", "hifigan.hip", "hifigan_train.hip", "hifigan_disc.hip", "hifigan_msd.hip", "mrd.hip", "bigvgan.hip", "vocos.hip", "univnet.hip", "fastpitch.hip", "pitch.hip", "psola.hip", "stft_loss.hip", "mel_loss.hip", "denoise.hip",
+SOURCES = ["gemm_f32.hip", "winograd_conv.hip", "skinny.hip", "dec_resident.hip", "attention.hip", "attn_persist.hip", "misc.hip", "prenet_fused.hip", "griffinlim.hip", "wav_finalize.hip", "wav_to_mel.hip", "resample.hip", "eval_metrics.hip", "mas.hip", "time_warp.hip", "melgan.hip", "melgan_train.hip", "melgan_disc.hip", "hifigan.hip", "hifigan_train.hip", "hifigan_disc.hip", "hifigan_msd.hip", "mrd.hip", "bigvgan.hip", "vocos.hip", "univnet.hip", "fastpitch.hip", "pitch.hip", "psola.hip", "stft_loss.hip", "mel_loss.hip", "denoise.hip",
            "train_conv.hip", "train_ops.hip", "train_bptt_decoder.hip", "train_bptt_encoder.hip", "train_guided.hip", "gvx_pack.hip", "gvx_decoder.hip", "gvx_api.hip"]
 ARCH = "gfx950"
 HIPCC = os.environ.get("HIPCC", "/opt/rocm/bin/hipcc")
diff --git a/genvox_amd/csrc/gvx_api.hip b/genvox_amd/csrc/gvx_api.hip
--- a/genvox_amd/csrc/gvx_api.hip
+++ b/genvox_amd/csrc/gvx_api.hip
@@ -185,6 +185,7 @@
     m->ar_split_h = flag("GVX_AR_SPLIT_H", true);
     m->enc_persistent = flag("GVX_ENC_PERSISTENT", true);
     m->enc_fork_after = number("GVX_ENC_FORK_AFTER", 2);
+    m->prenet_fused = flag("GVX_PRENET_FUSED", false);
     m->train_resident = flag("GVX_TRAIN_RESIDENT", true);
     m->train_resident_loop = flag("GVX_TRAIN_RESIDENT_LOOP", true);
     m->tf_rows64 = flag("GVX_TF_ROWS64", false);
@@ -254,6 +255,7 @@
     HIP_TRY(attention_init());
     HIP_TRY(attention_persistent_init());
     HIP_TRY(decoder_resident_init());
+    HIP_TRY(prenet_fused_init());
     return GVX_OK;
 }
 
@@ -316,9 +318,11 @@
     return front >= back ? WinoScratch{wp.xg, front / sizeof(float)} : WinoScratch{wp.h_a, back / sizeof(float)};
 }
 
+struct EncoderFold { bool states_and_handoff = false; };
 int encoder_impl(gvx_model* m, const int64_t* tokens, const int32_t* lengths, int B, int L, float* memory_out, void* ws,
                  const WsPlan& wp, const WinoScratch& wsc, hipStream_t s, const float* conv_out = nullptr, float* c_seq_out = nullptr,
-                 float* xg_out = nullptr, hipEvent_t dense_done = nullptr) {
+                 float* xg_out = nullptr, hipEvent_t dense_done = nullptr,
+                 EncoderFold* fold = nullptr) {
     const gvx_dims& d = m->d;
     const int E = d.embed_dim, H = E / 2, pe = (d.enc_kernel - 1) / 2;
     float* xa = ws_ptr<float>(ws, wp.xa);
@@ -359,9 +363,10 @@
     float* mem_ws = ws_ptr<float>(ws, wp.memory);
     if (!resident) HIP_TRY(zero_async(mem_ws, (size_t)B * L * E * sizeof(float), s));
     const int32_t* len_ws = nullptr;
+    const bool folded = fold && resident;
     if (lengths) {
         int32_t* lc = ws_ptr<int32_t>(ws, wp.len_copy);
-        HIP_TRY(hipMemcpyAsync(lc, lengths, (size_t)B * sizeof(int32_t), hipMemcpyDeviceToDevice, s));
+        if (!folded) HIP_TRY(hipMemcpyAsync(lc, lengths, (size_t)B * sizeof(int32_t), hipMemcpyDeviceToDevice, s));
         len_ws = lc;
     }
     auto enqueue = [&](hipStream_t st) -> int {
@@ -390,8 +395,10 @@
     if (resident) {
         unsigned* sync = ws_ptr<unsigned>(ws, wp.sync);
         void* const zp[2] = {enc_h, sync + HANDOFF_TIMEOUT};
-        const size_t zb[2] = {(size_t)4 * B * H * sizeof(float), sizeof(unsigned)};
-        HIP_TRY(launch_zero_many(zp, zb, 2, s));
+        static_assert(HANDOFF_TICKET == HANDOFF_TIMEOUT + 1, "the time-out word and the ticket counter are cleared as one range");
+        const size_t zb[2] = {(size_t)4 * B * H * sizeof(float), (folded ? 2 : 1) * sizeof(unsigned)};
+        if (folded) HIP_TRY(launch_encoder_setup(zp, zb, 2, lengths, ws_ptr<int32_t>(ws, wp.len_copy), lengths ? B : 0, s));
+        else HIP_TRY(launch_zero_many(zp, zb, 2, s));
         EncPersistParams ep{};
         ep.Wp[0] = m->dev_blob + m->blob.enc_whh_frag[0]; ep.Wp[1] = m->dev_blob + m->blob.enc_whh_frag[1];
         ep.xg = xg; ep.lengths = len_ws; ep.hx = enc_h; ep.seq_out = mem_ws; ep.c_seq_out = c_seq_out;
@@ -400,7 +407,18 @@
         HIP_TRY(launch_encoder_persistent(ep, s));
         float* outs[2] = {mem_ws, c_seq_out};
         const size_t counts[2] = {(size_t)B * L * E, (size_t)B * L * E};
-        HIP_TRY(launch_poison_on_timeout(sync + HANDOFF_TIMEOUT, flags + FLAG_TIMEOUT, outs, counts, c_seq_out ? 2 : 1, s));
+        if (folded) {
+            void* zero[7];
+            size_t zero_bytes[7];
+            int n = decoder_zero_states_list(m, B, L, decoder_buffers(ws, wp), zero, zero_bytes);
+            zero[n] = sync; zero_bytes[n++] = (size_t)HANDOFF_TIMEOUT * sizeof(unsigned);
+            zero[n] = sync + HANDOFF_TICKET + 1; zero_bytes[n++] = (size_t)(HANDOFF_WORDS - HANDOFF_TICKET - 1) * sizeof(unsigned);
+            HIP_TRY(launch_encoder_tail(sync + HANDOFF_TIMEOUT, sync + HANDOFF_TICKET, flags + FLAG_TIMEOUT, outs, counts, c_seq_out ? 2 : 1,
+                                        zero, zero_bytes, n, s));
+            fold->states_and_handoff = true;
+        } else {
+            HIP_TRY(launch_poison_on_timeout(sync + HANDOFF_TIMEOUT, flags + FLAG_TIMEOUT, outs, counts, c_seq_out ? 2 : 1, s));
+        }
     } else {
         const gvx_model::LoopKey key{ws, mem_ws, m->dev_blob, B, L, 0, lengths != nullptr};
         const int rc = run_chunk(m, m->use_graph && !c_seq_out ? touch_graph_set(m, m->enc_graphs, key) : nullptr, 0, s, enqueue);
@@ -524,6 +542,17 @@
     return GVX_OK;
 }
 
+int gvx_model_set_prenet_fused(gvx_model* m, int enable) {
+    if (!m) return fail(GVX_ERR_INVALID_ARG, "null argument");
+    m->prenet_fused = enable != 0;
+    return GVX_OK;
+}
+
+int gvx_debug_prenet_fused(const gvx_model* m, int B, int T) {
+    if (!m || B < 1 || T < 1) return -1;
+    return prenet_takes_fused_kernel(m) ? 1 : 0;
+}
+
 int gvx_model_set_winograd(gvx_model* m, int mode) {
     if (!m) return fail(GVX_ERR_INVALID_ARG, "null argument");
     if (mode < 0 || mode > 2) return fail(GVX_ERR_INVALID_ARG, "winograd mode must be 0, 1 or 2 (got %d)", mode);
@@ -661,7 +690,7 @@
     if (att_cell_all) HIP_TRY(zero_async(att_cell_all, (size_t)B * A * sizeof(float), s));
     if (dec_cell_all) HIP_TRY(zero_async(dec_cell_all, (size_t)B * D * sizeof(float), s));
     const WsPlan wp = make_ws_plan(m, B, L, T);
-    rc = decoder_tf_impl(m, memory, lengths, B, L, mel_in, T, keep_masks, mel_out, gate_out, align_out, ws, wp, s, false, &tr);
+    rc = decoder_tf_impl(m, memory, lengths, B, L, mel_in, T, keep_masks, mel_out, gate_out, align_out, ws, wp, s, TfSetupDone{}, &tr);
     if (rc != GVX_OK) return rc;
     {
         float* outs[3] = {mel_out, gate_out, align_out};
@@ -733,14 +762,21 @@
     float* memory = ws_ptr<float>(ws, wp.memory);
     if (timed) HIP_TRY(hipEventRecord(m->ev[0], s));
     const bool overlap = plan_teacher_forced(m, B, L, TF_INFERENCE).side_stream;
+    TfSetupDone done;
     if (overlap) {
         rc = ensure_side_stream(m);
         if (rc != GVX_OK) return rc;
         HIP_TRY(hipEventRecord(m->pa_fork, s));
         HIP_TRY(hipStreamWaitEvent(m->pa_stream, m->pa_fork, 0));
-        rc = encoder_impl(m, tokens, token_lengths, B, L, memory, ws, wp, encoder_wino_scratch(wp, false), m->pa_stream, nullptr, nullptr, nullptr, m->enc_mid);
+        EncoderFold fold;
+        rc = encoder_impl(m, tokens, token_lengths, B, L, memory, ws, wp, encoder_wino_scratch(wp, false), m->pa_stream, nullptr, nullptr, nullptr, m->enc_mid,
+                          &fold);
         if (rc != GVX_OK) return rc;
-        rc = decoder_init_states(m, memory, B, L, decoder_buffers(ws, wp), m->pa_stream);
+        done.prenet = true;
+        done.lengths = true;
+        if (!fold.states_and_handoff) HIP_TRY(zero_async(ws_ptr<unsigned>(ws, wp.sync), HANDOFF_WORDS * sizeof(unsigned), m->pa_stream));
+        done.handoff = true;
+        rc = decoder_init_states(m, memory, B, L, decoder_buffers(ws, wp), m->pa_stream, fold.states_and_handoff);
         if (rc != GVX_OK) return rc;
         HIP_TRY(hipEventRecord(m->pa_join, m->pa_stream));
         HIP_TRY(hipStreamWaitEvent(s, m->enc_mid, 0));
@@ -752,7 +788,7 @@
         if (rc != GVX_OK) return rc;
     }
     if (timed) HIP_TRY(hipEventRecord(m->ev[1], s));
-    rc = decoder_tf_impl(m, memory, token_lengths, B, L, mel_in, T, keep_masks, mel_out, gate_out, align_out, ws, wp, s, overlap);
+    rc = decoder_tf_impl(m, memory, token_lengths, B, L, mel_in, T, keep_masks, mel_out, gate_out, align_out, ws, wp, s, done);
     if (rc != GVX_OK) return rc;
     if (timed) HIP_TRY(hipEventRecord(m->ev[4], s));
     if (mel_post_out) {
diff --git a/genvox_amd/csrc/gvx_decoder.hip b/genvox_amd/csrc/gvx_decoder.hip
--- a/genvox_amd/csrc/gvx_decoder.hip
+++ b/genvox_amd/csrc/gvx_decoder.hip
@@ -58,13 +58,25 @@
     return b;
 }
 
-int decoder_init_states(gvx_model* m, const float* memory, int B, int L, const DecoderBuffers& db, hipStream_t s) {
+int decoder_zero_states_list(const gvx_model* m, int B, int L, const DecoderBuffers& db, void** zp, size_t* zb) {
     const gvx_dims& d = m->d;
     const int E = d.embed_dim, A = d.att_rnn_dim, D = d.dec_rnn_dim;
-    void* const zp[5] = {db.h_a, db.c_a, db.c_d, db.hc , db.w_cum};
-    const size_t zb[5] = {(size_t)RS_HA_SLOTS * B * A * sizeof(float), (size_t)B * A * sizeof(float), (size_t)B * D * sizeof(float),
-                          (size_t)B * (D + E) * sizeof(float), (size_t)B * L * sizeof(float)};
-    HIP_TRY(launch_zero_many(zp, zb, 5, s));
+    void* const p[5] = {db.h_a, db.c_a, db.c_d, db.hc , db.w_cum};
+    const size_t b[5] = {(size_t)RS_HA_SLOTS * B * A * sizeof(float), (size_t)B * A * sizeof(float), (size_t)B * D * sizeof(float),
+                         (size_t)B * (D + E) * sizeof(float), (size_t)B * L * sizeof(float)};
+    for (int i = 0; i < 5; ++i) { zp[i] = p[i]; zb[i] = b[i]; }
+    return 5;
+}
+
+int decoder_init_states(gvx_model* m, const float* memory, int B, int L, const DecoderBuffers& db, hipStream_t s, bool states_zeroed) {
+    const gvx_dims& d = m->d;
+    const int E = d.embed_dim;
+    if (!states_zeroed) {
+        void* zp[5];
+        size_t zb[5];
+        const int n = decoder_zero_states_list(m, B, L, db, zp, zb);
+        HIP_TRY(launch_zero_many(zp, zb, n, s));
+    }
     GemmParams g{};
     g.A = memory; g.amap = RowMap{B * L, 0, (long)E};
     g.W = m->dev_blob + m->blob.wmem; g.ldw = E;
@@ -234,27 +246,38 @@
 
 }
 
+bool prenet_takes_fused_kernel(const gvx_model* m) { return m->prenet_fused && prenet_fused_supported(m->d.n_mels, m->d.prenet_dim); }
+
 int decoder_prenet_part(gvx_model* m, int B, int L, const float* mel_in, int T, const uint8_t* keep_masks, void* ws, const WsPlan& wp,
                         hipStream_t s) {
     const gvx_dims& d = m->d;
     const int M = d.n_mels, P = d.prenet_dim;
     const DecoderBuffers db = decoder_buffers(ws, wp);
-    HIP_TRY(zero_async(db.frames, (size_t)B * M * sizeof(float), s));
-    HIP_TRY(launch_frames_from_mel(mel_in, db.frames, B, M, T, s));
     const int rows = (T + 1) * B;
-    GemmParams g{};
-    g.A = db.frames; g.amap = RowMap{rows, 0, (long)M};
-    g.W = m->dev_blob + m->blob.pre_w0; g.ldw = M;
-    g.C = db.pre1; g.cmap = RowMap{rows, 0, (long)P};
-    g.keep = keep_masks; g.keep_ld = P;
-    g.M = rows; g.N = P; g.K = M; g.act = ACT_RELU;
-    HIP_TRY(launch_gemm(g, s));
-    g.A = db.pre1; g.amap = RowMap{rows, 0, (long)P};
-    g.W = m->dev_blob + m->blob.pre_w1; g.ldw = P;
-    g.C = db.prenet; g.cmap = RowMap{B, (long)B * P, 8}; g.c_nblk = (long)B * 8;
-    g.keep = keep_masks + (size_t)rows * P;
-    g.K = P;
-    HIP_TRY(launch_gemm(g, s));
+    if (prenet_takes_fused_kernel(m)) {
+        PrenetFusedParams pf{};
+        pf.mel_in = mel_in; pf.w0 = m->dev_blob + m->blob.pre_w0; pf.w1 = m->dev_blob + m->blob.pre_w1;
+        pf.keep0 = keep_masks; pf.keep1 = keep_masks + (size_t)rows * P;
+        pf.frames = db.frames; pf.pre1 = db.pre1; pf.prenet = db.prenet;
+        pf.B = B; pf.T = T; pf.M = M; pf.P = P;
+        HIP_TRY(launch_prenet_fused(pf, s));
+    } else {
+        HIP_TRY(zero_async(db.frames, (size_t)B * M * sizeof(float), s));
+        HIP_TRY(launch_frames_from_mel(mel_in, db.frames, B, M, T, s));
+        GemmParams g{};
+        g.A = db.frames; g.amap = RowMap{rows, 0, (long)M};
+        g.W = m->dev_blob + m->blob.pre_w0; g.ldw = M;
+        g.C = db.pre1; g.cmap = RowMap{rows, 0, (long)P};
+        g.keep = keep_masks; g.keep_ld = P;
+        g.M = rows; g.N = P; g.K = M; g.act = ACT_RELU;
+        HIP_TRY(launch_gemm(g, s));
+        g.A = db.pre1; g.amap = RowMap{rows, 0, (long)P};
+        g.W = m->dev_blob + m->blob.pre_w1; g.ldw = P;
+        g.C = db.prenet; g.cmap = RowMap{B, (long)B * P, 8}; g.c_nblk = (long)B * 8;
+        g.keep = keep_masks + (size_t)rows * P;
+        g.K = P;
+        HIP_TRY(launch_gemm(g, s));
+    }
     if (plan_teacher_forced(m, B, L, TF_INFERENCE).pre_gate) {
         GemmParams h{};
         h.A = db.prenet; h.amap = RowMap{B, (long)B * P, 8}; h.a_kblk = (long)B * 8;
@@ -492,15 +515,15 @@
 
 int decoder_tf_impl(gvx_model* m, const float* memory, const int32_t* lengths, int B, int L, const float* mel_in, int T,
                     const uint8_t* keep_masks, float* mel_out, float* gate_out, float* align_out, void* ws, const WsPlan& wp,
-                    hipStream_t s, bool prenet_done, const LstmDropout* train) {
+                    hipStream_t s, TfSetupDone done, const LstmDropout* train) {
     const gvx_dims& d = m->d;
     const int E = d.embed_dim, M = d.n_mels, D = d.dec_rnn_dim;
     const DecoderBuffers db = decoder_buffers(ws, wp);
     unsigned* sync = ws_ptr<unsigned>(ws, wp.sync);
-    HIP_TRY(zero_async(sync, HANDOFF_WORDS * sizeof(unsigned), s));
+    if (!done.handoff) HIP_TRY(zero_async(sync, HANDOFF_WORDS * sizeof(unsigned), s));
     const bool timed = m->timing && m->ev_valid;
     int rc = GVX_OK;
-    if (!prenet_done) {
+    if (!done.prenet) {
         rc = decoder_prenet_part(m, B, L, mel_in, T, keep_masks, ws, wp, s);
         if (rc != GVX_OK) return rc;
         rc = decoder_init_states(m, memory, B, L, db, s);
@@ -509,7 +532,7 @@
     if (timed) HIP_TRY(hipEventRecord(m->ev[2], s));
     const int32_t* len_ws = nullptr;
     if (lengths) {
-        HIP_TRY(hipMemcpyAsync(db.len_copy, lengths, (size_t)B * sizeof(int32_t), hipMemcpyDeviceToDevice, s));
+        if (!done.lengths) HIP_TRY(hipMemcpyAsync(db.len_copy, lengths, (size_t)B * sizeof(int32_t), hipMemcpyDeviceToDevice, s));
         len_ws = db.len_copy;
     }
     if (m->ktiming) {
@@ -522,7 +545,7 @@
     const TfLoop c{m, plan, db, memory, len_ws, ws, sync, ws_ptr<float>(ws, wp.xchg), B, L, T, train};
     std::unique_lock<std::mutex> turn;
     if (plan.side_stream) {
-        if (!prenet_done) {
+        if (!done.prenet) {
             rc = ensure_side_stream(m);
             if (rc != GVX_OK) return rc;
         }
@@ -536,6 +559,8 @@
         if (plan.kind == 2) use_resident_flags(m, pp);
         rc = launch_resident_attention(m, pp, s);
         if (rc != GVX_OK) return rc;
+        HIP_TRY(launch_permute01(db.align_tm, align_out, T, B, L, m->pa_stream));
+        HIP_TRY(hipEventRecord(m->pa_join, m->pa_stream));
     }
     int launches = 0;
     switch (plan.kind) {
@@ -555,7 +580,7 @@
         rc = tf_time_step_launches(c, s);
         if (rc != GVX_OK) return rc;
     }
-    HIP_TRY(launch_permute01(db.align_tm, align_out, T, B, L, s));
+    if (!plan.side_stream) HIP_TRY(launch_permute01(db.align_tm, align_out, T, B, L, s));
     m->last_decoder_launches = launches;
     if (timed) HIP_TRY(hipEventRecord(m->ev[3], s));
     {
diff --git a/genvox_amd/csrc/gvx_internal.h b/genvox_amd/csrc/gvx_internal.h
--- a/genvox_amd/csrc/gvx_internal.h
+++ b/genvox_amd/csrc/gvx_internal.h
@@ -86,6 +86,7 @@
     unsigned spin_limit = 0;
     int rs_debug = 0;
     bool debug_skip_resident = false;
+    bool prenet_fused = false;
     int debug_enc_skip_block = -1;
     bool debug_plan = false;
     bool timing = false;
@@ -229,12 +230,19 @@
 };
 
 int ensure_side_stream(gvx_model* m);
-int decoder_init_states(gvx_model* m, const float* memory, int B, int L, const DecoderBuffers& db, hipStream_t s);
+int decoder_zero_states_list(const gvx_model* m, int B, int L, const DecoderBuffers& db, void** zp, size_t* zb);
+int decoder_init_states(gvx_model* m, const float* memory, int B, int L, const DecoderBuffers& db, hipStream_t s, bool states_zeroed = false);
+bool prenet_takes_fused_kernel(const gvx_model* m);
 int decoder_prenet_part(gvx_model* m, int B, int L, const float* mel_in, int T, const uint8_t* keep_masks, void* ws, const WsPlan& wp,
                         hipStream_t s);
+struct TfSetupDone {
+    bool prenet = false;
+    bool lengths = false;
+    bool handoff = false;
+};
 int decoder_tf_impl(gvx_model* m, const float* memory, const int32_t* lengths, int B, int L, const float* mel_in, int T,
                     const uint8_t* keep_masks, float* mel_out, float* gate_out, float* align_out, void* ws, const WsPlan& wp,
-                    hipStream_t s, bool prenet_done = false, const LstmDropout* train = nullptr);
+                    hipStream_t s, TfSetupDone done = TfSetupDone{}, const LstmDropout* train = nullptr);
 int poison_if_timed_out(const gvx_model* m, int B, int L, void* ws, const WsPlan& wp, float* const* outs, const size_t* counts, int n,
                         hipStream_t s);
 
diff --git a/genvox_amd/csrc/gvx_kernels.h b/genvox_amd/csrc/gvx_kernels.h
--- a/genvox_amd/csrc/gvx_kernels.h
+++ b/genvox_amd/csrc/gvx_kernels.h
@@ -148,6 +148,7 @@
 bool attention_supported(int L, int a, int F, int kl, int E);
 
 constexpr int HANDOFF_CNT_Q = 0, HANDOFF_CNT_CTX = 1024, HANDOFF_READY = 2048, HANDOFF_TIMEOUT = 3072;
+constexpr int HANDOFF_TICKET = HANDOFF_TIMEOUT + 1;
 constexpr int HANDOFF_STOP = 3072 + 512;
 constexpr int HANDOFF_PAIR = 4096;
 constexpr int HANDOFF_WORDS = 69632;
@@ -283,6 +284,16 @@
 hipError_t launch_embed(const int64_t* tokens, const float* emb, int n_tokens, float* x, float* x2, int B, int L, int E, int halo,
                         int* err_flag, hipStream_t s);
 hipError_t launch_frames_from_mel(const float* mel_in, float* frames, int B, int M, int T, hipStream_t s);
+struct PrenetFusedParams {
+    const float* mel_in;
+    const float* w0; const float* w1;
+    const uint8_t* keep0; const uint8_t* keep1;
+    float* frames; float* pre1; float* prenet;
+    int B, T, M, P;
+};
+bool prenet_fused_supported(int n_mels, int prenet_dim);
+hipError_t prenet_fused_init();
+hipError_t launch_prenet_fused(const PrenetFusedParams& p, hipStream_t s);
 hipError_t launch_split_projection(const float* proj, float* mel_out, float* gate_out, int B, int M, int T, hipStream_t s);
 hipError_t launch_to_channels_last(const float* src, float* dst, int B, int M, int T, int halo, const int32_t* lens, hipStream_t s);
 hipError_t launch_residual_to_channels_first(const float* mel, const float* y, float* mel_post, int B, int M, int T,
@@ -294,6 +305,10 @@
                                hipStream_t s);
 hipError_t launch_zero_many(void* const* ptrs, const size_t* bytes, int n_arrays, hipStream_t s);
 hipError_t launch_poison_on_timeout(const unsigned* tmo, int* sticky, float* const* ptrs, const size_t* counts, int n_arrays, hipStream_t s);
+hipError_t launch_encoder_setup(void* const* ptrs, const size_t* bytes, int n_arrays, const int32_t* len_src, int32_t* len_dst, int n_len,
+                                hipStream_t s);
+hipError_t launch_encoder_tail(unsigned* tmo, unsigned* ticket, int* sticky, float* const* poison, const size_t* counts, int n_poison,
+                               void* const* zero, const size_t* zero_bytes, int n_zero, hipStream_t s);
 hipError_t launch_permute01(const float* src, float* dst, int T, int B, int n, hipStream_t s);
 size_t loss_scratch_bytes();
 hipError_t launch_tacotron2_loss(const float* mel, const float* mel_post, const float* gate, const float* mel_t, const float* gate_t,
diff --git a/genvox_amd/csrc/misc.hip b/genvox_amd/csrc/misc.hip
--- a/genvox_amd/csrc/misc.hip
+++ b/genvox_amd/csrc/misc.hip
@@ -207,6 +207,71 @@
     PoisonArgs a{};
     for (int i = 0; i < 4; ++i) { a.p[i] = i < n_arrays ? ptrs[i] : nullptr; a.n[i] = i < n_arrays && ptrs[i] ? counts[i] : 0; }
     hipLaunchKernelGGL(poison_on_timeout_kernel, dim3(64), dim3(256), 0, s, tmo, sticky, a);
+    return hipGetLastError();
+}
+
+__global__ void encoder_setup_kernel(ZeroArgs a, const int32_t* len_src, int32_t* len_dst, int n_len) {
+    if (blockIdx.x == 0 && blockIdx.y == 0 && (int)threadIdx.x < n_len) len_dst[threadIdx.x] = len_src[threadIdx.x];
+    uint32_t* p = a.p[blockIdx.y];
+    const size_t n = a.n[blockIdx.y];
+    for (size_t k = (size_t)blockIdx.x * blockDim.x + threadIdx.x; k < n; k += (size_t)gridDim.x * blockDim.x) p[k] = 0u;
+}
+hipError_t launch_encoder_setup(void* const* ptrs, const size_t* bytes, int n_arrays, const int32_t* len_src, int32_t* len_dst, int n_len,
+                                hipStream_t s) {
+    if (n_arrays < 1 || n_arrays > 8 || n_len < 0 || n_len > 64 || (n_len > 0 && (!len_src || !len_dst))) return hipErrorInvalidValue;
+    ZeroArgs a{};
+    size_t most = 0;
+    for (int i = 0; i < n_arrays; ++i) {
+        if ((reinterpret_cast<uintptr_t>(ptrs[i]) & 3) || (bytes[i] & 3)) return hipErrorInvalidValue;
+        a.p[i] = reinterpret_cast<uint32_t*>(ptrs[i]); a.n[i] = bytes[i] / 4;
+        if (a.n[i] > most) most = a.n[i];
+    }
+    int gx = (int)((most + 1023) / 1024);
+    if (gx < 1) gx = 1;
+    if (gx > 64) gx = 64;
+    hipLaunchKernelGGL(encoder_setup_kernel, dim3(gx, n_arrays), dim3(256), 0, s, a, len_src, len_dst, n_len);
+    return hipGetLastError();
+}
+
+constexpr int TAIL_BLOCKS = 64;
+__global__ void encoder_tail_kernel(unsigned* tmo, unsigned* ticket, int* sticky, PoisonArgs a, ZeroArgs z, int n_zero) {
+    __shared__ unsigned code_s;
+    if (threadIdx.x == 0) code_s = __hip_atomic_load(tmo, __ATOMIC_RELAXED, __HIP_MEMORY_SCOPE_AGENT);
+    __syncthreads();
+    const unsigned code = code_s;
+    const size_t first = (size_t)blockIdx.x * blockDim.x + threadIdx.x, stride = (size_t)gridDim.x * blockDim.x;
+    if (code != 0u) {
+        if (blockIdx.x == 0 && threadIdx.x == 0) *sticky = (int)code;
+        const float nan = __int_as_float(0x7fc00000);
+#pragma unroll
+        for (int i = 0; i < 4; ++i)
+            for (size_t k = first; k < a.n[i]; k += stride) a.p[i][k] = nan;
+    }
+    for (int i = 0; i < n_zero; ++i)
+        for (size_t k = first; k < z.n[i]; k += stride) z.p[i][k] = 0u;
+    if (threadIdx.x == 0) {
+        const unsigned t = __hip_atomic_fetch_add(ticket, 1u, __ATOMIC_ACQ_REL, __HIP_MEMORY_SCOPE_AGENT);
+        if (t == gridDim.x - 1u) {
+            __hip_atomic_store(tmo, 0u, __ATOMIC_RELAXED, __HIP_MEMORY_SCOPE_AGENT);
+            __hip_atomic_store(ticket, 0u, __ATOMIC_RELAXED, __HIP_MEMORY_SCOPE_AGENT);
+        }
+    }
+}
+hipError_t launch_encoder_tail(unsigned* tmo, unsigned* ticket, int* sticky, float* const* poison, const size_t* counts, int n_poison,
+                               void* const* zero, const size_t* zero_bytes, int n_zero, hipStream_t s) {
+    if (!tmo || !ticket || !sticky || n_poison < 0 || n_poison > 4 || n_zero < 0 || n_zero > 8) return hipErrorInvalidValue;
+    PoisonArgs a{};
+    for (int i = 0; i < 4; ++i) { a.p[i] = i < n_poison ? poison[i] : nullptr; a.n[i] = i < n_poison && poison[i] ? counts[i] : 0; }
+    ZeroArgs z{};
+    for (int i = 0; i < n_zero; ++i) {
+        if ((reinterpret_cast<uintptr_t>(zero[i]) & 3) || (zero_bytes[i] & 3)) return hipErrorInvalidValue;
+        const uint32_t* lo = reinterpret_cast<const uint32_t*>(zero[i]);
+        const uint32_t* hi = lo + zero_bytes[i] / 4;
+        for (const unsigned* w : {(const unsigned*)tmo, (const unsigned*)ticket})
+            if (reinterpret_cast<const uint32_t*>(w) >= lo && reinterpret_cast<const uint32_t*>(w) < hi) return hipErrorInvalidValue;
+        z.p[i] = reinterpret_cast<uint32_t*>(zero[i]); z.n[i] = zero_bytes[i] / 4;
+    }
+    hipLaunchKernelGGL(encoder_tail_kernel, dim3(TAIL_BLOCKS), dim3(256), 0, s, tmo, ticket, sticky, a, z, n_zero);
     return hipGetLastError();
 }
 
diff --git a/genvox_amd/csrc/prenet_fused.hip b/genvox_amd/csrc/prenet_fused.hip
--- /dev/null
+++ b/genvox_amd/csrc/prenet_fused.hip
@@ -0,0 +1,167 @@
+#include "gvx_kernels.h"
+
+namespace gvx {
+
+namespace {
+
+using f32x16 = __attribute__((ext_vector_type(16))) float;
+
+constexpr int PF_BM = 64, PF_BK = 32, PF_LD = PF_BK + 4, PF_THREADS = 512;
+
+template <int P> constexpr int pf_y_ld() { return P + 4; }
+template <int P> constexpr size_t pf_lds_bytes() { return ((size_t)PF_BM * pf_y_ld<P>() + 2 * P * PF_LD + 2 * PF_BM * PF_LD) * sizeof(float); }
+
+template <int P>
+__global__ __launch_bounds__(PF_THREADS) void prenet_fused_kernel(PrenetFusedParams p) {
+    constexpr int TN = P / 128;
+    constexpr int W_V4 = P / 64;
+    constexpr int Y_LD = pf_y_ld<P>();
+    extern __shared__ __attribute__((aligned(16))) float smem[];
+    float* Ys = smem;
+    float* Ws = Ys + PF_BM * Y_LD;
+    float* As = Ws + 2 * P * PF_LD;
+    const int tid = threadIdx.x, lane = tid & 63, wave = tid >> 6;
+    const int wr = wave >> 2, wc = wave & 3;
+    const int r = lane & 31, h = lane >> 5;
+    const int B = p.B, T = p.T, M = p.M;
+    const int rows = (T + 1) * B;
+    const int m0 = (int)blockIdx.x * PF_BM;
+    const int ld_row = tid >> 3, ld_c4 = tid & 7;
+    const int a_m = m0 + ld_row;
+    const bool a_row = a_m < rows && a_m >= B;
+    const int a_t = a_m / B, a_b = a_m - a_t * B;
+    const float* a_src = p.mel_in + ((long)(a_row ? a_b : 0) * M) * T + (a_row ? a_t - 1 : 0);
+    float4 a_reg, w_reg[W_V4];
+
+    auto load_frames = [&](int k0) {
+        const int k = k0 + 4 * ld_c4;
+        const bool ok = a_row && k < M;
+        const float* s = a_src + (long)(ok ? k : 0) * T;
+        const float x = s[0], y = s[T], z = s[2 * (long)T], w = s[3 * (long)T];
+        a_reg = make_float4(ok ? x : 0.f, ok ? y : 0.f, ok ? z : 0.f, ok ? w : 0.f);
+    };
+    auto store_frames = [&](int buf, int k0) {
+        *reinterpret_cast<float4*>(&As[(buf * PF_BM + ld_row) * PF_LD + 4 * ld_c4]) = a_reg;
+        const int k = k0 + 4 * ld_c4;
+        if (a_m < rows && k < M) *reinterpret_cast<float4*>(p.frames + (long)a_m * M + k) = a_reg;
+    };
+    auto load_w = [&](const float* W, int ldw, int K, int k0) {
+        const int k = k0 + 4 * ld_c4;
+        const bool ok = k < K;
+#pragma unroll
+        for (int i = 0; i < W_V4; ++i) {
+            const float4 v = *reinterpret_cast<const float4*>(W + (long)(ld_row + 64 * i) * ldw + (ok ? k : 0));
+            w_reg[i] = make_float4(ok ? v.x : 0.f, ok ? v.y : 0.f, ok ? v.z : 0.f, ok ? v.w : 0.f);
+        }
+    };
+    auto store_w = [&](int buf) {
+#pragma unroll
+        for (int i = 0; i < W_V4; ++i) *reinterpret_cast<float4*>(&Ws[(buf * P + ld_row + 64 * i) * PF_LD + 4 * ld_c4]) = w_reg[i];
+    };
+
+    f32x16 acc[TN];
+    auto clear_acc = [&]() {
+#pragma unroll
+        for (int j = 0; j < TN; ++j)
+#pragma unroll
+            for (int q = 0; q < 16; ++q) acc[j][q] = 0.f;
+    };
+    auto compute_tile = [&](const float* a_base, int wbuf) {
+        const float* b_base = &Ws[(wbuf * P + wc * TN * 32 + r) * PF_LD + 4 * h];
+#pragma unroll
+        for (int kg = 0; kg < PF_BK / 8; ++kg) {
+            const float4 af = *reinterpret_cast<const float4*>(a_base + 8 * kg);
+            float4 bf[TN];
+#pragma unroll
+            for (int j = 0; j < TN; ++j) bf[j] = *reinterpret_cast<const float4*>(b_base + j * 32 * PF_LD + 8 * kg);
+#pragma unroll
+            for (int j = 0; j < TN; ++j) {
+                acc[j] = __builtin_amdgcn_mfma_f32_32x32x2f32(af.x, bf[j].x, acc[j], 0, 0, 0);
+                acc[j] = __builtin_amdgcn_mfma_f32_32x32x2f32(af.y, bf[j].y, acc[j], 0, 0, 0);
+                acc[j] = __builtin_amdgcn_mfma_f32_32x32x2f32(af.z, bf[j].z, acc[j], 0, 0, 0);
+                acc[j] = __builtin_amdgcn_mfma_f32_32x32x2f32(af.w, bf[j].w, acc[j], 0, 0, 0);
+            }
+        }
+    };
+
+    const int nkt1 = (M + PF_BK - 1) / PF_BK;
+    clear_acc();
+    load_frames(0);
+    load_w(p.w0, M, M, 0);
+    store_frames(0, 0);
+    store_w(0);
+    __syncthreads();
+    for (int kt = 0; kt < nkt1; ++kt) {
+        const int cur = kt & 1;
+        const bool more = kt + 1 < nkt1;
+        if (more) { load_frames((kt + 1) * PF_BK); load_w(p.w0, M, M, (kt + 1) * PF_BK); }
+        compute_tile(&As[(cur * PF_BM + wr * 32 + r) * PF_LD + 4 * h], cur);
+        if (more) { store_frames(cur ^ 1, (kt + 1) * PF_BK); store_w(cur ^ 1); }
+        __syncthreads();
+    }
+    load_w(p.w1, P, P, 0);
+#pragma unroll
+    for (int q = 0; q < 16; ++q) {
+        const int lr = wr * 32 + (q & 3) + 8 * (q >> 2) + 4 * h;
+        const int m = m0 + lr;
+        const bool m_ok = m < rows;
+#pragma unroll
+        for (int j = 0; j < TN; ++j) {
+            const int n = wc * TN * 32 + j * 32 + r;
+            float v = fmaxf(acc[j][q], 0.f);
+            v = m_ok && p.keep0[(long)m * P + n] ? 2.f * v : 0.f;
+            Ys[lr * Y_LD + n] = v;
+            if (m_ok) p.pre1[(long)m * P + n] = v;
+        }
+    }
+    store_w(0);
+    __syncthreads();
+    constexpr int nkt2 = P / PF_BK;
+    clear_acc();
+    for (int kt = 0; kt < nkt2; ++kt) {
+        const int cur = kt & 1;
+        const bool more = kt + 1 < nkt2;
+        if (more) load_w(p.w1, P, P, (kt + 1) * PF_BK);
+        compute_tile(&Ys[(wr * 32 + r) * Y_LD + kt * PF_BK + 4 * h], cur);
+        if (more) store_w(cur ^ 1);
+        __syncthreads();
+    }
+#pragma unroll
+    for (int q = 0; q < 16; ++q) {
+        const int m = m0 + wr * 32 + (q & 3) + 8 * (q >> 2) + 4 * h;
+        if (m >= rows) continue;
+        const int t = m / B, b = m - t * B;
+        float* out = p.prenet + (long)t * B * P + (long)b * 8;
+#pragma unroll
+        for (int j = 0; j < TN; ++j) {
+            const int n = wc * TN * 32 + j * 32 + r;
+            float v = fmaxf(acc[j][q], 0.f);
+            v = p.keep1[(long)m * P + n] ? 2.f * v : 0.f;
+            out[(long)(n >> 3) * B * 8 + (n & 7)] = v;
+        }
+    }
+}
+
+}
+
+bool prenet_fused_supported(int n_mels, int prenet_dim) {
+    return (prenet_dim == 128 || prenet_dim == 256) && n_mels >= 4 && n_mels <= 96 && n_mels % 4 == 0;
+}
+
+hipError_t prenet_fused_init() {
+    hipError_t e = hipFuncSetAttribute(reinterpret_cast<const void*>(prenet_fused_kernel<256>), hipFuncAttributeMaxDynamicSharedMemorySize, (int)pf_lds_bytes<256>());
+    if (e != hipSuccess) return e;
+    return hipFuncSetAttribute(reinterpret_cast<const void*>(prenet_fused_kernel<128>), hipFuncAttributeMaxDynamicSharedMemorySize, (int)pf_lds_bytes<128>());
+}
+
+hipError_t launch_prenet_fused(const PrenetFusedParams& p, hipStream_t s) {
+    static_assert(pf_lds_bytes<256>() <= 160 * 1024, "one workgroup's LDS");
+    if (!prenet_fused_supported(p.M, p.P) || p.B < 1 || p.T < 1 || !p.mel_in || !p.w0 || !p.w1 || !p.keep0 || !p.keep1 || !p.frames || !p.pre1 || !p.prenet)
+        return hipErrorInvalidValue;
+    const int grid = ((p.T + 1) * p.B + PF_BM - 1) / PF_BM;
+    if (p.P == 256) prenet_fused_kernel<256><<<dim3(grid), dim3(PF_THREADS), pf_lds_bytes<256>(), s>>>(p);
+    else prenet_fused_kernel<128><<<dim3(grid), dim3(PF_THREADS), pf_lds_bytes<128>(), s>>>(p);
+    return hipGetLastError();
+}
+
+}
diff --git a/include/genvox_amd.h b/include/genvox_amd.h
--- a/include/genvox_amd.h
+++ b/include/genvox_amd.h
@@ -64,6 +64,8 @@
 int gvx_model_set_persistent_attention(gvx_model* model, int enable);
 
 int gvx_model_set_resident_kernels(gvx_model* model, int enable);
+
+int gvx_model_set_prenet_fused(gvx_model* model, int enable);
 
 int gvx_model_set_winograd(gvx_model* model, int mode);
 int gvx_debug_conv_plan(const gvx_model* model, int cin, int cout, int k);
```

Result: no change. 2.044 million, median of 4 (+0.1%).
